# mvenouziou/Boosted_DETR

Measured on AMD Instinct MI355X. Metric: images/sec training step (fwd+matcher+loss+bwd), 640x640 N=100, higher is better.
Workload: dtype f32 (conv/GEMM products as 3 split-f16 [fwd] / split-bf16 [grad] MFMA products, f32 accumulate)

## Files before the change

### boosted_detr_amd/_lib.py

```python
from __future__ import annotations

import ctypes as C
import os
from pathlib import Path

_LIB_PATH = Path(os.environ.get("BDETR_LIB") or Path(__file__).resolve().parent / "csrc" / "libbdetr.so")
_lib = None

c_f32p = C.c_void_p
c_i32p = C.c_void_p
c_i64p = C.c_void_p
c_stream = C.c_void_p


class ConvDesc(C.Structure):
    _fields_ = [(n, C.c_int) for n in ("N", "H", "W", "C", "K", "R", "S", "stride", "pad", "OH", "OW")]


class GemmDesc(C.Structure):
    _fields_ = [
        ("I", C.c_int), ("J", C.c_int), ("R", C.c_int), ("nb0", C.c_int), ("nb1", C.c_int),
        ("a", C.c_void_p), ("lda", C.c_int64), ("sa0", C.c_int64), ("sa1", C.c_int64), ("a_rcontig", C.c_int),
        ("b", C.c_void_p), ("ldb", C.c_int64), ("sb0", C.c_int64), ("sb1", C.c_int64), ("b_rcontig", C.c_int),
        ("c", C.c_void_p), ("ldc", C.c_int64), ("sc0", C.c_int64), ("sc1", C.c_int64),
        ("bias", C.c_void_p), ("alpha", C.c_float), ("act", C.c_int), ("accumulate", C.c_int), ("splitk", C.c_int),
        ("grad", C.c_int),
    ]


class BnAffine(C.Structure):
    _fields_ = [("mean", C.c_void_p), ("rstd", C.c_void_p), ("gamma", C.c_void_p), ("beta", C.c_void_p)]


class BnBwdFuse(C.Structure):
    _fields_ = [("y", C.c_void_p), ("mean", C.c_void_p), ("rstd", C.c_void_p), ("gamma", C.c_void_p), ("beta", C.c_void_p), ("relu", C.c_int),
                ("part_g", C.c_void_p), ("part_gx", C.c_void_p), ("relu_mask", C.c_void_p),
                ("y2", C.c_void_p), ("mean2", C.c_void_p), ("rstd2", C.c_void_p), ("part_gx2", C.c_void_p)]


class RowchainFwdDesc(C.Structure):
    _fields_ = ([("M", C.c_int64), ("nstages", C.c_int), ("eps", C.c_float), ("rate", C.c_float), ("ctx", C.c_void_p), ("resid", C.c_void_p),
                 ("w", C.c_void_p * 3), ("bias", C.c_void_p * 3)]
                + [(n, C.c_void_p) for n in ("g1", "b1", "g2", "b2", "pre1", "x1", "mean1", "rstd1", "h", "pre2", "x2", "mean2", "rstd2")]
                + [("seed1", C.c_uint64), ("seed2", C.c_uint64), ("seed_base", C.c_void_p)])


class RowchainBwdDesc(C.Structure):
    _fields_ = ([("M", C.c_int64), ("nstages", C.c_int), ("rate", C.c_float)]
                + [(n, C.c_void_p) for n in ("dout", "pre2", "mean2", "rstd2", "g2", "h", "pre1", "mean1", "rstd1", "g1")]
                + [("wt", C.c_void_p * 3)]
                + [(n, C.c_void_p) for n in ("G2", "G1", "G0", "dresid", "dctx", "partials")]
                + [("seed1", C.c_uint64), ("seed2", C.c_uint64), ("seed_base", C.c_void_p)])


class LossDesc(C.Structure):
    _fields_ = [("B", C.c_int), ("M", C.c_int), ("N", C.c_int), ("C", C.c_int), ("A", C.c_int),
                ("category_weight", C.c_float), ("attribute_weight", C.c_float),
                ("box_weight", C.c_float), ("exist_weight", C.c_float)]


P = C.c_void_p
I = C.c_int
L = C.c_int64
F = C.c_float
U64 = C.c_uint64

SIGNATURES = {
    "bdetr_abi_version": (I, []),
    "bdetr_last_error": (C.c_char_p, []),
    "bdetr_device_cus": (I, []),
    "bdetr_low_priority_stream_create": (I, [P]),
    "bdetr_side_stream_candidates": (I, [P, I, I, I, P, P, P]),
    "bdetr_stream_destroy": (I, [P]),
    "bdetr_stream_priority_range": (I, [P, P]),
    "bdetr_set_gemm_precision": (I, [I]),
    "bdetr_get_gemm_precision": (I, []),
    "bdetr_prof_enable": (I, [I]),
    "bdetr_prof_read": (I, [P, P, P]),
    "bdetr_prof_read_arith": (I, [I, P, P, P]),
    "bdetr_prof_dump": (I, [C.c_char_p]),
    "bdetr_image_prep": (I, [P, I, I, I, P, I, I, P]),
    "bdetr_tokens_prepare": (I, [P, P, L, I, I, I, P, P, P]),
    "bdetr_augment_ws_floats": (I, [I]),
    "bdetr_augment": (I, [P, P, P, P, I, I, I, P, P]),
    "bdetr_jpeg_quality_ws_bytes": (C.c_int64, [I, I, I]),
    "bdetr_jpeg_quality": (I, [P, P, P, I, I, I, P, P]),
    "bdetr_augment_jpeg": (I, [P, P, P, P, P, I, I, I, P, P, P]),
    "bdetr_conv2d_fwd": (I, [P, P, P, P, C.POINTER(ConvDesc), I, P, P, P]),
    "bdetr_conv2d_fwd_stat_chunks": (I, [C.POINTER(ConvDesc)]),
    "bdetr_conv2d_bwd_data": (I, [P, P, P, C.POINTER(ConvDesc), I, P]),
    "bdetr_conv2d_bwd_weight": (I, [P, P, P, C.POINTER(ConvDesc), I, P]),
    "bdetr_conv2d_bwd_weight_splitk": (I, [C.POINTER(ConvDesc)]),
    "bdetr_bn_apply_p16": (I, [P, P, P, P, P, P, I, C.POINTER(BnAffine), I, P, P, P, P, P, L, I, P]),
    "bdetr_bn_bwd_p16": (I, [P, P, I, P, P, P, P, P, I, I, P, P, P, P, P, P, P, P, I, L, I, P]),
    "bdetr_bn_bwd_p16_even_pixels": (I, [P, P, I, P, P, P, P, P, I, I, P, P, P, P, P, P, I, I, I, I, I, P]),
    "bdetr_p16_supported": (I, [C.POINTER(ConvDesc)]),
    "bdetr_p16_pack": (I, [P, L, P, P, P, P]),
    "bdetr_p16_unpack": (I, [P, I, L, P, P]),
    "bdetr_p16_pack_conv_weights": (I, [P, I, I, I, I, P, P, P, P]),
    "bdetr_p16_pack_conv_weights_multi": (I, [P, I, P, P]),
    "bdetr_p16_conv2d_fwd_stat_chunks": (I, [C.POINTER(ConvDesc)]),
    "bdetr_p16_conv2d_fwd": (I, [P, P, P, P, C.POINTER(ConvDesc), I, P, P, P]),
    "bdetr_p16_conv2d_bwd_data": (I, [P, P, P, C.POINTER(ConvDesc), I, P]),
    "bdetr_p16_conv2d_bwd_data_stat_chunks": (I, [C.POINTER(ConvDesc)]),
    "bdetr_p16_conv2d_bwd_data_masked_accum": (I, [P, P, P, P, C.POINTER(ConvDesc), C.POINTER(BnBwdFuse), P]),
    "bdetr_p16_conv2d_bwd_data_masked_accum_compact": (I, [P, P, P, P, P, C.POINTER(ConvDesc), C.POINTER(BnBwdFuse), P]),
    "bdetr_relu_mask_apply": (I, [P, P, C.c_int64, P]),
    "bdetr_p16_conv2d_bwd_data_bnstats": (I, [P, P, P, C.POINTER(ConvDesc), C.POINTER(BnBwdFuse), P]),
    "bdetr_p16_conv2d_bwd_weight_splitk": (I, [C.POINTER(ConvDesc)]),
    "bdetr_p16_conv2d_bwd_weight": (I, [P, P, P, C.POINTER(ConvDesc), I, P]),
    "bdetr_p16_conv2d_bwd_weight_xf16": (I, [P, P, P, C.POINTER(ConvDesc), I, P]),
    "bdetr_gemm": (I, [C.POINTER(GemmDesc), P]),
    "bdetr_gemm_ws": (I, [C.POINTER(GemmDesc), P, L, P]),
    "bdetr_splitk_workspace_elems": (L, [L, L, I]),
    "bdetr_conv2d_bwd_weight_ws": (I, [P, P, P, C.POINTER(ConvDesc), I, P, L, P]),
    "bdetr_p16_conv2d_bwd_weight_ws": (I, [P, I, P, P, C.POINTER(ConvDesc), I, P, L, P]),
    "bdetr_gemm_grouped": (I, [C.POINTER(GemmDesc), I, P]),
    "bdetr_colsum_chunks": (I, [L]),
    "bdetr_colsum": (I, [P, L, I, P, P, P]),
    "bdetr_colsum_accumulate": (I, [P, L, I, P, P]),
    "bdetr_colsum_accumulate_group": (I, [P, P, I, P, I, P]),
    "bdetr_colstats": (I, [P, L, I, P, P, P]),
    "bdetr_bn_stats": (I, [P, L, I, P, P, I, F, F, I, P, P, P, P, P, P, P]),
    "bdetr_flag_nonfinite": (I, [P, L, P, P]),
    "bdetr_flag_snapshot": (I, [P, P, P, I, P]),
    "bdetr_debug_checksum": (I, [P, L, P, P, P, I, U64, P]),
    "bdetr_graph_node_census": (I, [P, P, I]),
    "bdetr_bn_stats_fold_rows": (I, []),
    "bdetr_bn_stats_frozen": (I, [P, P, I, F, P, P, P]),
    "bdetr_bn_apply": (I, [P, P, P, P, P, P, I, P, L, I, P]),
    "bdetr_bn_bwd_chunks": (I, [L]),
    "bdetr_bn_bwd": (I, [P, P, P, P, P, P, P, I, I, P, P, P, P, P, L, I, P]),
    "bdetr_bn_rows_stats": (I, [P, I, L, I, F, P, P, P, P, P]),
    "bdetr_bn_rows_apply": (I, [P, P, P, P, P, P, I, L, I, I, P, F, P, P, P, P]),
    "bdetr_bn_rows_bwd": (I, [P, P, P, P, P, I, I, P, P, P, P, I, L, I, P]),
    "bdetr_maxpool3x3s2_fwd": (I, [P, P, I, I, I, I, I, I, P]),
    "bdetr_maxpool3x3s2_bwd": (I, [P, P, P, P, I, I, I, I, I, I, P]),
    "bdetr_stem_pool_bwd_chunks": (I, [L]),
    "bdetr_stem_pool_fwd": (I, [P, P, P, P, P, I, I, I, I, P, P, P, P, P]),
    "bdetr_stem_pool_bwd": (I, [P, P, P, P, P, P, P, I, I, I, I, P, I, P, P, P, P]),
    "bdetr_p16_s2d_pack_bf16": (I, [P, I, I, I, P, P]),
    "bdetr_p16_stem_bwd_weight": (I, [P, P, P, I, I, I, I, P]),
    "bdetr_p16_s2d_unpack_dw": (I, [P, P, I, P]),
    "bdetr_attention_head_dim": (I, []),
    "bdetr_attention_fwd": (I, [P, P, P, P, P, I, I, I, I, F, P]),
    "bdetr_attention_bwd": (I, [P, P, P, P, P, P, P, P, P, P, I, I, I, I, F, P]),
    "bdetr_softmax_rows_fwd": (I, [P, P, L, I, F, P]),
    "bdetr_softmax_rows_bwd": (I, [P, P, P, L, I, F, P]),
    "bdetr_add_dropout_layernorm_fwd": (I, [P, P, P, P, P, P, P, L, I, F, F, U64, P, P]),
    "bdetr_ln_bwd_chunks": (I, [L]),
    "bdetr_add_dropout_layernorm_bwd": (I, [P, P, P, P, P, P, P, P, P, P, P, L, I, F, U64, P, I, P]),
    "bdetr_rowchain_fwd": (I, [C.POINTER(RowchainFwdDesc), P]),
    "bdetr_rowchain_bwd": (I, [C.POINTER(RowchainBwdDesc), P]),
    "bdetr_rowchain_reduce": (I, [P, I, C.POINTER(C.c_void_p * 7), C.POINTER(C.c_int * 7), P]),
    "bdetr_rowchain_width": (I, []),
    "bdetr_rowchain_pack_elems": (L, []),
    "bdetr_rowchain_partial_rows": (I, [L]),
    "bdetr_rowchain_pack_weights": (I, [P, I, P, P]),
    "bdetr_resize_bilinear_nhwc": (I, [P, I, I, I, I, P, I, I, P]),
    "bdetr_layernorm_act_fwd": (I, [P, L, I, I, P, P, F, F, P, I, P]),
    "bdetr_copy_cols": (I, [P, L, I, I, P, I, I, P]),
    "bdetr_nhwc_to_nchw": (I, [P, I, I, I, I, P, P]),
    "bdetr_layernorm_act_bwd_chunks": (I, [L]),
    "bdetr_layernorm_act_bwd": (I, [P, L, I, I, P, P, F, F, P, I, P, P, P, P, P, P]),
    "bdetr_resize_bilinear_nhwc_bwd": (I, [P, I, I, I, I, P, I, I, P]),
    "bdetr_nchw_to_nhwc": (I, [P, I, I, I, P, I, P]),
    "bdetr_conv_weight_pack": (I, [P, P, I, I, I, I, I, I, I, P, P, P]),
    "bdetr_conv_weight_unpack": (I, [P, P, I, I, I, I, I, I, P, P, P]),
    "bdetr_mask_loss": (I, [P, P, P, P, I, I, I, I, F, F, F, F, P, P, P, P]),
    "bdetr_softmax_lastdim_fwd": (I, [P, P, L, I, P]),
    "bdetr_softmax_lastdim_bwd": (I, [P, P, P, L, I, P]),
    "bdetr_sigmoid_fwd": (I, [P, P, L, P]),
    "bdetr_sigmoid_bwd": (I, [P, P, P, L, P]),
    "bdetr_boxsigmoid_fwd": (I, [P, P, L, P]),
    "bdetr_boxsigmoid_bwd": (I, [P, P, P, L, P]),
    "bdetr_zero": (I, [P, L, P]),
    "bdetr_add": (I, [P, P, P, L, P]),
    "bdetr_add_bcast_rows": (I, [P, P, P, L, L, P]),
    "bdetr_sum_over_batch": (I, [P, P, L, L, I, P]),
    "bdetr_tanh_bwd": (I, [P, P, P, L, P]),
    "bdetr_relu_bwd": (I, [P, P, P, L, P]),
    "bdetr_axpy": (I, [F, P, P, L, P]),
    "bdetr_cost_matrix": (I, [C.POINTER(LossDesc), P, P, P, P, P, P, P, P, P, P, P, P]),
    "bdetr_lsa": (I, [P, P, I, I, I, P, P]),
    "bdetr_set_loss": (I, [C.POINTER(LossDesc), P, P, P, P, P, P, P, P, P, P, P, P, F, P]),
    "bdetr_cost_matrix_tiled": (I, [C.POINTER(LossDesc), I, P, P, P, P, P, P, P, P, P]),
    "bdetr_lsa_tiled": (I, [P, P, I, I, I, I, P, P]),
    "bdetr_set_loss_tiled": (I, [C.POINTER(LossDesc), I, P, P, P, P, P, P, P, P, P, P, P, P, F, P]),
    "bdetr_match_to_mask": (I, [P, P, I, I, I, P]),
    "bdetr_sgd_slab_elems": (I, []),
    "bdetr_sgd_nesterov_clipnorm": (I, [P, P, I, P, P, I, P, P, P, F, F, F, P, P]),
    "bdetr_adamw_clipnorm": (I, [P, P, I, P, P, I, P, P, P, P, F, F, F, F, F, F, F, P, P]),
    "bdetr_det_postprocess": (I, [P, I, I, I, P, P, P]),
    "bdetr_det_match": (I, [P, P, P, P, P, P, P, I, I, I, I, I, I, P, P, P, P, P]),
    "bdetr_mask_binarize": (I, [P, L, I, F, P, P, P]),
    "bdetr_mask_match": (I, [P, P, P, P, P, P, P, P, P, I, I, I, I, I, I, I, P, P, P, P, P]),
    "bdetr_det_match_coco": (I, [P] * 11 + [I] * 7 + [P] * 7),
    "bdetr_mask_match_coco": (I, [P] * 13 + [I] * 8 + [P] * 7),
    "bdetr_mask_targets": (I, [P, L, P, P, P, P, I, I, I, P, P, P]),
    "bdetr_mask_upsample_bits": (I, [P, P, I, I, I, I, I, P, P, P]),
    "bdetr_mask_source_bits": (I, [P, L, P, P, P, I, I, I, I, P, P, P]),
    "bdetr_mask_inter": (I, [P, P, P, I, I, I, I, I, P, P]),
    "bdetr_mask_match_coco_inter": (I, [P] * 13 + [I] * 7 + [P] * 7),
    "bdetr_panoptic_select": (I, [P, P, P, I, I, I, F, P, P]),
    "bdetr_panoptic_merge": (I, [P, P, P, I, I, I, I, I, P, P, P, P]),
    "bdetr_panoptic_gt_exclusive": (I, [P, P, P, I, I, I, I, I, P, P]),
    "bdetr_panoptic_match": (I, [P] * 8 + [I] * 5 + [P] * 5),
}


class BdetrError(RuntimeError):
    pass


def lib_path() -> Path:
    return _LIB_PATH


def lib():
    global _lib
    if _lib is not None:
        return _lib
    if not _LIB_PATH.exists():
        raise BdetrError(
            f"{_LIB_PATH} not found: the HIP extension is not built. Run `python -m boosted_detr_amd.build` "
            "(or __graft_entry__.build()). There is no CPU fallback in the product path.")
    import torch
    h = C.CDLL(str(_LIB_PATH))
    for name, (res, args) in SIGNATURES.items():
        fn = getattr(h, name)
        fn.restype = res
        fn.argtypes = args
    if h.bdetr_abi_version() != 8:
        raise BdetrError("libbdetr.so ABI version mismatch; rebuild")
    _lib = h
    return _lib


def check(status: int, what: str = "") -> None:
    if status != 0:
        msg = lib().bdetr_last_error().decode(errors="replace")
        raise BdetrError(f"{what or 'libbdetr'} failed (status {status}): {msg}")
```

### boosted_detr_amd/build.py

```python
from __future__ import annotations

import hashlib
import os
import subprocess
import sys
from concurrent.futures import ThreadPoolExecutor
from pathlib import Path

CSRC = Path(__file__).resolve().parent / "csrc"
LIB = CSRC / "libbdetr.so"
OBJ_DIR = CSRC / "_obj"
SOURCES = ["common.cpp", "igemm.hip", "sgemm.hip", "hconv.hip", "hwgrad.hip", "p16.hip", "attention.hip", "rowchain.hip", "augment.hip", "norm.hip", "groupnorm_rows.hip", "elementwise.hip", "panoptic.hip", "matcher.hip", "optim.hip", "detmetric.hip", "maskmetric.hip", "maskraster.hip", "maskimage.hip", "panopticmerge.hip"]
ARCH = "gfx950"
COMMON_FLAGS = ["-O3", "-fPIC", f"--offload-arch={ARCH}", "-std=c++20", "-Wall", "-Wno-unused-function"] + os.environ.get("BDETR_CXXFLAGS", "").split()
PER_FILE_FLAGS = {"matcher.hip": ["-ffp-contract=off"], "detmetric.hip": ["-ffp-contract=off"], "maskmetric.hip": ["-ffp-contract=off"],
                  "maskraster.hip": ["-ffp-contract=off"], "maskimage.hip": ["-ffp-contract=off"], "panopticmerge.hip": ["-ffp-contract=off"]}


def _hipcc() -> str:
    for cand in (os.environ.get("HIPCC"), "/opt/rocm/bin/hipcc", "hipcc"):
        if cand and (os.path.isabs(cand) and os.path.exists(cand) or not os.path.isabs(cand)):
            return cand
    raise RuntimeError("hipcc not found")


def _digest(paths) -> str:
    h = hashlib.sha256()
    for p in sorted(paths):
        h.update(p.name.encode())
        h.update(p.read_bytes())
    return h.hexdigest()


def build(force: bool = False, verbose: bool = True) -> Path:
    deps = [CSRC / s for s in SOURCES] + [CSRC / "common.h", CSRC / "gemm_common.h", CSRC / "p16.h", CSRC.parent.parent / "include" / "bdetr.h"]
    stamp = CSRC / "_obj" / "stamp"
    dig = _digest(deps) + "|" + " ".join(COMMON_FLAGS)
    if not force and LIB.exists() and stamp.exists() and stamp.read_text() == dig:
        return LIB
    OBJ_DIR.mkdir(exist_ok=True)
    hipcc = _hipcc()

    headers = [d for d in deps if d.suffix == ".h"]

    def compile_one(src: str) -> Path:
        obj = OBJ_DIR / (src.rsplit(".", 1)[0] + ".o")
        flags = COMMON_FLAGS + PER_FILE_FLAGS.get(src, [])
        ostamp = OBJ_DIR / (src + ".stamp")
        odig = _digest([CSRC / src] + headers) + "|" + " ".join(flags)
        if not force and obj.exists() and ostamp.exists() and ostamp.read_text() == odig:
            return obj
        cmd = [hipcc, *flags, "-x", "hip", "-c", str(CSRC / src), "-o", str(obj)]
        if verbose:
            print(" ".join(cmd), flush=True)
        subprocess.run(cmd, check=True)
        ostamp.write_text(odig)
        return obj

    with ThreadPoolExecutor(max_workers=min(8, len(SOURCES))) as ex:
        objs = list(ex.map(compile_one, SOURCES))
    cmd = [hipcc, "-shared", "-fPIC", f"--offload-arch={ARCH}", *map(str, objs), "-o", str(LIB)]
    if verbose:
        print(" ".join(cmd), flush=True)
    subprocess.run(cmd, check=True)
    stamp.write_text(dig)
    return LIB


if __name__ == "__main__":
    build(force="--force" in sys.argv)
    print(LIB)
```

### boosted_detr_amd/csrc/igemm.hip

```cpp
#include "gemm_common.h"
#include <stdlib.h>
#include <string.h>
#include <type_traits>
#include <utility>
#include <vector>

using namespace bdgemm;

namespace {

constexpr int BK = 32;
constexpr int RPAD = 4;
constexpr int NTHREADS = 256;

constexpr int SLD = 36;
constexpr int SLD3 = 52;
constexpr float LO_SCALE = 2048.f;
typedef __bf16 bf16x2 __attribute__((ext_vector_type(2)));
typedef __bf16 bf16x8 __attribute__((ext_vector_type(8)));
typedef _Float16 f16x2 __attribute__((ext_vector_type(2)));
typedef _Float16 f16x8 __attribute__((ext_vector_type(8)));
typedef float f32x2 __attribute__((ext_vector_type(2)));

template <int ARITH>
__device__ __forceinline__ void split2(float x0, float x1, unsigned& hi, unsigned& lo) {
    f32x2 v; v[0] = x0; v[1] = x1;
    if (ARITH == AR_BF16X3) {
        hi = __builtin_bit_cast(unsigned, __builtin_convertvector(v, bf16x2));
        f32x2 r;
        r[0] = x0 - __builtin_bit_cast(float, hi << 16);
        r[1] = x1 - __builtin_bit_cast(float, hi & 0xFFFF0000u);
        lo = __builtin_bit_cast(unsigned, __builtin_convertvector(r, bf16x2));
    } else {
        const f16x2 h = __builtin_convertvector(v, f16x2);
        hi = __builtin_bit_cast(unsigned, h);
        const f32x2 r = (v - __builtin_convertvector(h, f32x2)) * LO_SCALE;
        lo = __builtin_bit_cast(unsigned, __builtin_convertvector(r, f16x2));
    }
}

__device__ __forceinline__ void split3(float x0, float x1, unsigned& hi, unsigned& mid, unsigned& lo) {
    f32x2 v; v[0] = x0; v[1] = x1;
    hi = __builtin_bit_cast(unsigned, __builtin_convertvector(v, bf16x2));
    f32x2 r;
    r[0] = x0 - __builtin_bit_cast(float, hi << 16);
    r[1] = x1 - __builtin_bit_cast(float, hi & 0xFFFF0000u);
    mid = __builtin_bit_cast(unsigned, __builtin_convertvector(r, bf16x2));
    r[0] -= __builtin_bit_cast(float, mid << 16);
    r[1] -= __builtin_bit_cast(float, mid & 0xFFFF0000u);
    lo = __builtin_bit_cast(unsigned, __builtin_convertvector(r, bf16x2));
}

struct DenseOp { const float* p; int64_t ld, s0, s1; int rows, cols; };
struct PatchOp { const float* p; int N, H, W, C, OH, OW, R, S, stride, pad; int rows, cols; };
struct WFlipOp { const float* p; int K, C, R, S; int rows, cols; };

typedef unsigned int u32x4 __attribute__((ext_vector_type(4)));
typedef unsigned int u32x2 __attribute__((ext_vector_type(2)));
constexpr unsigned OOB = 0xFFFFFFF0u;
constexpr unsigned NUM_RECORDS = 0xFFFFFF00u;

__device__ __forceinline__ __amdgpu_buffer_rsrc_t make_rsrc(const float* p) {
    const unsigned long long a = reinterpret_cast<unsigned long long>(p);
    const unsigned lo = __builtin_amdgcn_readfirstlane((unsigned)a), hi = __builtin_amdgcn_readfirstlane((unsigned)(a >> 32));
    void* q = reinterpret_cast<void*>(((unsigned long long)hi << 32) | lo);
    return __builtin_amdgcn_make_buffer_rsrc(q, 0, (int)NUM_RECORDS, 0x00020000);
}
__device__ __forceinline__ f32x4 buf_load4(__amdgpu_buffer_rsrc_t r, unsigned byte_off) {
    return __builtin_bit_cast(f32x4, __builtin_amdgcn_raw_buffer_load_b128(r, (int)byte_off, 0, 0));
}
__device__ __forceinline__ float buf_load1(__amdgpu_buffer_rsrc_t r, unsigned byte_off) {
    return __builtin_bit_cast(float, __builtin_amdgcn_raw_buffer_load_b32(r, (int)byte_off, 0, 0));
}

template <int VEC>
struct DenseLoader {
    using Op = DenseOp;
    struct Ctx { unsigned off; bool ok; };
    static __device__ __forceinline__ const float* batch_base(const Op& op, int b0, int b1) {
        return op.p + (int64_t)b0 * op.s0 + (int64_t)b1 * op.s1;
    }
    static __device__ __forceinline__ void regroup(Op& op, const float* p, int x_extent, bool rc) {
        op.p = p;
        if (x_extent >= 0) { if (rc) op.rows = x_extent; else op.cols = x_extent; }
    }
    static __device__ __forceinline__ Ctx row_ctx(const Op& op, int row, int row_limit) {
        Ctx c; c.ok = row < row_limit; c.off = (unsigned)row * (unsigned)op.ld; return c;
    }
    static __device__ __forceinline__ f32x4 load(__amdgpu_buffer_rsrc_t rs, const Op& op, const Ctx& c, int col, int col_limit) {
        if (VEC == 4) {
            return buf_load4(rs, (c.ok && col < col_limit) ? (c.off + (unsigned)col) * 4u : OOB);
        } else {
            f32x4 v;
#pragma unroll
            for (int e = 0; e < 4; ++e) v[e] = buf_load1(rs, (c.ok && col + e < col_limit) ? (c.off + (unsigned)(col + e)) * 4u : OOB);
            return v;
        }
    }
};

struct PatchLoader {
    using Op = PatchOp;
    struct Ctx { int nbase; int ih0, iw0; bool ok; };
    static __device__ __forceinline__ const float* batch_base(const Op& op, int, int) { return op.p; }
    static __device__ __forceinline__ void regroup(Op&, const float*, int, bool) {}
    static __device__ __forceinline__ Ctx row_ctx(const Op& op, int row, int row_limit) {
        Ctx c; c.ok = row < row_limit;
        int ohw = op.OH * op.OW;
        int n = row / ohw; int rem = row - n * ohw;
        int oh = rem / op.OW; int ow = rem - oh * op.OW;
        c.nbase = n * op.H * op.W;
        c.ih0 = oh * op.stride - op.pad; c.iw0 = ow * op.stride - op.pad;
        return c;
    }
    static __device__ __forceinline__ f32x4 load(__amdgpu_buffer_rsrc_t rs, const Op& op, const Ctx& c, int col, int col_limit) {
        int tap = col / op.C; int ch = col - tap * op.C;
        int r = tap / op.S; int s = tap - r * op.S;
        int ih = c.ih0 + r, iw = c.iw0 + s;
        const bool ok = c.ok && col < col_limit && (unsigned)ih < (unsigned)op.H && (unsigned)iw < (unsigned)op.W;
        const unsigned off = ((unsigned)(c.nbase + ih * op.W + iw) * (unsigned)op.C + (unsigned)ch) * 4u;
        return buf_load4(rs, ok ? off : OOB);
    }
};

struct WFlipLoader {
    using Op = WFlipOp;
    struct Ctx { unsigned off; bool ok; };
    static __device__ __forceinline__ const float* batch_base(const Op& op, int, int) { return op.p; }
    static __device__ __forceinline__ void regroup(Op&, const float*, int, bool) {}
    static __device__ __forceinline__ Ctx row_ctx(const Op& op, int row, int row_limit) {
        Ctx c; c.ok = row < row_limit;
        int tap = row / op.K; int k = row - tap * op.K;
        int r = tap / op.S; int s = tap - r * op.S;
        c.off = (unsigned)(((k * op.R + (op.R - 1 - r)) * op.S + (op.S - 1 - s)) * op.C);
        return c;
    }
    static __device__ __forceinline__ f32x4 load(__amdgpu_buffer_rsrc_t rs, const Op& op, const Ctx& c, int col, int col_limit) {
        return buf_load4(rs, (c.ok && col < col_limit) ? (c.off + (unsigned)col) * 4u : OOB);
    }
};

template <int BX, bool RC>
struct TileGeom {
    static constexpr int LDS_FLOATS = RC ? BX * (BK + RPAD) : BK * BX;
    static constexpr int NV = BX * BK / 4 / NTHREADS;
    static constexpr int VPR = RC ? BK / 4 : BX / 4;
    static constexpr int LDS_LD = RC ? BK + RPAD : BX;
};

template <int BM, int BN, int WM, int WN, class LA, bool A_RC, class LB, bool B_RC, int ARITH>
__global__ __launch_bounds__(NTHREADS, 2)
void igemm_kernel(typename LA::Op opa, typename LB::Op opb, GemmParams g)
{
    static_assert(WM * WN == 4, "4 waves per workgroup");
    constexpr int WTM = BM / WM, WTN = BN / WN;
    constexpr int TM = WTM / 32, TN = WTN / 32;
    static_assert(TM >= 1 && TN >= 1, "wave tile must hold at least one 32x32 MFMA tile");
    using GA = TileGeom<BM, A_RC>;
    using GB = TileGeom<BN, B_RC>;
    static_assert(GA::NV >= 1 && GB::NV >= 1, "tile too small for 256 threads");

    constexpr bool SPLIT = ARITH != AR_FP32;
    constexpr bool X6 = ARITH == AR_BF16X6;
    constexpr int SLDK = X6 ? SLD3 : SLD;
    constexpr int A_FLOATS = SPLIT ? BM * SLDK : GA::LDS_FLOATS;
    constexpr int B_FLOATS = SPLIT ? BN * SLDK : GB::LDS_FLOATS;
    constexpr int STAGE_FLOATS = A_FLOATS + B_FLOATS;
    static_assert(!SPLIT || ((A_RC || GA::NV % 2 == 0) && (B_RC || GB::NV % 2 == 0)), "split mode transposes k-pairs");
    __shared__ __attribute__((aligned(16))) float lds[2 * STAGE_FLOATS];

    const int tid = threadIdx.x;
    const int lane = tid & 63;
    const int wave = tid >> 6;
    const int wm = wave / WN, wn = wave % WN;
    const int li = lane & 31, lh = lane >> 5;

    const int nwg_ = g.tiles_i * g.tiles_j;
    const bool sk_ = g.ngroups == 0 && g.splitk > 1;
    const int lin_ = sk_ ? xcd_tile(blockIdx.z * nwg_ + blockIdx.x, nwg_ * gridDim.z) : xcd_tile(blockIdx.x, nwg_);
    const int zz_ = sk_ ? lin_ / nwg_ : blockIdx.z;
    const int wg = sk_ ? lin_ - zz_ * nwg_ : lin_;
    const int tile_i = wg / g.tiles_j, tile_j = wg - tile_i * g.tiles_j;
    const int i0 = tile_i * BM, j0 = tile_j * BN;

    int b0 = 0, b1 = 0, r_begin = 0, r_end = g.R;
    if (g.ngroups > 0) {
        const int z = g.splitk > 1 ? (int)blockIdx.z / g.splitk : (int)blockIdx.z;
        if (g.splitk > 1) {
            r_begin = ((int)blockIdx.z - z * g.splitk) * g.r_chunk;
            r_end = min(g.R, r_begin + g.r_chunk);
        }
#define BDETR_PICK(arr) (z == 0 ? g.arr[0] : z == 1 ? g.arr[1] : z == 2 ? g.arr[2] : g.arr[3])
        g.I = BDETR_PICK(gI); g.c = BDETR_PICK(gc); g.bias = BDETR_PICK(gbias);
        const float* pa = BDETR_PICK(ga);
        const float* pb = BDETR_PICK(gb);
#undef BDETR_PICK
        if (i0 >= g.I) return;
        LA::regroup(opa, pa, g.I, A_RC);
        LB::regroup(opb, pb, -1, B_RC);
    } else if (g.splitk > 1) {
        r_begin = zz_ * g.r_chunk;
        r_end = min(g.R, r_begin + g.r_chunk);
    } else {
        b0 = blockIdx.z / g.nb1; b1 = blockIdx.z - b0 * g.nb1;
    }
    const __amdgpu_buffer_rsrc_t rsA = make_rsrc(LA::batch_base(opa, b0, b1));
    const __amdgpu_buffer_rsrc_t rsB = make_rsrc(LB::batch_base(opb, b0, b1));
    const int a_rows = A_RC ? opa.rows : min(opa.rows, r_end), a_cols = A_RC ? min(opa.cols, r_end) : opa.cols;
    const int b_rows = B_RC ? opb.rows : min(opb.rows, r_end), b_cols = B_RC ? min(opb.cols, r_end) : opb.cols;

    typename LA::Ctx ctxA[GA::NV];
    typename LB::Ctx ctxB[GB::NV];
    int colA[GA::NV], colB[GB::NV], ldsoffA[GA::NV], ldsoffB[GB::NV], rowA[GA::NV], rowB[GB::NV];
    auto stage_geom = [&](int p, int vpr, int bx, bool rc, int lds_ld, int& row, int& col, int& ldsoff) {
        if (!SPLIT) {
            const int v = tid + NTHREADS * p;
            const int rt = v / vpr, c4 = v - rt * vpr;
            row = rt; col = 4 * c4; ldsoff = rt * lds_ld + 4 * c4;
        } else if (rc) {
            const int v = tid + NTHREADS * p;
            const int q = v / vpr, c4 = v - q * vpr;
            const int rt = (q & ~15) | ((q & 3) << 2) | ((q >> 2) & 3);
            row = rt; col = 4 * c4;
            ldsoff = rt * SLDK * 32 + ((((c4 >> 1) ^ ((rt >> 4) & 7)) << 2) | ((c4 & 1) << 1));
        } else {
            const int u = tid + NTHREADS * (p >> 1);
            const int kp = u / (bx / 4), c4 = u - kp * (bx / 4);
            row = 2 * kp + (p & 1); col = 4 * c4;
            ldsoff = (4 * c4) * SLDK * 32 + ((((kp >> 2) ^ ((c4 >> 2) & 7)) << 2) | (kp & 3));
        }
    };
#pragma unroll
    for (int p = 0; p < GA::NV; ++p) {
        stage_geom(p, GA::VPR, BM, A_RC, GA::LDS_LD, rowA[p], colA[p], ldsoffA[p]);
        if (A_RC) ctxA[p] = LA::row_ctx(opa, i0 + rowA[p], a_rows);
    }
#pragma unroll
    for (int p = 0; p < GB::NV; ++p) {
        stage_geom(p, GB::VPR, BN, B_RC, GB::LDS_LD, rowB[p], colB[p], ldsoffB[p]);
        if (B_RC) ctxB[p] = LB::row_ctx(opb, j0 + rowB[p], b_rows);
    }

    f32x4 stA0[GA::NV], stB0[GB::NV], stA1[GA::NV], stB1[GB::NV];
    auto load_stage = [&](int r0, f32x4 (&ra)[GA::NV], f32x4 (&rb)[GB::NV]) {
#pragma unroll
        for (int p = 0; p < GA::NV; ++p) {
            if (A_RC) ra[p] = LA::load(rsA, opa, ctxA[p], r0 + colA[p], a_cols);
            else      ra[p] = LA::load(rsA, opa, LA::row_ctx(opa, r0 + rowA[p], a_rows), i0 + colA[p], a_cols);
        }
#pragma unroll
        for (int p = 0; p < GB::NV; ++p) {
            if (B_RC) rb[p] = LB::load(rsB, opb, ctxB[p], r0 + colB[p], b_cols);
            else      rb[p] = LB::load(rsB, opb, LB::row_ctx(opb, r0 + rowB[p], b_rows), j0 + colB[p], b_cols);
        }
    };
    auto write_split = [&](unsigned* base, bool rc, auto nv_c, const f32x4* r, const int* ldsoff) {
        constexpr int nv = decltype(nv_c)::value;
        if (rc) {
#pragma unroll
            for (int p = 0; p < nv; ++p) {
                unsigned* row = base + (ldsoff[p] >> 5);
                const int w = ldsoff[p] & 31;
                if constexpr (X6) {
                    unsigned h0, m0, l0, h1, m1, l1;
                    split3(r[p][0], r[p][1], h0, m0, l0);
                    split3(r[p][2], r[p][3], h1, m1, l1);
                    u32x2 hi, mid, lo;
                    hi[0] = h0; hi[1] = h1; mid[0] = m0; mid[1] = m1; lo[0] = l0; lo[1] = l1;
                    *reinterpret_cast<u32x2*>(row + w) = hi;
                    *reinterpret_cast<u32x2*>(row + (w ^ 16)) = mid;
                    *reinterpret_cast<u32x2*>(row + 32 + (w & 15)) = lo;
                } else {
                    unsigned h0, l0, h1, l1;
                    split2<ARITH>(r[p][0], r[p][1], h0, l0);
                    split2<ARITH>(r[p][2], r[p][3], h1, l1);
                    u32x2 hi, lo;
                    hi[0] = h0; hi[1] = h1; lo[0] = l0; lo[1] = l1;
                    *reinterpret_cast<u32x2*>(row + w) = hi;
                    *reinterpret_cast<u32x2*>(row + (w ^ 16)) = lo;
                }
            }
        } else {
#pragma unroll
            for (int p = 0; p + 1 < nv; p += 2) {
                unsigned* row = base + (ldsoff[p] >> 5);
                const int w = ldsoff[p] & 31;
#pragma unroll
                for (int e = 0; e < 4; ++e) {
                    if constexpr (X6) {
                        unsigned hi, mid, lo;
                        split3(r[p][e], r[p + 1][e], hi, mid, lo);
                        row[e * SLDK + w] = hi;
                        row[e * SLDK + (w ^ 16)] = mid;
                        row[e * SLDK + 32 + (w & 15)] = lo;
                    } else {
                        unsigned hi, lo;
                        split2<ARITH>(r[p][e], r[p + 1][e], hi, lo);
                        row[e * SLDK + w] = hi;
                        row[e * SLDK + (w ^ 16)] = lo;
                    }
                }
            }
        }
    };
    auto write_stage = [&](int buf, const f32x4 (&ra)[GA::NV], const f32x4 (&rb)[GB::NV]) {
        if (SPLIT) {
            unsigned* st = reinterpret_cast<unsigned*>(lds + buf * STAGE_FLOATS);
            write_split(st, A_RC, std::integral_constant<int, GA::NV>{}, ra, ldsoffA);
            write_split(st + A_FLOATS, B_RC, std::integral_constant<int, GB::NV>{}, rb, ldsoffB);
            return;
        }
#pragma unroll
        for (int p = 0; p < GA::NV; ++p) *reinterpret_cast<f32x4*>(lds + buf * STAGE_FLOATS + ldsoffA[p]) = ra[p];
#pragma unroll
        for (int p = 0; p < GB::NV; ++p) *reinterpret_cast<f32x4*>(lds + buf * STAGE_FLOATS + GA::LDS_FLOATS + ldsoffB[p]) = rb[p];
    };

    constexpr int TM2 = ARITH == AR_FP16X3 ? TM : 1, TN2 = ARITH == AR_FP16X3 ? TN : 1;
    f32x16 acc[TM][TN], acc2[TM2][TN2];
#pragma unroll
    for (int a = 0; a < TM; ++a)
#pragma unroll
        for (int b = 0; b < TN; ++b)
#pragma unroll
            for (int e = 0; e < 16; ++e) acc[a][b][e] = 0.f;
#pragma unroll
    for (int a = 0; a < TM2; ++a)
#pragma unroll
        for (int b = 0; b < TN2; ++b)
#pragma unroll
            for (int e = 0; e < 16; ++e) acc2[a][b][e] = 0.f;

    auto compute = [&](int buf) {
        if (SPLIT) {
            const unsigned* qA = reinterpret_cast<const unsigned*>(lds + buf * STAGE_FLOATS);
            const unsigned* qB = qA + A_FLOATS;
#pragma unroll
            for (int ks = 0; ks < BK / 16; ++ks) {
                u32x4 ah[TM], al[TM], bh[TN], bl[TN];
                u32x4 a3[X6 ? TM : 1], b3[X6 ? TN : 1];
#pragma unroll
                for (int a = 0; a < TM; ++a) {
                    const int xb = wm * WTM + a * 32 + li;
                    const int w = ((ks * 2 + lh) ^ ((xb >> 4) & 7)) << 2;
                    ah[a] = *reinterpret_cast<const u32x4*>(qA + xb * SLDK + w);
                    al[a] = *reinterpret_cast<const u32x4*>(qA + xb * SLDK + (w ^ 16));
                    if constexpr (X6) a3[a] = *reinterpret_cast<const u32x4*>(qA + xb * SLDK + 32 + (w & 15));
                }
#pragma unroll
                for (int b = 0; b < TN; ++b) {
                    const int xb = wn * WTN + b * 32 + li;
                    const int w = ((ks * 2 + lh) ^ ((xb >> 4) & 7)) << 2;
                    bh[b] = *reinterpret_cast<const u32x4*>(qB + xb * SLDK + w);
                    bl[b] = *reinterpret_cast<const u32x4*>(qB + xb * SLDK + (w ^ 16));
                    if constexpr (X6) b3[b] = *reinterpret_cast<const u32x4*>(qB + xb * SLDK + 32 + (w & 15));
                }
#pragma unroll
                for (int a = 0; a < TM; ++a)
#pragma unroll
                    for (int b = 0; b < TN; ++b) {
                        if constexpr (X6) {
#define BF8(v) __builtin_bit_cast(bf16x8, v)
                            acc[a][b] = __builtin_amdgcn_mfma_f32_32x32x16_bf16(BF8(a3[a]), BF8(bh[b]), acc[a][b], 0, 0, 0);
                            acc[a][b] = __builtin_amdgcn_mfma_f32_32x32x16_bf16(BF8(ah[a]), BF8(b3[b]), acc[a][b], 0, 0, 0);
                            acc[a][b] = __builtin_amdgcn_mfma_f32_32x32x16_bf16(BF8(al[a]), BF8(bl[b]), acc[a][b], 0, 0, 0);
                            acc[a][b] = __builtin_amdgcn_mfma_f32_32x32x16_bf16(BF8(al[a]), BF8(bh[b]), acc[a][b], 0, 0, 0);
                            acc[a][b] = __builtin_amdgcn_mfma_f32_32x32x16_bf16(BF8(ah[a]), BF8(bl[b]), acc[a][b], 0, 0, 0);
                            acc[a][b] = __builtin_amdgcn_mfma_f32_32x32x16_bf16(BF8(ah[a]), BF8(bh[b]), acc[a][b], 0, 0, 0);
#undef BF8
                        } else if constexpr (ARITH == AR_BF16X3) {
#define BF8(v) __builtin_bit_cast(bf16x8, v)
                            acc[a][b] = __builtin_amdgcn_mfma_f32_32x32x16_bf16(BF8(al[a]), BF8(bh[b]), acc[a][b], 0, 0, 0);
                            acc[a][b] = __builtin_amdgcn_mfma_f32_32x32x16_bf16(BF8(ah[a]), BF8(bl[b]), acc[a][b], 0, 0, 0);
                            acc[a][b] = __builtin_amdgcn_mfma_f32_32x32x16_bf16(BF8(ah[a]), BF8(bh[b]), acc[a][b], 0, 0, 0);
#undef BF8
                        } else if constexpr (ARITH == AR_FP16X3) {
#define H8(v) __builtin_bit_cast(f16x8, v)
                            acc2[a][b] = __builtin_amdgcn_mfma_f32_32x32x16_f16(H8(al[a]), H8(bh[b]), acc2[a][b], 0, 0, 0);
                            acc2[a][b] = __builtin_amdgcn_mfma_f32_32x32x16_f16(H8(ah[a]), H8(bl[b]), acc2[a][b], 0, 0, 0);
                            acc[a][b] = __builtin_amdgcn_mfma_f32_32x32x16_f16(H8(ah[a]), H8(bh[b]), acc[a][b], 0, 0, 0);
#undef H8
                        }
                    }
            }
            return;
        }
        const float* sA = lds + buf * STAGE_FLOATS;
        const float* sB = sA + GA::LDS_FLOATS;
#pragma unroll
        for (int kb = 0; kb < BK / 8; ++kb) {
            f32x4 fa[TM], fb[TN];
#pragma unroll
            for (int a = 0; a < TM; ++a) {
                const int xb = wm * WTM + a * 32 + li;
                if (A_RC) {
                    fa[a] = *reinterpret_cast<const f32x4*>(sA + xb * GA::LDS_LD + kb * 8 + 4 * lh);
                } else {
#pragma unroll
                    for (int e = 0; e < 4; ++e) fa[a][e] = sA[(kb * 8 + 4 * lh + e) * GA::LDS_LD + xb];
                }
            }
#pragma unroll
            for (int b = 0; b < TN; ++b) {
                const int xb = wn * WTN + b * 32 + li;
                if (B_RC) {
                    fb[b] = *reinterpret_cast<const f32x4*>(sB + xb * GB::LDS_LD + kb * 8 + 4 * lh);
                } else {
#pragma unroll
                    for (int e = 0; e < 4; ++e) fb[b][e] = sB[(kb * 8 + 4 * lh + e) * GB::LDS_LD + xb];
                }
            }
#pragma unroll
            for (int e = 0; e < 4; ++e)
#pragma unroll
                for (int a = 0; a < TM; ++a)
#pragma unroll
                    for (int b = 0; b < TN; ++b)
                        acc[a][b] = __builtin_amdgcn_mfma_f32_32x32x2f32(fa[a][e], fb[b][e], acc[a][b], 0, 0, 0);
        }
    };

    const int nk = (r_end - r_begin + BK - 1) / BK;
    constexpr bool PF1 = SPLIT && BM * BN >= 128 * 128;
    if constexpr (PF1) {
        if (nk > 0) { load_stage(r_begin, stA0, stB0); write_stage(0, stA0, stB0); }
        __syncthreads();
        for (int kt = 0; kt < nk; ++kt) {
            if (kt + 1 < nk) load_stage(r_begin + (kt + 1) * BK, stA0, stB0);
            compute(kt & 1);
            if (kt + 1 < nk) write_stage((kt + 1) & 1, stA0, stB0);
            __syncthreads();
        }
    } else {
    if (nk > 0) {
        load_stage(r_begin, stA0, stB0);
        if (nk > 1) load_stage(r_begin + BK, stA1, stB1);
        write_stage(0, stA0, stB0);
    }
    __syncthreads();

    for (int kt = 0; kt < nk; kt += 2) {
        if (kt + 2 < nk) load_stage(r_begin + (kt + 2) * BK, stA0, stB0);
        compute(0);
        if (kt + 1 < nk) write_stage(1, stA1, stB1);
        __syncthreads();
        if (kt + 1 >= nk) break;
        if (kt + 3 < nk) load_stage(r_begin + (kt + 3) * BK, stA1, stB1);
        compute(1);
        if (kt + 2 < nk) write_stage(0, stA0, stB0);
        __syncthreads();
    }
    }

    if constexpr (ARITH == AR_FP16X3) {
#pragma unroll
        for (int a = 0; a < TM; ++a)
#pragma unroll
            for (int b = 0; b < TN; ++b)
#pragma unroll
                for (int e = 0; e < 16; ++e) acc[a][b][e] += acc2[a][b][e] * (1.f / LO_SCALE);
    }
    gemm_epilogue<BM, BN, WM, WN, NTHREADS, 2 * STAGE_FLOATS>(acc, g, lds, tile_i, i0, j0, g.c + (int64_t)(sk_ ? zz_ : b0) * g.sc0 + (int64_t)b1 * g.sc1);
}

struct TileChoice { int bm, bn; };

}

namespace bdgemm {
int g_num_cus = 0;
int num_cus() {
    if (g_num_cus == 0) {
        int dev = 0; hipDeviceProp_t p;
        if (hipGetDevice(&dev) == hipSuccess && hipGetDeviceProperties(&p, dev) == hipSuccess) g_num_cus = p.multiProcessorCount;
        if (g_num_cus <= 0) g_num_cus = 256;
    }
    return g_num_cus;
}
}

namespace {

}
namespace bdgemm {
thread_local int g_gemm_mode = -1;
int gemm_mode() {
    if (g_gemm_mode < 0) {
        const char* e = getenv("BDETR_GEMM_PRECISION");
        g_gemm_mode = !e ? BDETR_GEMM_MIXED : (!strcmp(e, "fp32") || !strcmp(e, "f32")) ? BDETR_GEMM_FP32
                    : !strcmp(e, "bf16x3") ? BDETR_GEMM_BF16X3 : !strcmp(e, "split") ? BDETR_GEMM_SPLIT : !strcmp(e, "bf16x6") ? BDETR_GEMM_BF16X6 : BDETR_GEMM_MIXED;
    }
    return g_gemm_mode;
}
}
namespace {
int use_split(bool grad) {
    switch (gemm_mode()) {
        case BDETR_GEMM_FP32:   return AR_FP32;
        case BDETR_GEMM_BF16X3: return AR_BF16X3;
        case BDETR_GEMM_SPLIT:  return grad ? AR_BF16X3 : AR_FP16X3;
        case BDETR_GEMM_BF16X6: return AR_BF16X6;
        default:                return grad ? AR_BF16X3 : AR_FP32;
    }
}

TileChoice choose_tile(int I, int J, int zdim, bool both_rc, bool split, bool patch = false) {
    static int forced_bm = -1, forced_bn = -1;
    if (forced_bm < 0) {
        forced_bm = forced_bn = 0;
        if (const char* e = getenv("BDETR_TILE")) sscanf(e, "%dx%d", &forced_bm, &forced_bn);
    }
    if (forced_bm > 0) {
        if (J <= 32) return {128, 32};
        return {forced_bm, forced_bn};
    }
    auto tiles = [&](int bm, int bn) { return cdiv64(I, bm) * cdiv64(J, bn) * zdim; };
    if (J <= 32) return {128, 32};
    if (split) {
        if (both_rc && J % 128 == 0 && tiles(128, 128) * 4 >= 3LL * num_cus()) return {128, 128};
        if (patch && !both_rc && I % 128 == 0 && J % 128 == 0 && (zdim > 1 || tiles(128, 128) * 4 >= 3LL * num_cus())) return {128, 128};
        return {64, 64};
    }
    if (tiles(128, 128) >= 16LL * num_cus() && J >= 1024) return {128, 128};
    return {64, 64};
}

struct ProfRec { hipEvent_t e0, e1; double flops; int I, J, R, z, bm, bn, kind; };
std::vector<ProfRec> g_prof_recs;
std::vector<std::pair<hipEvent_t, hipEvent_t>> g_prof_pool;
size_t g_prof_used = 0;

template <class L> struct LoaderId { static constexpr int v = 0; };
template <> struct LoaderId<PatchLoader> { static constexpr int v = 1; };
template <> struct LoaderId<WFlipLoader> { static constexpr int v = 2; };
template <> struct LoaderId<DenseLoader<1>> { static constexpr int v = 3; };

}
namespace bdgemm {
bool g_prof_on = false;
void prof_begin(hipStream_t st, double flops, int I, int J, int R, int z, int bm, int bn, int kind) {
    if (g_prof_used == g_prof_pool.size()) {
        hipEvent_t a, b;
        if (hipEventCreate(&a) != hipSuccess || hipEventCreate(&b) != hipSuccess) return;
        g_prof_pool.emplace_back(a, b);
    }
    auto& ev = g_prof_pool[g_prof_used++];
    g_prof_recs.push_back({ev.first, ev.second, flops, I, J, R, z, bm, bn, kind});
    (void)hipEventRecord(ev.first, st);
}
void prof_end(hipStream_t st) { (void)hipEventRecord(g_prof_recs.back().e1, st); }
}
namespace {

template <int BM, int BN, int WM, int WN, class LA, bool A_RC, class LB, bool B_RC, int ARITH = AR_FP32>
int launch_cfg(const typename LA::Op& a, const typename LB::Op& b, GemmParams g, int zdim, hipStream_t st) {
    g.tiles_i = (int)cdiv64(g.I, BM);
    g.tiles_j = (int)cdiv64(g.J, BN);
    dim3 grid(g.tiles_i * g.tiles_j, 1, zdim);
    g.vec_store = (g.J % 4 == 0) && (g.ldc % 4 == 0) && (g.sc0 % 4 == 0) && (g.sc1 % 4 == 0) && ((reinterpret_cast<uintptr_t>(g.c) & 15) == 0);
    const bool prof = g_prof_on;
    if (prof) prof_begin(st, 2.0 * (double)g.I * (double)g.J * (double)g.R * (g.splitk > 1 ? (g.ngroups > 0 ? (double)g.ngroups : 1.0) : (double)zdim), g.I, g.J, g.R, zdim, BM, BN,
                         ARITH * 10000 + LoaderId<LA>::v * 1000 + (A_RC ? 100 : 0) + LoaderId<LB>::v * 10 + (B_RC ? 1 : 0));
    hipLaunchKernelGGL((igemm_kernel<BM, BN, WM, WN, LA, A_RC, LB, B_RC, ARITH>), grid, dim3(NTHREADS), 0, st, a, b, g);
    if (prof) prof_end(st);
    return bdetr_launch_status("igemm");
}

template <class LA, bool A_RC, class LB, bool B_RC>
int launch_any(const typename LA::Op& a, const typename LB::Op& b, GemmParams g, int zdim, hipStream_t st, int arith, bool small_only = false) {
    if (arith == AR_FP16X3 && !(A_RC && B_RC)) arith = AR_FP32;
    constexpr bool PATCH = LoaderId<LA>::v == 1 || LoaderId<LB>::v == 1;
    TileChoice t = small_only ? TileChoice{64, 64} : choose_tile(g.I, g.J, g.splitk > 1 ? 2 : zdim, A_RC && B_RC, arith != AR_FP32, PATCH);
    if constexpr (LoaderId<LA>::v != 3 && LoaderId<LB>::v != 3) {
        if (arith == AR_BF16X3 && t.bn >= 64) {
            if (t.bm == 128 && t.bn == 128) return launch_cfg<128, 128, 2, 2, LA, A_RC, LB, B_RC, AR_BF16X3>(a, b, g, zdim, st);
            if (t.bm == 128 && t.bn == 64)  return launch_cfg<128, 64, 2, 2, LA, A_RC, LB, B_RC, AR_BF16X3>(a, b, g, zdim, st);
            return launch_cfg<64, 64, 2, 2, LA, A_RC, LB, B_RC, AR_BF16X3>(a, b, g, zdim, st);
        }
        if (arith == AR_BF16X6 && t.bn >= 64) {
            if (t.bm == 128) return launch_cfg<128, 64, 2, 2, LA, A_RC, LB, B_RC, AR_BF16X6>(a, b, g, zdim, st);
            return launch_cfg<64, 64, 2, 2, LA, A_RC, LB, B_RC, AR_BF16X6>(a, b, g, zdim, st);
        }
        if constexpr (A_RC && B_RC) {
            if (arith == AR_FP16X3 && t.bn >= 64) {
                if (t.bm == 128 && t.bn == 128) return launch_cfg<128, 128, 2, 2, LA, A_RC, LB, B_RC, AR_FP16X3>(a, b, g, zdim, st);
                if (t.bm == 128 && t.bn == 64)  return launch_cfg<128, 64, 2, 2, LA, A_RC, LB, B_RC, AR_FP16X3>(a, b, g, zdim, st);
                return launch_cfg<64, 64, 2, 2, LA, A_RC, LB, B_RC, AR_FP16X3>(a, b, g, zdim, st);
            }
        }
    }
    if (t.bm == 128 && t.bn == 128) return launch_cfg<128, 128, 2, 2, LA, A_RC, LB, B_RC>(a, b, g, zdim, st);
    if (t.bm == 128 && t.bn == 64)  return launch_cfg<128, 64, 2, 2, LA, A_RC, LB, B_RC>(a, b, g, zdim, st);
    if (t.bm == 128 && t.bn == 32)  return launch_cfg<128, 32, 4, 1, LA, A_RC, LB, B_RC>(a, b, g, zdim, st);
    return launch_cfg<64, 64, 2, 2, LA, A_RC, LB, B_RC>(a, b, g, zdim, st);
}

constexpr int64_t MAX_OPERAND_ELEMS = (int64_t)(NUM_RECORDS / 4) - 64;
bool span_ok(int64_t elems) { return elems >= 0 && elems <= MAX_OPERAND_ELEMS; }
int64_t dense_span(const DenseOp& o) { return (int64_t)(o.rows - 1) * o.ld + o.cols; }

int stat_chunks(int I, int J) {
    TileChoice t = choose_tile(I, J, 1, true, use_split(false) != AR_FP32);
    const int wm = (t.bm == 128 && t.bn == 32) ? 4 : 2;
    return (int)cdiv64(I, t.bm) * wm;
}

__global__ __launch_bounds__(256) void splitk_fold_kernel(const float* __restrict__ ws, int zdim, int64_t slab, float* __restrict__ dst, int64_t n) {
    const int64_t i = ((int64_t)blockIdx.x * 256 + threadIdx.x) * 4;
    if (i >= n) return;
    if (i + 4 <= n && (reinterpret_cast<uintptr_t>(dst) & 15) == 0) {
        f32x4 a = *reinterpret_cast<const f32x4*>(ws + i);
        for (int z = 1; z < zdim; ++z) a += *reinterpret_cast<const f32x4*>(ws + (int64_t)z * slab + i);
        f32x4 d = *reinterpret_cast<f32x4*>(dst + i);
        d += a;
        *reinterpret_cast<f32x4*>(dst + i) = d;
    } else {
        for (int64_t k = i; k < n && k < i + 4; ++k) {
            float a = ws[k];
            for (int z = 1; z < zdim; ++z) a += ws[(int64_t)z * slab + k];
            dst[k] += a;
        }
    }
}

}

namespace bdgemm {
int splitk_fold(const float* ws, int zdim, int64_t slab, float* dst, int64_t n, hipStream_t st) {
    hipLaunchKernelGGL(splitk_fold_kernel, dim3((unsigned)cdiv64(cdiv64(n, 4), 256)), dim3(256), 0, st, ws, zdim, slab, dst, n);
    return bdetr_launch_status("splitk_fold");
}
}

extern "C" int64_t bdetr_splitk_workspace_elems(int64_t I, int64_t J, int splitk) {
    return splitk > 1 ? (int64_t)splitk * bdgemm::splitk_slab(I * J) : 0;
}

extern "C" int bdetr_device_cus(void) { return num_cus(); }

extern "C" int bdetr_set_gemm_precision(int mode) {
    BDETR_CHECK_ARG(mode >= BDETR_GEMM_FP32 && mode <= BDETR_GEMM_BF16X6, "bdetr_set_gemm_precision: unknown mode %d", mode);
    bdgemm::g_gemm_mode = mode;
    return 0;
}
extern "C" int bdetr_get_gemm_precision(void) { return gemm_mode(); }

extern "C" int bdetr_prof_enable(int on) {
    g_prof_on = on != 0;
    if (on) { g_prof_recs.clear(); g_prof_used = 0; }
    return 0;
}
extern "C" int bdetr_prof_dump(const char* path) {
    FILE* f = fopen(path, "w");
    if (!f) { bdetr_set_error("bdetr_prof_dump: cannot open %s", path); return -1; }
    fprintf(f, "I,J,R,z,bm,bn,kind,ms,gflop\n");
    for (auto& r : g_prof_recs) {
        float t = 0.f;
        if (hipEventElapsedTime(&t, r.e0, r.e1) != hipSuccess) t = -1.f;
        fprintf(f, "%d,%d,%d,%d,%d,%d,%d,%.5f,%.4f\n", r.I, r.J, r.R, r.z, r.bm, r.bn, r.kind, t, r.flops * 1e-9);
    }
    fclose(f);
    return 0;
}

static int prof_sum(int arith, double* total_ms, int64_t* launches, double* flops) {
    double ms = 0, fl = 0; int64_t n = 0;
    for (auto& r : g_prof_recs) {
        if (arith >= 0 && r.kind / 10000 != arith) continue;
        float t = 0.f;
        hipError_t e = hipEventElapsedTime(&t, r.e0, r.e1);
        if (e != hipSuccess) { bdetr_set_error("bdetr_prof_read: %s", hipGetErrorString(e)); return (int)e; }
        ms += t; fl += r.flops; ++n;
    }
    if (total_ms) *total_ms = ms;
    if (launches) *launches = n;
    if (flops) *flops = fl;
    return 0;
}
extern "C" int bdetr_prof_read(double* total_ms, int64_t* launches, double* flops) { return prof_sum(-1, total_ms, launches, flops); }
extern "C" int bdetr_prof_read_arith(int arith, double* total_ms, int64_t* launches, double* flops) {
    BDETR_CHECK_ARG(arith >= AR_FP32 && arith <= AR_BF16X6, "bdetr_prof_read_arith: arith must be 0 (fp32), 1 (bf16x3), 2 (fp16x3), 3 (pre-split f16), 4 (pre-split bf16) or 5 (bf16x6)");
    return prof_sum(arith, total_ms, launches, flops);
}

extern "C" int bdetr_gemm_grouped(const bdetr_gemm_desc* d, int n, void* stream) {
    BDETR_CHECK_ARG(d && n >= 1 && n <= 4, "bdetr_gemm_grouped: 1..4 problems");
    GemmParams g; init_params(g);
    int maxI = 0;
    bool v4 = true;
    for (int k = 0; k < n; ++k) {
        const bdetr_gemm_desc& e = d[k];
        BDETR_CHECK_ARG(e.a && e.b && e.c && e.I > 0, "bdetr_gemm_grouped: null pointer / empty problem %d", k);
        BDETR_CHECK_ARG(e.J == d[0].J && e.R == d[0].R && e.a_rcontig == d[0].a_rcontig && e.b_rcontig == d[0].b_rcontig &&
                        e.act == d[0].act && e.alpha == d[0].alpha && e.accumulate == d[0].accumulate &&
                        e.lda == d[0].lda && e.ldb == d[0].ldb && e.ldc == d[0].ldc,
                        "bdetr_gemm_grouped: problems must share J, R, leading dimensions, flavours and epilogue");
        BDETR_CHECK_ARG(e.grad == d[0].grad, "bdetr_gemm_grouped: problems must share the grad flag");
        BDETR_CHECK_ARG((e.nb0 <= 1) && (e.nb1 <= 1) && e.splitk == d[0].splitk, "bdetr_gemm_grouped: no batching inside a group; one split-K factor for all problems");
        BDETR_CHECK_ARG(e.splitk <= 1 || (!e.bias && e.act == 0 && e.I == d[0].I), "bdetr_gemm_grouped: split-K problems are plain GEMMs of one shape (C += partial products, atomics)");
        BDETR_CHECK_ARG(span_ok((int64_t)(e.a_rcontig ? e.I : e.R) * e.lda) && span_ok((int64_t)(e.b_rcontig ? e.J : e.R) * e.ldb),
                        "bdetr_gemm_grouped: operand %d spans 4 GB or more (32-bit buffer offsets)", k);
        g.ga[k] = e.a; g.gb[k] = e.b; g.gc[k] = e.c; g.gbias[k] = e.bias; g.gI[k] = e.I;
        if (e.I > maxI) maxI = e.I;
        v4 = v4 && aligned16(e.a) && aligned16(e.b) && aligned16(e.c);
    }
    const bdetr_gemm_desc& f = d[0];
    bool dims4 = f.J % 4 == 0 && (f.a_rcontig || f.b_rcontig ? f.R % 4 == 0 : true);
    for (int k = 0; k < n; ++k) dims4 = dims4 && (f.a_rcontig || d[k].I % 4 == 0);
    BDETR_CHECK_ARG(v4 && f.lda % 4 == 0 && f.ldb % 4 == 0 && f.ldc % 4 == 0 && dims4,
                    "bdetr_gemm_grouped: operands must be 16-byte aligned with contiguous dimensions that are multiples of 4");
    g.ngroups = n;
    g.I = maxI; g.J = f.J; g.R = f.R;
    g.c = f.c; g.ldc = f.ldc; g.bias = f.bias; g.alpha = f.alpha; g.act = f.act;
    g.mode = f.accumulate ? ST_ACCUM : ST_STORE;
    int zdim = n;
    if (f.splitk > 1) {
        g.r_chunk = (int)(cdiv64(cdiv64(f.R, f.splitk), BK) * BK);
        g.splitk = (int)cdiv64(f.R, g.r_chunk);
        g.mode = ST_ATOMIC;
        zdim = n * g.splitk;
    }
    DenseOp a{f.a, f.lda, 0, 0, f.a_rcontig ? maxI : f.R, f.a_rcontig ? f.R : maxI};
    DenseOp b{f.b, f.ldb, 0, 0, f.b_rcontig ? f.J : f.R, f.b_rcontig ? f.R : f.J};
    hipStream_t st = (hipStream_t)stream;
    const bool arc = f.a_rcontig != 0, brc = f.b_rcontig != 0;
    const int sp = use_split(f.grad != 0);
    if (arc && brc)   return launch_any<DenseLoader<4>, true, DenseLoader<4>, true>(a, b, g, zdim, st, sp);
    if (arc && !brc)  return launch_any<DenseLoader<4>, true, DenseLoader<4>, false>(a, b, g, zdim, st, sp);
    if (!arc && !brc) return launch_any<DenseLoader<4>, false, DenseLoader<4>, false>(a, b, g, zdim, st, sp);
    return launch_any<DenseLoader<4>, false, DenseLoader<4>, true>(a, b, g, zdim, st, sp, true);
}

extern "C" int bdetr_gemm(const bdetr_gemm_desc* d, void* stream) { return bdetr_gemm_ws(d, nullptr, 0, stream); }

template <class F>
static int with_splitk_slabs(GemmParams& g, int zdim, float* ws, int64_t ws_elems, hipStream_t st, const char* who, F&& launch) {
    float* c = g.c;
    const int64_t n = (int64_t)g.I * g.J, slab = splitk_slab(n);
    BDETR_CHECK_ARG(g.ldc == g.J, "%s: the split-K workspace form needs a dense C (ldc == J)", who);
    BDETR_CHECK_ARG(aligned16(ws) && ws_elems >= (int64_t)zdim * slab, "%s: workspace too small or misaligned (%lld floats, need %lld)", who,
                    (long long)ws_elems, (long long)((int64_t)zdim * slab));
    g.c = ws; g.sc0 = slab; g.mode = ST_STORE;
    if (int e = launch()) return e;
    return splitk_fold(ws, zdim, slab, c, n, st);
}

extern "C" int bdetr_gemm_ws(const bdetr_gemm_desc* d, float* ws, int64_t ws_elems, void* stream) {
    BDETR_CHECK_ARG(d && d->a && d->b && d->c, "bdetr_gemm: null pointer");
    BDETR_CHECK_ARG(d->I > 0 && d->J > 0 && d->R >= 0, "bdetr_gemm: bad shape I=%d J=%d R=%d", d->I, d->J, d->R);
    const int nb0 = d->nb0 > 0 ? d->nb0 : 1, nb1 = d->nb1 > 0 ? d->nb1 : 1;
    const int splitk = d->splitk > 1 ? d->splitk : 1;
    BDETR_CHECK_ARG(splitk == 1 || (nb0 * nb1 == 1 && !d->bias && d->act == 0), "bdetr_gemm: splitk needs a single plain GEMM");
    hipStream_t st = (hipStream_t)stream;

    DenseOp a{d->a, d->lda, d->sa0, d->sa1, d->a_rcontig ? d->I : d->R, d->a_rcontig ? d->R : d->I};
    DenseOp b{d->b, d->ldb, d->sb0, d->sb1, d->b_rcontig ? d->J : d->R, d->b_rcontig ? d->R : d->J};
    BDETR_CHECK_ARG(span_ok(dense_span(a)) && span_ok(dense_span(b)),
                    "bdetr_gemm: an operand matrix spans 4 GB or more (32-bit buffer offsets); split the problem");
    GemmParams g; init_params(g);
    g.I = d->I; g.J = d->J; g.R = d->R; g.nb1 = nb1;
    g.c = d->c; g.ldc = d->ldc; g.sc0 = d->sc0; g.sc1 = d->sc1;
    g.bias = d->bias; g.alpha = d->alpha; g.act = d->act;
    g.mode = splitk > 1 ? ST_ATOMIC : (d->accumulate ? ST_ACCUM : ST_STORE);
    int zdim = nb0 * nb1;
    if (splitk > 1) {
        g.splitk = splitk;
        g.r_chunk = (int)(cdiv64(cdiv64(d->R, splitk), BK) * BK);
        zdim = (int)cdiv64(d->R, g.r_chunk);
        g.splitk = zdim > 1 ? zdim : 2;
    }
    auto vec_ok = [&](const DenseOp& o) {
        return aligned16(o.p) && o.ld % 4 == 0 && o.s0 % 4 == 0 && o.s1 % 4 == 0 && o.cols % 4 == 0;
    };
    const bool v4 = vec_ok(a) && vec_ok(b);
    const bool arc = d->a_rcontig != 0, brc = d->b_rcontig != 0;
    const int sp = use_split(d->grad != 0);
    auto launch = [&]() -> int {
        if (v4) {
            if (arc && brc)   return launch_any<DenseLoader<4>, true, DenseLoader<4>, true>(a, b, g, zdim, st, sp);
            if (arc && !brc)  return launch_any<DenseLoader<4>, true, DenseLoader<4>, false>(a, b, g, zdim, st, sp);
            if (!arc && !brc) return launch_any<DenseLoader<4>, false, DenseLoader<4>, false>(a, b, g, zdim, st, sp);
            return launch_any<DenseLoader<4>, false, DenseLoader<4>, true>(a, b, g, zdim, st, sp, true);
        }
        if (arc && brc)   return launch_any<DenseLoader<1>, true, DenseLoader<1>, true>(a, b, g, zdim, st, AR_FP32, true);
        if (arc && !brc)  return launch_any<DenseLoader<1>, true, DenseLoader<1>, false>(a, b, g, zdim, st, AR_FP32, true);
        if (!arc && !brc) return launch_any<DenseLoader<1>, false, DenseLoader<1>, false>(a, b, g, zdim, st, AR_FP32, true);
        return launch_any<DenseLoader<1>, false, DenseLoader<1>, true>(a, b, g, zdim, st, AR_FP32, true);
    };
    if (ws != nullptr && splitk > 1) return with_splitk_slabs(g, zdim, ws, ws_elems, st, "bdetr_gemm_ws", launch);
    return launch();
}

static int check_conv(const bdetr_conv_desc* d, const char* who) {
    BDETR_CHECK_ARG(d != nullptr, "%s: null desc", who);
    BDETR_CHECK_ARG(d->N > 0 && d->H > 0 && d->W > 0 && d->C > 0 && d->K > 0 && d->R > 0 && d->S > 0 && d->stride > 0 && d->pad >= 0,
                    "%s: bad conv geometry", who);
    BDETR_CHECK_ARG(d->C % 4 == 0, "%s: input channels must be a multiple of 4 (got %d)", who, d->C);
    BDETR_CHECK_ARG(d->OH == (d->H + 2 * d->pad - d->R) / d->stride + 1 && d->OW == (d->W + 2 * d->pad - d->S) / d->stride + 1,
                    "%s: OH/OW inconsistent with geometry", who);
    BDETR_CHECK_ARG((int64_t)d->N * d->OH * d->OW < (1LL << 31) && (int64_t)d->R * d->S * d->C < (1LL << 31), "%s: problem too large", who);
    BDETR_CHECK_ARG(span_ok((int64_t)d->N * d->H * d->W * d->C) && span_ok((int64_t)d->N * d->OH * d->OW * d->K) && span_ok((int64_t)d->K * d->R * d->S * d->C),
                    "%s: a tensor spans 4 GB or more (the loaders use 32-bit buffer offsets); use a smaller per-GPU batch", who);
    return 0;
}

extern "C" int bdetr_conv2d_fwd_stat_chunks(const bdetr_conv_desc* d) {
    if (check_conv(d, "bdetr_conv2d_fwd_stat_chunks")) return -1;
    return stat_chunks(d->N * d->OH * d->OW, d->K);
}

extern "C" int bdetr_conv2d_fwd(const float* x, const float* w, const float* bias, float* y,
                                const bdetr_conv_desc* d, int act, float* stat_sum, float* stat_sq, void* stream) {
    if (int e = check_conv(d, "bdetr_conv2d_fwd")) return e;
    BDETR_CHECK_ARG(x && w && y, "bdetr_conv2d_fwd: null pointer");
    BDETR_CHECK_ARG(aligned16(x) && aligned16(w), "bdetr_conv2d_fwd: x and w must be 16-byte aligned");
    BDETR_CHECK_ARG((stat_sum == nullptr) == (stat_sq == nullptr), "bdetr_conv2d_fwd: stat_sum/stat_sq must both be set or both null");
    const int M = d->N * d->OH * d->OW, Kd = d->R * d->S * d->C;
    GemmParams g; init_params(g);
    g.I = M; g.J = d->K; g.R = Kd;
    g.c = y; g.ldc = d->K; g.bias = bias; g.act = act;
    g.stat_sum = stat_sum; g.stat_sq = stat_sq;
    DenseOp wop{w, Kd, 0, 0, d->K, Kd};
    hipStream_t st = (hipStream_t)stream;
    if (d->R == 1 && d->S == 1 && d->stride == 1 && d->pad == 0) {
        DenseOp xop{x, d->C, 0, 0, M, d->C};
        return launch_any<DenseLoader<4>, true, DenseLoader<4>, true>(xop, wop, g, 1, st, use_split(false));
    }
    PatchOp xop{x, d->N, d->H, d->W, d->C, d->OH, d->OW, d->R, d->S, d->stride, d->pad, M, Kd};
    return launch_any<PatchLoader, true, DenseLoader<4>, true>(xop, wop, g, 1, st, use_split(false));
}

extern "C" int bdetr_conv2d_bwd_data(const float* dy, const float* w, float* dx,
                                     const bdetr_conv_desc* d, int accumulate, void* stream) {
    if (int e = check_conv(d, "bdetr_conv2d_bwd_data")) return e;
    BDETR_CHECK_ARG(dy && w && dx, "bdetr_conv2d_bwd_data: null pointer");
    BDETR_CHECK_ARG(d->K % 4 == 0, "bdetr_conv2d_bwd_data: output channels must be a multiple of 4");
    hipStream_t st = (hipStream_t)stream;
    const int M = d->N * d->OH * d->OW;
    GemmParams g; init_params(g);
    g.c = dx; g.ldc = d->C; g.mode = accumulate ? ST_ACCUM : ST_STORE;
    if (d->R == 1 && d->S == 1 && d->pad == 0) {
        g.I = M; g.J = d->C; g.R = d->K;
        if (d->stride > 1) {
            if (!accumulate) {
                if (int e = bdetr_zero_bytes(dx, sizeof(float) * (size_t)d->N * d->H * d->W * d->C, st)) return e;
            }
            g.rowmap = 1; g.rm_OW = d->OW; g.rm_OHOW = d->OH * d->OW; g.rm_H = d->H; g.rm_W = d->W; g.rm_stride = d->stride;
        }
        DenseOp a{dy, d->K, 0, 0, M, d->K};
        DenseOp b{w, d->C, 0, 0, d->K, d->C};
        return launch_any<DenseLoader<4>, true, DenseLoader<4>, false>(a, b, g, 1, st, use_split(true));
    }
    if (d->stride > 1 && d->pad == 0 && d->R <= d->stride && d->S <= d->stride) {
        if (!accumulate) {
            if (int e = bdetr_zero_bytes(dx, sizeof(float) * (size_t)d->N * d->H * d->W * d->C, st)) return e;
        }
        g.I = M; g.J = d->C; g.R = d->K;
        g.rowmap = 1; g.rm_OW = d->OW; g.rm_OHOW = d->OH * d->OW; g.rm_H = d->H; g.rm_W = d->W; g.rm_stride = d->stride;
        DenseOp a{dy, d->K, 0, 0, M, d->K};
        for (int r = 0; r < d->R; ++r)
            for (int s = 0; s < d->S; ++s) {
                g.rm_off = r * d->W + s;
                DenseOp b{w + (int64_t)(r * d->S + s) * d->C, (int64_t)d->R * d->S * d->C, 0, 0, d->K, d->C};
                if (int e = launch_any<DenseLoader<4>, true, DenseLoader<4>, false>(a, b, g, 1, st, use_split(true))) return e;
            }
        return 0;
    }
    BDETR_CHECK_ARG(d->stride == 1, "bdetr_conv2d_bwd_data: stride>1 only for 1x1 convs or taps that do not overlap (R, S <= stride, pad 0)");
    const int Mx = d->N * d->H * d->W;
    g.I = Mx; g.J = d->C; g.R = d->R * d->S * d->K;
    PatchOp a{dy, d->N, d->OH, d->OW, d->K, d->H, d->W, d->R, d->S, 1, d->R - 1 - d->pad, Mx, d->R * d->S * d->K};
    BDETR_CHECK_ARG(d->R == d->S, "bdetr_conv2d_bwd_data: square kernels only");
    WFlipOp b{w, d->K, d->C, d->R, d->S, d->R * d->S * d->K, d->C};
    return launch_any<PatchLoader, true, WFlipLoader, false>(a, b, g, 1, st, use_split(true));
}

extern "C" int bdetr_conv2d_bwd_weight_splitk(const bdetr_conv_desc* d) {
    if (check_conv(d, "bdetr_conv2d_bwd_weight_splitk")) return -1;
    const int M = d->N * d->OH * d->OW, Kd = d->R * d->S * d->C;
    TileChoice t = choose_tile(d->K, Kd, 2, false, use_split(true) != AR_FP32, !(d->R == 1 && d->S == 1 && d->stride == 1 && d->pad == 0));
    int64_t tiles = cdiv64(d->K, t.bm) * cdiv64(Kd, t.bn);
    int64_t want = 3LL * num_cus();
    const bool few_tiles = tiles <= 8 && M >= (1 << 20);
    if (few_tiles) want = 16LL * num_cus();
    int64_t sk = cdiv64(want, tiles);
// ... 42 lines not shown
```

### boosted_detr_amd/engine.py

```python
from __future__ import annotations

import math
import zlib
from typing import Callable, Dict, List, Optional, Sequence

import numpy as np
import torch

from . import kernels as K

_DEVICE = None


def device() -> torch.device:
    global _DEVICE
    if _DEVICE is None:
        if not torch.cuda.is_available():
            raise RuntimeError("boosted_detr_amd needs an AMD GPU (HIP device); there is no CPU execution path")
        _DEVICE = torch.device("cuda", torch.cuda.current_device())
    return _DEVICE


def to_device(a, dtype=torch.float32) -> torch.Tensor:
    if isinstance(a, torch.Tensor):
# ... 50 lines not shown
            a = a.T
        return np.ascontiguousarray(a)

    def _to_keras(self, a: np.ndarray) -> np.ndarray:
        if self.kind == "conv_kernel":
            if self.pad_in_channels:
                a = a[..., : a.shape[3] - self.pad_in_channels]
            a = np.transpose(a, (1, 2, 3, 0))
        elif self.kind == "dense_kernel":
            a = a.T
        return np.ascontiguousarray(a)

    def assign(self, keras_array) -> None:
        t = to_device(self._to_internal(np.asarray(keras_array)))
        bump_weights_version()
        if self.value is None:
            self.value = t
        else:
            self.value.copy_(t)

    def numpy(self) -> np.ndarray:
        return self._to_keras(self.value.detach().cpu().numpy())

    def grad_numpy(self) -> np.ndarray:
        return self._to_keras(self.grad.detach().cpu().numpy())

    @property
    def num_params(self) -> int:
        return int(np.prod(self.keras_shape))

    @property
    def needs_grad(self) -> bool:
        return self.trainable and getattr(self, "owner", None) is not None and self.owner.trainable

    def reset_grad(self) -> None:
        self.grad, self._grad_fresh = None, False


def _seed_for(name: str, seed: int) -> int:
    return (zlib.crc32(name.encode()) ^ (seed * 0x9E3779B1)) & 0xFFFFFFFF


def _fans(shape):
    if len(shape) == 2:
        return shape[0], shape[1]
    rf = int(np.prod(shape[:-2]))
    return shape[-2] * rf, shape[-1] * rf


def initializer(kind: str) -> Callable:
    def trunc_normal(rng, shape, std):
        out = rng.standard_normal(shape)
        bad = np.abs(out) > 2.0
        while bad.any():
            out[bad] = rng.standard_normal(int(bad.sum()))
            bad = np.abs(out) > 2.0
        return (out * std / 0.87962566103423978).astype(np.float32)

    def init(name, shape, seed=0):
        rng = np.random.Generator(np.random.PCG64(_seed_for(name, seed)))
        fan_in, fan_out = _fans(shape) if len(shape) >= 2 else (shape[0], shape[0])
        if kind == "zeros":
            return np.zeros(shape, np.float32)
        if kind == "ones":
            return np.ones(shape, np.float32)
        if kind == "glorot_normal":
            return trunc_normal(rng, shape, math.sqrt(2.0 / (fan_in + fan_out)))
        if kind == "he_normal":
            return trunc_normal(rng, shape, math.sqrt(2.0 / fan_in))
        if kind == "lecun_normal":
            return trunc_normal(rng, shape, math.sqrt(1.0 / fan_in))
        if kind == "glorot_uniform":
            lim = math.sqrt(6.0 / (fan_in + fan_out))
            return rng.uniform(-lim, lim, size=shape).astype(np.float32)
        raise ValueError(kind)

    return init


class GradInfo:
    __slots__ = ("owned", "lazy_mask", "compact_even", "even_pixels", "bnb_parts", "bnb_parts_shortcut")

    def __init__(self):
        self.owned = False
        self.lazy_mask = self.compact_even = self.even_pixels = self.bnb_parts = self.bnb_parts_shortcut = None


_NO_INFO = GradInfo()


def info(g) -> GradInfo:
    return getattr(g, "_grad_info", _NO_INFO)


def tag(g: torch.Tensor) -> GradInfo:
    r = getattr(g, "_grad_info", None)
    if r is None:
        r = g._grad_info = GradInfo()
    return r


def own(t: torch.Tensor) -> torch.Tensor:
    tag(t).owned = True
    return t


def dense_contribution(g: torch.Tensor, keep_even=None) -> None:
    r = info(g)
    if r is _NO_INFO:
        return
    r.bnb_parts = r.bnb_parts_shortcut = None
    if r.even_pixels != keep_even:
        r.even_pixels = None


def materialise(g):
    r = info(g)
    if r.compact_even is not None:
        N, H, W = r.compact_even
        d = torch.empty(N, H, W, g.shape[-1], dtype=g.dtype, device=g.device)
        K.zero_(d)
        d[:, ::2, ::2] = g.view(N, H // 2, W // 2, g.shape[-1])
        mask, r = r.lazy_mask, tag(d)
        r.owned, r.even_pixels, r.lazy_mask = True, (N, H, W), mask
        g = d
    if r.lazy_mask is not None:
        K.relu_mask_apply_(g, r.lazy_mask)
        r.lazy_mask = None
    return g


class Tape:

    def __init__(self):
        self.nodes: List[tuple] = []

    def record(self, outputs: Sequence[torch.Tensor], inputs: Sequence[Optional[torch.Tensor]], fn: Callable) -> None:
        self.nodes.append((tuple(outputs), tuple(inputs), fn))

    def backward(self, seeds: Dict[int, torch.Tensor]) -> Dict[int, torch.Tensor]:
        grads: Dict[int, torch.Tensor] = dict(seeds)
        for outputs, inputs, fn in reversed(self.nodes):
            gouts = [grads.pop(id(o), None) for o in outputs]
            if all(g is None for g in gouts):
                continue
            if not getattr(fn, "accepts_lazy", False):
                gouts = [materialise(g) for g in gouts]
            acc = None
            if getattr(fn, "wants_acc", False):
                acc = []
                for t in inputs:
                    have = grads.get(id(t)) if t is not None else None
                    acc.append(have if info(have).owned else None)
                gins = fn(*gouts, acc=acc)
            else:
                gins = fn(*gouts)
            if not isinstance(gins, (tuple, list)):
                gins = (gins,)
            assert len(gins) == len(inputs), (len(gins), len(inputs))
            for i, (t, g) in enumerate(zip(inputs, gins)):
                if t is None or g is None:
                    continue
                key = id(t)
                if key in grads:
                    if acc is not None and acc[i] is not None and g is acc[i]:
                        grads[key] = g
                        continue
                    g, have = materialise(g), materialise(grads[key])
                    dense_contribution(have)
                    if info(have).owned:
                        K.axpy_(1.0, g.view(have.shape), have)
                        grads[key] = have
                    else:
                        grads[key] = own(K.add(have, g.view(have.shape)))
                else:
                    grads[key] = g
            if _CAPTURE[0] is not None:
                _CAPTURE[0].maybe_cut(next((g for g in gins if isinstance(g, torch.Tensor)), None) if _DEBUG_LOG[0] is not None else None)
            elif _DEBUG_LOG[0] is not None and _DEBUG_LOG[0].eager_pending >= SegmentedCapture.SIDE_TASKS_PER_SEGMENT:
                _debug_cut(next((g for g in gins if isinstance(g, torch.Tensor)), None))
        return grads


_TAPE: Optional[Tape] = None
_CAPTURE = [None]


def capture() -> Optional["SegmentedCapture"]:
    return _CAPTURE[0]


def set_capture(cap: Optional["SegmentedCapture"]) -> None:
    _CAPTURE[0] = cap

import os as _os

_SIDE = {"stream": None, "enabled": _os.environ.get("BDETR_SIDE_STREAM", "1") != "0", "used": False, "keep": []}


def side_stream() -> Optional["torch.cuda.Stream"]:
    if not _SIDE["enabled"]:
        return None
    if _SIDE["stream"] is None:
        if _os.environ.get("BDETR_SIDE_PRIORITY", "low") == "low":
            import ctypes as _C
            from . import _lib
            for _ in range(int(_os.environ.get("BDETR_SIDE_QUEUE_SKIP", "0"))):
                d = _C.c_void_p()
                _lib.check(_lib.lib().bdetr_low_priority_stream_create(_C.byref(d)), "low_priority_stream_create")
                _SIDE.setdefault("dummies", []).append(d)
            ncand = int(_os.environ.get("BDETR_SIDE_CANDIDATES", "4"))
            if ncand > 1 and not torch.cuda.is_current_stream_capturing():
                _SIDE["placement"] = {"picked": None, "tick_ms": [], "unloaded_ms": None, "good": [], "limit": ncand}
                _SIDE["candidates"] = []
                _more_candidates(1)
                while not _SIDE["placement"]["good"] and len(_SIDE["placement"]["tick_ms"]) < ncand:
                    _more_candidates(1)
                pl = _SIDE["placement"]
                pick = pl["good"][0] if pl["good"] else min(range(len(pl["tick_ms"])), key=lambda c: pl["tick_ms"][c])
                pl["picked"] = pick
                _SIDE["stream"] = _SIDE["candidates"][pick]
                side_stream_release()
            else:
                h = _C.c_void_p()
                _lib.check(_lib.lib().bdetr_low_priority_stream_create(_C.byref(h)), "low_priority_stream_create")
                _SIDE["stream"] = torch.cuda.ExternalStream(h.value, device=device())
        else:
            _SIDE["stream"] = torch.cuda.Stream(device=device())
    return _SIDE["stream"]


SIDE_BAD_RATIO = 3.0


def _more_candidates(n: int) -> None:
    import ctypes as _C
    from . import _lib
    pl = _SIDE["placement"]
    hs, scores, base = (_C.c_void_p * n)(), (_C.c_float * n)(), _C.c_float(0.0)
    _lib.check(_lib.lib().bdetr_side_stream_candidates(_C.c_void_p(torch.cuda.current_stream().cuda_stream), n, 120, 200, hs, scores, _C.byref(base)),
               "side_stream_candidates")
    if pl["unloaded_ms"] is None:
        pl["unloaded_ms"] = round(float(base.value), 3)
    for c in range(n):
        _SIDE["candidates"].append(torch.cuda.ExternalStream(hs[c], device=device()))
        pl["tick_ms"].append(round(float(scores[c]), 3))
        if float(scores[c]) < SIDE_BAD_RATIO * max(pl["unloaded_ms"], 1e-3):
            pl["good"].append(len(pl["tick_ms"]) - 1)


def side_stream_expand() -> list:
    pl = _SIDE.get("placement")
    if pl is None or _SIDE["used"] or torch.cuda.is_current_stream_capturing():
        return [] if pl is None else [c for c in pl["good"] if _SIDE["candidates"][c] is not None]
    while len(pl["tick_ms"]) < pl["limit"]:
        _more_candidates(1)
    return [c for c in pl["good"] if _SIDE["candidates"][c] is not None]


def side_stream_release() -> None:
    from . import _lib
    if _SIDE["used"]:
        raise RuntimeError("side_stream_release: side-stream work is pending (join_side_stream first)")
    for c, st in enumerate(_SIDE.get("candidates", [])):
        if st is not None and st is not _SIDE["stream"]:
            st.synchronize()
            _lib.check(_lib.lib().bdetr_stream_destroy(st.cuda_stream), "stream_destroy")
            _SIDE["candidates"][c] = None


def side_stream_placement() -> Optional[dict]:
    return _SIDE.get("placement")


def side_stream_select(index: int) -> None:
    if _SIDE["used"]:
        raise RuntimeError("side_stream_select: side-stream work is pending (join_side_stream first)")
    if _SIDE["candidates"][index] is None:
        raise RuntimeError(f"side_stream_select: candidate {index} was released")
    _SIDE["stream"] = _SIDE["candidates"][index]
    _SIDE["placement"]["picked"] = index


def set_side_stream_enabled(on: bool) -> None:
    _SIDE["enabled"] = bool(on)


class on_side_stream:

    def __init__(self, *tensors):
        self.tensors = [t for t in tensors if t is not None]
        self.side = side_stream()

    def __enter__(self):
        if self.side is None:
            return self
        ev = torch.cuda.Event()
        ev.record()
        self.side.wait_event(ev)
        _SIDE["keep"].extend(self.tensors)
        self.ctx = torch.cuda.stream(self.side)
        self.ctx.__enter__()
        self.prev_handle = K.set_launch_stream(self.side.cuda_stream if K._LAUNCH_STREAM[0] is not None else None)
        _SIDE["used"] = True
        return self

    def __exit__(self, *exc):
# ... 340 lines not shown
```

### boosted_detr_amd/kernels.py

```python
from __future__ import annotations

import ctypes as C
from dataclasses import dataclass
from typing import Optional, Tuple

import numpy as np
import torch

from . import _lib
from ._lib import BnAffine, BnBwdFuse, ConvDesc, GemmDesc, LossDesc, RowchainBwdDesc, RowchainFwdDesc, check

ACT_NONE, ACT_RELU, ACT_TANH = 0, 1, 2


_LAUNCH_STREAM = [None]


def set_launch_stream(handle: Optional[int]) -> Optional[int]:
    prev = _LAUNCH_STREAM[0]
    _LAUNCH_STREAM[0] = handle
    return prev


GEMM_FP32, GEMM_BF16X3, GEMM_MIXED, GEMM_SPLIT, GEMM_BF16X6 = 0, 1, 2, 3, 4
_GEMM_MODES = {"fp32": GEMM_FP32, "bf16x3": GEMM_BF16X3, "mixed": GEMM_MIXED, "split": GEMM_SPLIT, "bf16x6": GEMM_BF16X6}


def set_gemm_precision(mode) -> int:
    code = _GEMM_MODES.get(mode, mode)
    prev = _lib.lib().bdetr_get_gemm_precision()
    check(_lib.lib().bdetr_set_gemm_precision(int(code)), "set_gemm_precision")
    return prev


def get_gemm_precision() -> str:
    code = _lib.lib().bdetr_get_gemm_precision()
    return next(k for k, v in _GEMM_MODES.items() if v == code)


def demote_split_forward() -> None:
    L = _lib.lib()
    if L.bdetr_get_gemm_precision() == GEMM_SPLIT:
        check(L.bdetr_set_gemm_precision(GEMM_MIXED), "set_gemm_precision")


import os as _os

_DETERMINISTIC = [_os.environ.get("BDETR_DETERMINISTIC", "0") == "1"]


def set_deterministic(on: bool) -> bool:
    prev = _DETERMINISTIC[0]
    _DETERMINISTIC[0] = bool(on)
    return prev


def deterministic() -> bool:
    return _DETERMINISTIC[0]


def _splitk_ws(rows: int, cols: int, sk: int, like: torch.Tensor):
    if not _DETERMINISTIC[0] or sk <= 1:
        return None, 0
    n = int(_lib.lib().bdetr_splitk_workspace_elems(rows, cols, sk))
    return torch.empty(n, dtype=torch.float32, device=like.device), n


class gemm_precision:

    def __init__(self, mode):
        self.mode = mode

    def __enter__(self):
        self.prev = set_gemm_precision(self.mode) if self.mode is not None else None
        return self

    def __exit__(self, *exc):
        if self.prev is not None:
            set_gemm_precision(self.prev)
        return False


def _stream() -> int:
    h = _LAUNCH_STREAM[0]
    return h if h is not None else torch.cuda.current_stream().cuda_stream


def _p(t: Optional[torch.Tensor]) -> Optional[int]:
    if t is None:
        return None
    return t.data_ptr()


def _chk(*tensors, dtype=torch.float32):
    for t in tensors:
        if t is None:
            continue
        if not t.is_cuda:
            raise _lib.BdetrError("kernel operands must live in HBM (cuda tensors); no CPU path exists")
        if t.dtype != dtype:
            raise _lib.BdetrError(f"expected {dtype}, got {t.dtype}")
        if not t.is_contiguous():
            raise _lib.BdetrError("kernel operands must be contiguous")


def empty(*shape, like: torch.Tensor, dtype=torch.float32) -> torch.Tensor:
    return torch.empty(shape, dtype=dtype, device=like.device)


def image_prep(image: torch.Tensor, H: int, W: int) -> torch.Tensor:
    _chk(image)
    B, h, w, c = image.shape
    assert c == 3
    out = empty(B, H, W, 4, like=image)
    check(_lib.lib().bdetr_image_prep(_p(image), B, h, w, _p(out), H, W, _stream()), "image_prep")
    return out


def tokens_prepare(cat_ids: torch.Tensor, att_ids: torch.Tensor, C_: int, A: int):
    _chk(cat_ids, att_ids, dtype=torch.int32)
    if cat_ids.dim() == 3:
        cat_ids = cat_ids[..., 0].contiguous()
    B, M = cat_ids.shape
    slots = att_ids.shape[2] if att_ids.dim() == 3 else 1
    cat = torch.empty_like(cat_ids)
    hot = torch.empty((B, M, A), dtype=torch.float32, device=cat_ids.device)
    check(_lib.lib().bdetr_tokens_prepare(_p(cat_ids), _p(att_ids), B * M, slots, C_, A, _p(cat), _p(hot), _stream()), "tokens_prepare")
    return cat, hot


def augment(image: torch.Tensor, iparams: torch.Tensor, fparams: torch.Tensor, quality: Optional[torch.Tensor] = None) -> torch.Tensor:
    _chk(image, fparams)
    _chk(iparams, dtype=torch.int32)
    B, H, W, c = image.shape
    assert c == 3
    L = _lib.lib()
    out = torch.empty_like(image)
    ws = empty(L.bdetr_augment_ws_floats(B), like=image)
    if quality is None:
        check(L.bdetr_augment(_p(image), _p(out), _p(iparams), _p(fparams), B, H, W, _p(ws), _stream()), "augment")
        return out
    _chk(quality, dtype=torch.int32)
    jws = torch.empty(int(L.bdetr_jpeg_quality_ws_bytes(B, H, W)), dtype=torch.uint8, device=image.device)
    check(L.bdetr_augment_jpeg(_p(image), _p(out), _p(iparams), _p(fparams), _p(quality), B, H, W, _p(ws), _p(jws), _stream()), "augment_jpeg")
    return out


def jpeg_quality(image: torch.Tensor, quality: torch.Tensor) -> torch.Tensor:
    _chk(image)
    _chk(quality, dtype=torch.int32)
    B, H, W, c = image.shape
    assert c == 3 and quality.numel() == B
    L = _lib.lib()
    out = torch.empty_like(image)
    jws = torch.empty(int(L.bdetr_jpeg_quality_ws_bytes(B, H, W)), dtype=torch.uint8, device=image.device)
    check(L.bdetr_jpeg_quality(_p(image), _p(out), _p(quality), B, H, W, _p(jws), _stream()), "jpeg_quality")
    return out


@dataclass(frozen=True)
class ConvGeom:
    N: int
    H: int
# ... 162 lines not shown
    ws = empty(2 * Cc * L.bdetr_bn_bwd_chunks(rows), like=x2d) if pre is None else None
    if even_pixels is not None and pre is None:
        N, H, W = even_pixels
        assert N * H * W == rows
        assert not dout_compact or (dres is None and dout.numel() == N * (H // 2) * (W // 2) * Cc and H % 2 == 0 and W % 2 == 0)
        check(L.bdetr_bn_bwd_p16_even_pixels(_p(dout), _p(out), int(out_p16), _p(x2d), _p(mean), _p(rstd), _p(gamma), _p(beta), int(relu), int(frozen),
                                             _p(dx32), _p(dxb), _p(dgamma), _p(dbeta), _p(dres), _p(ws), N, H, W, Cc, int(dout_compact), _stream()), "bn_bwd_p16_even_pixels")
        return dxb, dx32, dgamma, dbeta, dres
    assert not dout_compact, "a compact dout goes through the even-pixel reduction (even_pixels=(N, H, W), no pre)"
    pg, pgx, pn = pre if pre is not None else (None, None, 0)
    check(L.bdetr_bn_bwd_p16(_p(dout), _p(out), int(out_p16), _p(x2d), _p(mean), _p(rstd), _p(gamma), _p(beta), int(relu), int(frozen), _p(dx32),
                             _p(dxb), _p(dgamma), _p(dbeta), _p(dres), _p(ws), _p(pg), _p(pgx), int(pn), rows, Cc, _stream()), "bn_bwd_p16")
    return dxb, dx32, dgamma, dbeta, dres


def p16_pack_conv_weights_multi(table: torch.Tensor) -> None:
    _chk(table, dtype=torch.int64)
    check(_lib.lib().bdetr_p16_pack_conv_weights_multi(_p(table), table.shape[0], _p(overflow_flag()), _stream()), "p16_pack_conv_weights_multi")


def p16_conv2d_fwd(x_f16, w_f16, bias, g: ConvGeom, act: int = ACT_NONE, want_stats: bool = False):
    _chk(x_f16, w_f16, bias)
    L = _lib.lib()
    d = g.desc()
    y = empty(g.N, g.OH, g.OW, g.K, like=x_f16)
    psum = psq = None
    nparts = 0
    if want_stats:
        nparts = L.bdetr_p16_conv2d_fwd_stat_chunks(C.byref(d))
        if nparts <= 0:
            check(-1, "p16_conv2d_fwd_stat_chunks")
        psum = empty(nparts, g.K, like=x_f16)
        psq = empty(nparts, g.K, like=x_f16)
    check(L.bdetr_p16_conv2d_fwd(_p(x_f16), _p(w_f16), _p(bias), _p(y), C.byref(d), act, _p(psum), _p(psq), _stream()), "p16_conv2d_fwd")
    return y, (psum, psq, nparts)


def p16_conv2d_bwd_data(dy_bf16, wt_bf16, g: ConvGeom, dx: Optional[torch.Tensor] = None, accumulate: bool = False):
    _chk(dy_bf16, wt_bf16, dx)
    d = g.desc()
    if dx is None:
        assert not accumulate
        dx = empty(g.N, g.H, g.W, g.C, like=dy_bf16)
    check(_lib.lib().bdetr_p16_conv2d_bwd_data(_p(dy_bf16), _p(wt_bf16), _p(dx), C.byref(d), int(accumulate), _stream()), "p16_conv2d_bwd_data")
    return dx


def relu_mask_apply_(x: torch.Tensor, relu_mask: torch.Tensor) -> torch.Tensor:
    _chk(x)
    _chk(relu_mask, dtype=torch.int64)
    check(_lib.lib().bdetr_relu_mask_apply(_p(x), _p(relu_mask), x.numel(), _stream()), "relu_mask_apply")
    return x


def p16_conv2d_bwd_data_masked_accum(dy_bf16, wt_bf16, g: ConvGeom, dx: torch.Tensor, relu_mask: torch.Tensor, bn_ctx=None, bn_ctx2=None, old_even=None):
    _chk(dy_bf16, wt_bf16, dx)
    _chk(relu_mask, dtype=torch.int64)
    L = _lib.lib()
    d = g.desc()
    if old_even is not None:
        _chk(old_even)
        assert bn_ctx2 is None and old_even.numel() * 4 == dx.numel() and g.H % 2 == 0 and g.W % 2 == 0

        def launch(fuse):
            check(L.bdetr_p16_conv2d_bwd_data_masked_accum_compact(_p(dy_bf16), _p(wt_bf16), _p(dx), _p(old_even), _p(relu_mask), C.byref(d), fuse, _stream()),
                  "p16_conv2d_bwd_data_masked_accum_compact")
    else:
        def launch(fuse):
            check(L.bdetr_p16_conv2d_bwd_data_masked_accum(_p(dy_bf16), _p(wt_bf16), _p(dx), _p(relu_mask), C.byref(d), fuse, _stream()),
                  "p16_conv2d_bwd_data_masked_accum")
    if bn_ctx is None:
        launch(None)
        return dx
    y_prev, mean, rstd, gamma, beta, bits_prev = bn_ctx
    _chk(y_prev, mean, rstd, gamma, beta)
    _chk(bits_prev, dtype=torch.int64)
    n = L.bdetr_p16_conv2d_bwd_data_stat_chunks(C.byref(d))
    if n <= 0:
        check(-1, "p16_conv2d_bwd_data_stat_chunks")
    pg, pgx = empty(n, g.C, like=dy_bf16), empty(n, g.C, like=dy_bf16)
    f = BnBwdFuse(_p(y_prev), _p(mean), _p(rstd), _p(gamma), _p(beta), 1, _p(pg), _p(pgx), _p(bits_prev))
    pgx2 = None
    if bn_ctx2 is not None:
        y0, mean0, rstd0 = bn_ctx2
        _chk(y0, mean0, rstd0)
        pgx2 = empty(n, g.C, like=dy_bf16)
        f.y2, f.mean2, f.rstd2, f.part_gx2 = _p(y0), _p(mean0), _p(rstd0), _p(pgx2)
    launch(C.byref(f))
    if pgx2 is not None:
        return dx, (pg, pgx, n), (pg, pgx2, n)
    return dx, (pg, pgx, n)


def p16_conv2d_bwd_data_bnstats(dy_bf16, wt_bf16, g: ConvGeom, y_prev, mean, rstd, gamma, beta, relu: bool):
    _chk(dy_bf16, wt_bf16, y_prev, mean, rstd, gamma, beta)
    L = _lib.lib()
    d = g.desc()
    dx = empty(g.N, g.H, g.W, g.C, like=dy_bf16)
    n = L.bdetr_p16_conv2d_bwd_data_stat_chunks(C.byref(d))
    if n <= 0:
        check(-1, "p16_conv2d_bwd_data_stat_chunks")
    pg, pgx = empty(n, g.C, like=dy_bf16), empty(n, g.C, like=dy_bf16)
    f = BnBwdFuse(_p(y_prev), _p(mean), _p(rstd), _p(gamma), _p(beta), int(relu), _p(pg), _p(pgx), None)
    check(L.bdetr_p16_conv2d_bwd_data_bnstats(_p(dy_bf16), _p(wt_bf16), _p(dx), C.byref(d), C.byref(f), _stream()), "p16_conv2d_bwd_data_bnstats")
    return dx, (pg, pgx, n)


def p16_conv2d_bwd_weight(x_bf16, dy_bf16, g: ConvGeom, dw: Optional[torch.Tensor] = None, prezeroed: bool = False, x_f16: bool = False):
    _chk(x_bf16, dy_bf16, dw)
    L = _lib.lib()
    d = g.desc()
    if dw is None:
        dw = empty(g.K, g.R, g.S, g.C, like=x_bf16)
        prezeroed = False
    sk = L.bdetr_p16_conv2d_bwd_weight_splitk(C.byref(d))
    if sk > 1 and not prezeroed:
        check(L.bdetr_zero(_p(dw), dw.numel(), _stream()), "zero")
    ws, n = _splitk_ws(g.K, g.R * g.S * g.C, sk, x_bf16)
    check(L.bdetr_p16_conv2d_bwd_weight_ws(_p(x_bf16), int(x_f16), _p(dy_bf16), _p(dw), C.byref(d), sk, _p(ws), n, _stream()), "p16_conv2d_bwd_weight")
    return dw


def gemm_raw(I, J, R, a, lda, a_rc, b, ldb, b_rc, c, ldc, *, nb0=1, nb1=1, sa=(0, 0), sb=(0, 0), sc=(0, 0),
             bias=None, alpha=1.0, act=ACT_NONE, accumulate=False, splitk=1, grad=False):
    _chk(a, b, c, bias)
    g = GemmDesc(I, J, R, nb0, nb1, _p(a), lda, sa[0], sa[1], int(a_rc), _p(b), ldb, sb[0], sb[1], int(b_rc),
                 _p(c), ldc, sc[0], sc[1], _p(bias), float(alpha), act, int(accumulate), splitk, int(grad))
    ws, n = _splitk_ws(I, J, splitk, c) if ldc == J else (None, 0)
    check(_lib.lib().bdetr_gemm_ws(C.byref(g), _p(ws), n, _stream()), "gemm")
    return c


def gemm_grouped(descs):
    arr = (GemmDesc * len(descs))()
    for k, (I, J, R, a, lda, a_rc, b, ldb, b_rc, c, ldc, bias, act, acc) in enumerate(descs):
        _chk(a, b, c, bias)
        arr[k] = GemmDesc(I, J, R, 1, 1, _p(a), lda, 0, 0, int(a_rc), _p(b), ldb, 0, 0, int(b_rc), _p(c), ldc, 0, 0, _p(bias), 1.0, act,
                          int(acc), 1, int(not (a_rc and b_rc)))
    check(_lib.lib().bdetr_gemm_grouped(arr, len(descs), _stream()), "gemm_grouped")


def linear_fwd_group(xs, ws, biases, act=ACT_NONE):
    K_, O = xs[0].shape[1], ws[0].shape[0]
    ys = [empty(x.shape[0], O, like=x) for x in xs]
    gemm_grouped([(x.shape[0], O, K_, x, K_, True, w, K_, True, y, O, b, act, False) for x, w, b, y in zip(xs, ws, biases, ys)])
    return ys


def linear_bwd_data_group(dys, ws):
    O, K_ = ws[0].shape
    dxs = [empty(dy.shape[0], K_, like=dy) for dy in dys]
    gemm_grouped([(dy.shape[0], K_, O, dy, O, True, w, K_, False, dx, K_, None, ACT_NONE, False) for dy, w, dx in zip(dys, ws, dxs)])
    return dxs


def linear_fwd(x2d, w, bias, act=ACT_NONE):
    M, K = x2d.shape
    O = w.shape[0]
    y = empty(M, O, like=x2d)
    return gemm_raw(M, O, K, x2d, K, True, w, K, True, y, O, bias=bias, act=act)


def linear_bwd_data(dy2d, w, dx=None, accumulate=False):
    M, O = dy2d.shape
    K = w.shape[1]
    if dx is None:
        dx = empty(M, K, like=dy2d)
    return gemm_raw(M, K, O, dy2d, O, True, w, K, False, dx, K, accumulate=accumulate, grad=True)


def _auto_splitk(I, J, R) -> int:
    cus = _lib.lib().bdetr_device_cus()
    tiles = max(1, ((I + 63) // 64) * ((J + 63) // 64))
    sk = max(1, min((2 * cus) // tiles, R // 128))
    return sk


def linear_bwd_weight(dy2d, x2d, dw=None, prezeroed: bool = False):
    M, O = dy2d.shape
    K = x2d.shape[1]
    if dw is None:
        dw = empty(O, K, like=dy2d)
        prezeroed = False
    sk = _auto_splitk(O, K, M)
    if sk > 1 and not prezeroed:
        check(_lib.lib().bdetr_zero(_p(dw), dw.numel(), _stream()), "zero")
    return gemm_raw(O, K, M, dy2d, O, False, x2d, K, False, dw, K, splitk=sk, grad=True)


def linear_bwd_weight_group(dys, xs, dws, prezeroed):
    same = all(dy.shape == dys[0].shape and x.shape == xs[0].shape for dy, x in zip(dys, xs))
    if _DETERMINISTIC[0] or not same or len(dys) == 1 or len(dys) > 4:
        for dy, x, dw, pz in zip(dys, xs, dws, prezeroed):
            linear_bwd_weight(dy, x, dw=dw, prezeroed=pz)
        return dws
    M, O = dys[0].shape
    K_ = xs[0].shape[1]
    L = _lib.lib()
    for dw, pz in zip(dws, prezeroed):
        if not pz:
            check(L.bdetr_zero(_p(dw), dw.numel(), _stream()), "zero")
    tiles = len(dys) * max(1, ((O + 63) // 64) * ((K_ + 63) // 64))
    sk = max(1, min((2 * L.bdetr_device_cus()) // tiles, M // 128))
    arr = (GemmDesc * len(dys))()
    for k, (dy, x, dw) in enumerate(zip(dys, xs, dws)):
        _chk(dy, x, dw)
        arr[k] = GemmDesc(O, K_, M, 1, 1, _p(dy), O, 0, 0, 0, _p(x), K_, 0, 0, 0, _p(dw), K_, 0, 0, None, 1.0, ACT_NONE, 0, sk, 1)
    check(L.bdetr_gemm_grouped(arr, len(dys), _stream()), "gemm_grouped(weight gradients)")
    return dws


def colsum(x2d, out=None, prezeroed=False):
    _chk(x2d, out)
    L = _lib.lib()
    rows, cols = x2d.shape
    if prezeroed and out is not None and not _DETERMINISTIC[0]:
        check(L.bdetr_colsum_accumulate(_p(x2d), rows, cols, _p(out), _stream()), "colsum_accumulate")
        return out
    if out is None:
        out = empty(cols, like=x2d)
    ws = empty(L.bdetr_colsum_chunks(rows) * cols, like=x2d)
    check(L.bdetr_colsum(_p(x2d), rows, cols, _p(out), _p(ws), _stream()), "colsum")
    return out


def colsum_group(xs, outs):
    _chk(*xs, *outs)
    n, cols = len(xs), xs[0].shape[1]
    assert 1 <= n <= 4 and all(x.dim() == 2 and x.shape[1] == cols for x in xs) and all(o.numel() == cols for o in outs)
    PA, LA = C.c_void_p * n, C.c_int64 * n
    check(_lib.lib().bdetr_colsum_accumulate_group(PA(*[x.data_ptr() for x in xs]), LA(*[x.shape[0] for x in xs]), cols, PA(*[o.data_ptr() for o in outs]), n,
                                                   _stream()), "colsum_accumulate_group")


def colstats(x2d):
    _chk(x2d)
    L = _lib.lib()
    rows, Cc = x2d.shape
    n = L.bdetr_bn_bwd_chunks(rows)
    psum, psq = empty(n, Cc, like=x2d), empty(n, Cc, like=x2d)
    check(L.bdetr_colstats(_p(x2d), rows, Cc, _p(psum), _p(psq), _stream()), "colstats")
    return psum, psq, n


def bn_stats(rows, Cc, parts, eps, momentum, bessel, moving_mean, moving_var, like):
    psum, psq, n = parts
    L = _lib.lib()
    mean, rstd = empty(Cc, like=like), empty(Cc, like=like)
    fold = L.bdetr_bn_stats_fold_rows()
    ws = empty(2 * fold * Cc, like=like) if n > 4 * fold else None
    check(L.bdetr_bn_stats(None, rows, Cc, _p(psum), _p(psq), n, eps, momentum, int(bessel), _p(mean), _p(rstd),
                           _p(moving_mean), _p(moving_var), _p(ws), _p(overflow_flag()) if _GUARD_ACTIVE[0] else None, _stream()), "bn_stats")
    return mean, rstd


def bn_stats_frozen(moving_mean, moving_var, eps):
    _chk(moving_mean, moving_var)
    Cc = moving_mean.numel()
    mean, rstd = empty(Cc, like=moving_mean), empty(Cc, like=moving_mean)
    check(_lib.lib().bdetr_bn_stats_frozen(_p(moving_mean), _p(moving_var), Cc, eps, _p(mean), _p(rstd), _stream()), "bn_stats_frozen")
    return mean, rstd


def bn_apply(x2d, mean, rstd, gamma, beta, residual=None, relu=False, out=None):
    _chk(x2d, mean, rstd, gamma, beta, residual, out)
    rows, Cc = x2d.shape
    if out is None:
        out = torch.empty_like(x2d)
    check(_lib.lib().bdetr_bn_apply(_p(x2d), _p(mean), _p(rstd), _p(gamma), _p(beta), _p(residual), int(relu), _p(out), rows, Cc, _stream()),
          "bn_apply")
    return out


def bn_bwd(dout, out, x2d, mean, rstd, gamma, relu, frozen, want_residual_grad=False, dgamma=None, dbeta=None, beta=None):
    _chk(dout, out, x2d, mean, rstd, gamma, dgamma, dbeta)
    L = _lib.lib()
    rows, Cc = x2d.shape
    dx = torch.empty_like(x2d)
    dgamma = empty(Cc, like=x2d) if dgamma is None else dgamma
    dbeta = empty(Cc, like=x2d) if dbeta is None else dbeta
    dres = torch.empty_like(x2d) if want_residual_grad else None
    ws = empty(2 * Cc * L.bdetr_bn_bwd_chunks(rows), like=x2d)
    check(L.bdetr_bn_bwd(_p(dout), _p(out), _p(x2d), _p(mean), _p(rstd), _p(gamma), _p(beta), int(relu), int(frozen), _p(dx), _p(dgamma), _p(dbeta),
                         _p(dres), _p(ws), rows, Cc, _stream()), "bn_bwd")
    return dx, dgamma, dbeta, dres


def bn_rows_stats(x2d, groups: int, eps):
    _chk(x2d)
    rows, Cc = x2d.shape
    assert rows % groups == 0, (rows, groups)
    mean, rstd, var = empty(groups, Cc, like=x2d), empty(groups, Cc, like=x2d), empty(groups, Cc, like=x2d)
    check(_lib.lib().bdetr_bn_rows_stats(_p(x2d), groups, rows // groups, Cc, eps, _p(mean), _p(rstd), _p(var),
                                         _p(overflow_flag()) if _GUARD_ACTIVE[0] else None, _stream()), "bn_rows_stats")
    return mean, rstd, var


def bn_rows_apply(x2d, groups: int, mean, rstd, gamma, beta, var=None, momentum=0.0, moving_mean=None, moving_var=None):
    _chk(x2d, mean, rstd, gamma, beta, var, moving_mean, moving_var)
    rows, Cc = x2d.shape
    assert rows % groups == 0, (rows, groups)
    grouped = mean.dim() == 2
    out = torch.empty_like(x2d)
    check(_lib.lib().bdetr_bn_rows_apply(_p(x2d), _p(mean), _p(rstd), _p(gamma), _p(beta), _p(out), groups, rows // groups, Cc, int(grouped), _p(var),
                                         momentum, _p(moving_mean), _p(moving_var),
                                         _p(overflow_flag()) if (_GUARD_ACTIVE[0] and moving_mean is not None) else None, _stream()), "bn_rows_apply")
# ... 865 lines not shown
```

### boosted_detr_amd/ops.py

```python
from __future__ import annotations

import math
import os
import weakref
from typing import Optional

import numpy as np
import torch

from . import kernels as K
from . import _lib
from .engine import WEIGHTS_VERSION, Variable, capture, current_tape, dense_contribution, info, materialise, own, side_task, tag

_dropout_site = [0]
_dropout_seed_dev = [None]


def dropout_seed_tensor() -> torch.Tensor:
    if _dropout_seed_dev[0] is None:
        _dropout_seed_dev[0] = torch.full((1,), 0x5EED, dtype=torch.int64, device="cuda")
    return _dropout_seed_dev[0]


def set_dropout_seed(seed: int, write: bool = True) -> None:
# ... 401 lines not shown
        if s2:
            tag(dx).even_pixels = imap
    return own(dx)


def conv_act(x: torch.Tensor, w: Variable, b: Variable, stride: int, pad: int, act: int) -> torch.Tensor:
    N, H, W, Cin = x.shape
    Kout, R, S, _ = w.value.shape
    g = K.ConvGeom(N, H, W, Cin, Kout, R, S, stride, pad)
    y, _ = K.conv2d_fwd(x, w.value, b.value, g, act)

    def backward(g_out):
        g_out = g_out.contiguous()
        if act == K.ACT_TANH:
            dpre = K.tanh_bwd(y, g_out)
        elif act == K.ACT_RELU:
            dpre = K.relu_bwd(y, g_out)
        else:
            dpre = g_out
        _param_grads_task(w, b, lambda dw, pz: K.conv2d_bwd_weight(x, dpre, g, dw=dw, prezeroed=pz), _2d(dpre), x, dpre)
        return (own(K.conv2d_bwd_data(dpre, w.value, g)),)

    _rec([y], [x], backward)
    return y


def batchnorm(x: torch.Tensor, bn: BNState, training: bool, bessel: bool) -> torch.Tensor:
    x2d = _2d(x)
    rows, Cc = x2d.shape
    out2d, mean, rstd = _bn_forward(x2d, rows, Cc, None, bn, training, bessel, None, False)
    out = out2d.view(x.shape)

    def backward(g_out):
        dx, _ = _bn_backward(_2d(g_out.contiguous()), None, x2d, mean, rstd, bn, False, not training, False)
        return (own(dx.view(x.shape)),)

    _rec([out], [x], backward)
    return out


def batchnorm_rows(x: torch.Tensor, bn: BNState, training: bool, groups: int) -> torch.Tensor:
    x2d = _2d(x)
    g, b = bn.gamma.value, bn.beta.value
    if training:
        mean, rstd, var = K.bn_rows_stats(x2d, groups, bn.eps)
        out2d = K.bn_rows_apply(x2d, groups, mean, rstd, g, b, var, bn.momentum, bn.moving_mean.value, bn.moving_var.value)
    else:
        K.demote_split_forward()
        mean, rstd = K.bn_stats_frozen(bn.moving_mean.value, bn.moving_var.value, bn.eps)
        out2d = K.bn_rows_apply(x2d, groups, mean, rstd, g, b)
    out = out2d.view(x.shape)

    def backward(g_out):
        sg, sb = GradSink(bn.gamma), GradSink(bn.beta)
        dx, _, _ = K.bn_rows_bwd(_2d(g_out.contiguous()), x2d, groups, mean, rstd, bn.gamma.value, not training, dgamma=sg.buf, dbeta=sb.buf)
        sg.commit()
        sb.commit()
        return (own(dx.view(x.shape)),)

    _rec([out], [x], backward)
    return out


def stack_rows(xs) -> torch.Tensor:
    L, B = len(xs), xs[0].shape[0]
    out = torch.empty((L * B,) + tuple(xs[0].shape[1:]), dtype=xs[0].dtype, device=xs[0].device)
    for l, x in enumerate(xs):
        K.copy_cols(x.contiguous(), x.shape[-1], out[l * B:(l + 1) * B], 0)

    def backward(g):
        g, mine = g.contiguous(), info(g).owned
        return tuple(own(g[l * B:(l + 1) * B]) if mine else g[l * B:(l + 1) * B] for l in range(L))

    _rec([out], list(xs), backward)
    return out


def maxpool(x: torch.Tensor) -> torch.Tensor:
    y = K.maxpool_fwd(x)
    _rec([y], [x], lambda g: (own(K.maxpool_bwd(x, y, g.contiguous())),))
    return y


STEM_FUSE = os.environ.get("BDETR_STEM_FUSE", "1") != "0"
STEM_S2D = os.environ.get("BDETR_STEM_S2D", "1") != "0"


def conv_bn_relu_maxpool(x: torch.Tensor, w: Variable, b: Variable, bn: BNState, stride: int, pad: int, training: bool,
                         bn_batch_stats: bool) -> torch.Tensor:
    N, H, W, Cin = x.shape
    Kout, R, S, _ = w.value.shape
    if not (STEM_FUSE and training and bn_batch_stats and _p16_active() and Kout % 8 == 0):
        return maxpool(conv_bn(x, w, b, bn, stride, pad, True, training=training, bn_batch_stats=bn_batch_stats, x_needs_grad=False))
    g = K.ConvGeom(N, H, W, Cin, Kout, R, S, stride, pad)
    x32 = as_fp32(x)
    y, parts = K.conv2d_fwd(x32, w.value, b.value, g, K.ACT_NONE, want_stats=True)
    if parts is None or parts[0] is None:
        parts = K.colstats(_2d(y))
    mean, rstd = K.bn_stats(g.M, Kout, parts, bn.eps, bn.momentum, True, bn.moving_mean.value, bn.moving_var.value, like=y)
    _, out, tap = K.stem_pool_fwd(y, mean, rstd, bn.gamma.value, bn.beta.value)
    attach_packed(out, out.detach(), p16_only=True)

    def backward(g_out):
        sg, sb = GradSink(bn.gamma), GradSink(bn.beta)
        s2d = (STEM_S2D and w.needs_grad and (R, S, stride, pad, Cin) == (7, 7, 2, 3, 4) and H % 2 == 0 and W % 2 == 0 and Kout % 64 == 0
               and K.get_gemm_precision() in ("split", "mixed") and not K.deterministic())
        dy, _, _ = K.stem_pool_bwd(materialise(g_out).contiguous(), tap, y, mean, rstd, bn.gamma.value, bn.beta.value, dgamma=sg.buf, dbeta=sb.buf,
                                   dy_p16=s2d)
        sg.commit()
        sb.commit()
        if s2d:
            _param_grads_task(w, b, lambda dw, pz: K.stem_bwd_weight_s2d(x32, dy, dw), None, x32, dy)
        else:
            _param_grads_task(w, b, lambda dw, pz: K.conv2d_bwd_weight(x32, dy, g, dw=dw, prezeroed=pz), None, x32, dy)
        return (None,)

    _rec([out], [x], backward)
    return out


def dense(x: torch.Tensor, w: Variable, b: Variable, act: int = K.ACT_NONE) -> torch.Tensor:
    x2d = _2d(x)
    y2d = K.linear_fwd(x2d, w.value, b.value, act)
    y = y2d.view(*x.shape[:-1], w.value.shape[0])

    def backward(g_out, acc=None):
        g2d = _2d(g_out.contiguous())
        if act == K.ACT_RELU:
            g2d = K.relu_bwd(y2d, g2d)
        elif act == K.ACT_TANH:
            g2d = K.tanh_bwd(y2d, g2d)
        _param_grads_task(w, b, lambda dw, pz: K.linear_bwd_weight(g2d, x2d, dw=dw, prezeroed=pz), g2d, x2d, g2d)
        have = acc[0] if acc is not None else None
        if have is not None and have.is_contiguous() and have.shape == x.shape:
            K.linear_bwd_data(g2d, w.value, dx=_2d(materialise(have)), accumulate=True)
            dense_contribution(have)
            return (have,)
        return (own(K.linear_bwd_data(g2d, w.value).view(x.shape)),)

    backward.wants_acc = True
    _rec([y], [x], backward)
    return y


def dense_group(xs, ws, bs):
    x2 = [_2d(x) for x in xs]
    aligned = all(t.data_ptr() % 16 == 0 for t in x2) and x2[0].shape[1] % 4 == 0 and ws[0].value.shape[0] % 4 == 0
    same = all(w.value.shape == ws[0].value.shape for w in ws)
    if not (aligned and same) or len(xs) > 4:
        return [dense(x, w, b) for x, w, b in zip(xs, ws, bs)]
    y2 = K.linear_fwd_group(x2, [w.value for w in ws], [b.value for b in bs])
    ys = [y.view(*x.shape[:-1], y.shape[1]) for y, x in zip(y2, xs)]

    def backward(*gs):
        g2 = [_2d(g.contiguous()) for g in gs]

        def param_grads():
            groups = {}
            for g, x, w in zip(g2, x2, ws):
                if w.needs_grad:
                    groups.setdefault((tuple(g.shape), tuple(x.shape)), []).append((g, x, GradSink(w)))
            for members in groups.values():
                K.linear_bwd_weight_group([m[0] for m in members], [m[1] for m in members], [m[2].buf for m in members], [m[2].mode == "direct" for m in members])
                for m in members:
                    m[2].commit()
            sinks = [(g, GradSink(b)) for g, b in zip(g2, bs) if b.needs_grad]
            direct = [(g, s) for g, s in sinks if s.mode == "direct"]
            if len(direct) > 1 and not K.deterministic() and all(g.shape[1] == direct[0][0].shape[1] for g, _ in direct):
                K.colsum_group([g for g, _ in direct], [s.buf for _, s in direct])
                for _, s in direct:
                    s.commit()
                sinks = [(g, s) for g, s in sinks if s.mode != "direct"]
            for g, s in sinks:
                K.colsum(g, out=s.buf, prezeroed=s.mode == "direct")
                s.commit()
        if any(w.needs_grad or b.needs_grad for w, b in zip(ws, bs)):
            side_task(param_grads, *x2, *g2)
        dxs = K.linear_bwd_data_group(g2, [w.value for w in ws])
        return tuple(own(dx.view(x.shape)) for dx, x in zip(dxs, xs))

    _rec(ys, list(xs), backward)
    return ys


def add(a: torch.Tensor, b: torch.Tensor) -> torch.Tensor:
    out = K.add(a, b)
    _rec([out], [a, b], lambda g: (g, g))
    return out


def _param_or_tensor_grad(p, fn):
    if isinstance(p, Variable):
        if p.needs_grad:
            s = GradSink(p)
            fn(s.buf)
            s.commit()
        return None
    return fn(None)


def add_bcast(x: torch.Tensor, row) -> torch.Tensor:
    rv = row.value if isinstance(row, Variable) else row
    out = K.add_bcast_rows(x, rv)
    n = rv.numel()

    def backward(g):
        g = g.contiguous()
        grow = _param_or_tensor_grad(row, lambda out_: K.sum_over_batch(g, n, out=out_))
        return g, (grow.view(rv.shape) if grow is not None else None)

    _rec([out], [x, None if isinstance(row, Variable) else row], backward)
    return out


def tile_batch(row: Variable, B: int) -> torch.Tensor:
    rv = row.value
    zeros = torch.empty((B,) + tuple(rv.shape), dtype=rv.dtype, device=rv.device)
    K.zero_(zeros)
    out = K.add_bcast_rows(zeros, rv)
    n = rv.numel()
    from . import engine as _engine
    if _engine._DEBUG_LOG[0] is not None:
        _engine._DEBUG_LOG[0].emit("L", out)

    def backward(g):
        g = g.contiguous()
        _param_or_tensor_grad(row, lambda out_: K.sum_over_batch(g, n, out=out_))
        return ()

    _rec([out], [], backward)
    return out


def reshape(x: torch.Tensor, shape) -> torch.Tensor:
    y = x.view(shape)

    def backward(g):
        r = g.contiguous().view(x.shape)
        return (own(r) if info(g).owned else r,)

    _rec([y], [x], backward)
    return y


def attention_core(Q: torch.Tensor, Kt: torch.Tensor, V: torch.Tensor, heads: int) -> torch.Tensor:
    B, q, D = Q.shape
    kk = Kt.shape[1]
    d = D // heads
    scale = 1.0 / math.sqrt(float(d))
    if d == 32 and FUSED_ATTENTION[0]:
        O, lse = K.attention_fwd(Q, Kt, V, heads, scale)

        def backward_fused(gO):
            dQ, dK, dV = K.attention_bwd(Q, Kt, V, O, gO.contiguous(), lse, heads, scale)
            return own(dQ), own(dK), own(dV)

        _rec([O], [Q, Kt, V], backward_fused)
        return O
    S = K.empty(B, heads, q, kk, like=Q)
    K.gemm_raw(q, kk, d, Q, D, True, Kt, D, True, S, kk, nb0=B, nb1=heads, sa=(q * D, d), sb=(kk * D, d), sc=(heads * q * kk, q * kk))
    P = K.softmax_rows_fwd(S.view(-1, kk), scale, out=S.view(-1, kk)).view(B, heads, q, kk)
    O = K.empty(B, heads, q, d, like=Q)
    K.gemm_raw(q, d, kk, P, kk, True, V, D, False, O, d, nb0=B, nb1=heads, sa=(heads * q * kk, q * kk), sb=(kk * D, d), sc=(heads * q * d, q * d))

    def backward(gO):
        gO = gO.contiguous()
        sP, sO = (heads * q * kk, q * kk), (heads * q * d, q * d)
        dP = K.empty(B, heads, q, kk, like=Q)
        K.gemm_raw(q, kk, d, gO, d, True, V, D, True, dP, kk, nb0=B, nb1=heads, sa=sO, sb=(kk * D, d), sc=sP, grad=True)
        dV = K.empty(B, kk, D, like=Q)
        K.gemm_raw(kk, d, q, P, kk, False, gO, d, False, dV, D, nb0=B, nb1=heads, sa=sP, sb=sO, sc=(kk * D, d), grad=True)
        dS = K.softmax_rows_bwd(P.view(-1, kk), dP.view(-1, kk), scale, out=dP.view(-1, kk)).view(B, heads, q, kk)
        dQ = K.empty(B, q, D, like=Q)
        K.gemm_raw(q, d, kk, dS, kk, True, Kt, D, False, dQ, D, nb0=B, nb1=heads, sa=sP, sb=(kk * D, d), sc=(q * D, d), grad=True)
        dK = K.empty(B, kk, D, like=Q)
        K.gemm_raw(kk, d, q, dS, kk, False, Q, D, False, dK, D, nb0=B, nb1=heads, sa=sP, sb=(q * D, d), sc=(kk * D, d), grad=True)
        return own(dQ), own(dK), own(dV)

    _rec([O], [Q, Kt, V], backward)
    return O


FUSED_ATTENTION = [True]


def add_dropout_layernorm(x: torch.Tensor, y: torch.Tensor, gamma: Variable, beta: Variable, eps: float, rate: float,
                          training: bool) -> torch.Tensor:
    r = rate if training else 0.0
    seed = _next_dropout_seed() if r > 0.0 else 0
    x2d, y2d = _2d(x), _2d(y)
    base = dropout_seed_tensor() if r > 0.0 else None
    out2d, mean, rstd = K.add_dropout_layernorm_fwd(x2d, y2d, gamma.value, beta.value, eps, r, seed, seed_base=base)
    out = out2d.view(x.shape)

    def backward(g_out):
        sg, sb = GradSink(gamma), GradSink(beta)
        dx, dy, _, _ = K.add_dropout_layernorm_bwd(_2d(g_out.contiguous()), x2d, y2d, gamma.value, mean, rstd, r, seed,
                                                   dgamma=sg.buf, dbeta=sb.buf, seed_base=base)
        sg.commit()
        sb.commit()
        return own(dx.view(x.shape)), own(dy.view(y.shape))

    _rec([out], [x, y], backward)
    return out


ROWCHAIN = [os.environ.get("BDETR_ROWCHAIN", "1") != "0"]


def rowchain_active(width: int) -> bool:
    return ROWCHAIN[0] and width == K.ROWCHAIN_WIDTH and K.get_gemm_precision() == "split"


def _rowchain_pack_buffers(v: torch.Tensor):
    n = int(_lib.lib().bdetr_rowchain_pack_elems())
    return torch.empty(n, dtype=torch.float32, device=v.device), torch.empty(n, dtype=torch.float32, device=v.device)


_RC_PACKED = _PackCache(_rowchain_pack_buffers, lambda v, f, t: [v.data_ptr(), f.data_ptr(), t.data_ptr()],
                        K.rowchain_pack_weights)


def attention_out_chain(ctx: torch.Tensor, resid: torch.Tensor, out_proj, ln1, ffn, eps: float, rate: float, training: bool) -> torch.Tensor:
    r = rate if training else 0.0
    seed1 = _next_dropout_seed() if r > 0.0 else 0
    seed2 = _next_dropout_seed() if (r > 0.0 and ffn is not None) else 0
    base = dropout_seed_tensor() if r > 0.0 else None
    ctx2d, res2d = _2d(ctx.contiguous()), _2d(resid.contiguous())
    Wo, bo = out_proj
    g1, b1 = ln1
    ws = [Wo] + ([ffn[0], ffn[2]] if ffn is not None else [])
    bs = [bo] + ([ffn[1], ffn[3]] if ffn is not None else [])
    packs = [_RC_PACKED.get(w) for w in ws]
# ... 73 lines not shown
```

### include/bdetr.h

```cpp
#ifndef BDETR_H
#define BDETR_H
#include <stdint.h>
#ifdef __cplusplus
extern "C" {
#endif

#define BDETR_ABI_VERSION 8

int         bdetr_abi_version(void);
const char* bdetr_last_error(void);
int         bdetr_device_cus(void);

int         bdetr_low_priority_stream_create(void** stream_out);
int         bdetr_stream_priority_range(int* least, int* greatest);
int         bdetr_side_stream_candidates(void* main_stream, int ncand, int loads, int ticks, void** streams_out, float* scores_ms, float* unloaded_ms);
int         bdetr_stream_destroy(void* stream);

enum { BDETR_GEMM_FP32 = 0, BDETR_GEMM_BF16X3 = 1, BDETR_GEMM_MIXED = 2, BDETR_GEMM_SPLIT = 3, BDETR_GEMM_BF16X6 = 4 };
int         bdetr_set_gemm_precision(int mode);
int         bdetr_get_gemm_precision(void);

int bdetr_prof_enable(int on);
int bdetr_prof_read(double* total_ms, int64_t* launches, double* flops);
int bdetr_prof_read_arith(int arith, double* total_ms, int64_t* launches, double* flops);
int bdetr_prof_dump(const char* path);

enum { BDETR_ACT_NONE = 0, BDETR_ACT_RELU = 1, BDETR_ACT_TANH = 2 };

int bdetr_image_prep(const float* in, int B, int h, int w, float* out, int H, int W, void* stream);

int bdetr_tokens_prepare(const int* cat_ids, const int* att_ids, int64_t rows, int slots, int C, int A,
                         int* cat_out, float* att_hot, void* stream);

int bdetr_augment_ws_floats(int B);
int bdetr_augment(const float* in, float* out, const int32_t* iparams, const float* fparams,
                  int B, int H, int W, float* ws, void* stream);
int64_t bdetr_jpeg_quality_ws_bytes(int B, int H, int W);
int bdetr_jpeg_quality(const float* in, float* out, const int32_t* quality, int B, int H, int W, void* ws, void* stream);
int bdetr_augment_jpeg(const float* in, float* out, const int32_t* iparams, const float* fparams, const int32_t* quality,
                       int B, int H, int W, float* ws, void* jpeg_ws, void* stream);

typedef struct {
    int N, H, W, C;
    int K, R, S;
    int stride, pad;
    int OH, OW;
} bdetr_conv_desc;

int bdetr_conv2d_fwd(const float* x, const float* w, const float* bias, float* y,
                     const bdetr_conv_desc* d, int act, float* stat_sum, float* stat_sq, void* stream);
int bdetr_conv2d_fwd_stat_chunks(const bdetr_conv_desc* d);
int bdetr_conv2d_bwd_data(const float* dy, const float* w, float* dx,
                          const bdetr_conv_desc* d, int accumulate, void* stream);
int bdetr_conv2d_bwd_weight(const float* x, const float* dy, float* dw,
                            const bdetr_conv_desc* d, int splitk, void* stream);
int bdetr_conv2d_bwd_weight_splitk(const bdetr_conv_desc* d);
int bdetr_conv2d_bwd_weight_ws(const float* x, const float* dy, float* dw,
                               const bdetr_conv_desc* d, int splitk, float* ws, int64_t ws_elems, void* stream);
int64_t bdetr_splitk_workspace_elems(int64_t I, int64_t J, int splitk);

typedef struct { const float* mean; const float* rstd; const float* gamma; const float* beta; } bdetr_bn_affine;
int bdetr_bn_apply_p16(const float* x, const float* mean, const float* rstd, const float* gamma,
                       const float* beta, const void* residual, int residual_p16, const bdetr_bn_affine* residual_bn, int relu, float* out32,
                       void* out_f16, void* out_bf16, uint64_t* relu_mask, int* overflow_flag, int64_t rows, int C,
                       void* stream);
int bdetr_bn_bwd_p16(const float* dout, const void* out, int out_p16, const float* x, const float* mean,
                     const float* rstd, const float* gamma, const float* beta, int relu, int frozen,
                     float* dx32, void* dx_bf16, float* dgamma, float* dbeta, float* dresidual,
                     float* ws, const float* pre_g, const float* pre_gx, int pre_n, int64_t rows, int C, void* stream);
int bdetr_bn_bwd_p16_even_pixels(const float* dout, const void* out, int out_p16, const float* x, const float* mean,
                                 const float* rstd, const float* gamma, const float* beta, int relu, int frozen,
                                 float* dx32, void* dx_bf16, float* dgamma, float* dbeta, float* dresidual,
                                 float* ws, int N, int H, int W, int C,
                                 int dout_compact , void* stream);
int bdetr_p16_supported(const bdetr_conv_desc* d);
int bdetr_p16_pack(const float* x, int64_t n, void* f16_out, void* bf16_out, int* overflow_flag, void* stream);
int bdetr_p16_unpack(const void* p, int is_f16, int64_t n, float* out, void* stream);
int bdetr_p16_pack_conv_weights(const float* w, int K, int R, int S, int C, void* w_f16, void* wt_bf16,
                                int* overflow_flag, void* stream);
int bdetr_p16_pack_conv_weights_multi(const int64_t* table, int ntensors, int* overflow_flag, void* stream);
int bdetr_p16_conv2d_fwd_stat_chunks(const bdetr_conv_desc* d);
int bdetr_p16_conv2d_fwd(const void* x_f16, const void* w_f16, const float* bias, float* y,
                         const bdetr_conv_desc* d, int act, float* stat_sum, float* stat_sq, void* stream);
int bdetr_p16_conv2d_bwd_data(const void* dy_bf16, const void* wt_bf16, float* dx,
                              const bdetr_conv_desc* d, int accumulate, void* stream);
typedef struct {
    const float* y; const float* mean; const float* rstd; const float* gamma; const float* beta; int relu;
    float* part_g; float* part_gx;
    const uint64_t* relu_mask;
    const float* y2; const float* mean2; const float* rstd2; float* part_gx2;
} bdetr_bn_bwd_fuse;
int bdetr_p16_conv2d_bwd_data_stat_chunks(const bdetr_conv_desc* d);
int bdetr_relu_mask_apply(float* x, const uint64_t* relu_mask, int64_t n, void* stream);
int bdetr_p16_conv2d_bwd_data_masked_accum(const void* dy_bf16, const void* wt_bf16, float* dx, const uint64_t* relu_mask,
                                           const bdetr_conv_desc* d, const bdetr_bn_bwd_fuse* bn , void* stream);
int bdetr_p16_conv2d_bwd_data_masked_accum_compact(const void* dy_bf16, const void* wt_bf16, float* dx, const float* old_even,
                                                   const uint64_t* relu_mask, const bdetr_conv_desc* d, const bdetr_bn_bwd_fuse* bn, void* stream);
int bdetr_p16_conv2d_bwd_data_bnstats(const void* dy_bf16, const void* wt_bf16, float* dx,
                                      const bdetr_conv_desc* d, const bdetr_bn_bwd_fuse* bn, void* stream);
int bdetr_p16_conv2d_bwd_weight_splitk(const bdetr_conv_desc* d);
int bdetr_p16_conv2d_bwd_weight(const void* x_bf16, const void* dy_bf16, float* dw,
                                const bdetr_conv_desc* d, int splitk, void* stream);
int bdetr_p16_conv2d_bwd_weight_xf16(const void* x_f16, const void* dy_bf16, float* dw,
                                     const bdetr_conv_desc* d, int splitk, void* stream);
int bdetr_p16_conv2d_bwd_weight_ws(const void* x, int x_is_f16, const void* dy_bf16, float* dw,
                                   const bdetr_conv_desc* d, int splitk, float* ws, int64_t ws_elems, void* stream);

typedef struct {
    int I, J, R;
    int nb0, nb1;
    const float* a; int64_t lda, sa0, sa1; int a_rcontig;
    const float* b; int64_t ldb, sb0, sb1; int b_rcontig;
    float*       c; int64_t ldc, sc0, sc1;
    const float* bias; float alpha; int act; int accumulate; int splitk;
    int grad;
} bdetr_gemm_desc;
int bdetr_gemm(const bdetr_gemm_desc* g, void* stream);
int bdetr_gemm_ws(const bdetr_gemm_desc* g, float* ws, int64_t ws_elems, void* stream);
int bdetr_gemm_grouped(const bdetr_gemm_desc* g, int n, void* stream);

int bdetr_colsum_chunks(int64_t rows);
int bdetr_colsum(const float* x, int64_t rows, int cols, float* out, float* ws, void* stream);
int bdetr_colsum_accumulate(const float* x, int64_t rows, int cols, float* out, void* stream);
int bdetr_colsum_accumulate_group(const float* const* xs, const int64_t* rows, int cols, float* const* outs, int n, void* stream);

int bdetr_colstats(const float* x, int64_t rows, int C, float* part_sum, float* part_sq, void* stream);
int bdetr_bn_stats(const float* x, int64_t rows, int C, const float* part_sum, const float* part_sq,
                   int nparts, float eps, float momentum, int bessel,
                   float* mean, float* rstd, float* moving_mean, float* moving_var, float* fold_ws,
                   int* guard_flag, void* stream);
int bdetr_flag_nonfinite(const float* x, int64_t n, int* flag, void* stream);
int bdetr_flag_snapshot(const int* flag, int* ordinal, int* host_ring, int ring_len, void* stream);
int bdetr_debug_checksum(const float* x, int64_t n, uint64_t* scratch, uint64_t* log, int* cursor, int cap, uint64_t tag, void* stream);
int bdetr_graph_node_census(void* graph, int64_t* counts, int ncounts);
int bdetr_bn_stats_fold_rows(void);
int bdetr_bn_stats_frozen(const float* moving_mean, const float* moving_var, int C, float eps,
                          float* mean, float* rstd, void* stream);
int bdetr_bn_apply(const float* x, const float* mean, const float* rstd, const float* gamma,
                   const float* beta, const float* residual, int relu, float* out,
                   int64_t rows, int C, void* stream);
int bdetr_bn_bwd_chunks(int64_t rows);
int bdetr_bn_bwd(const float* dout, const float* out, const float* x, const float* mean,
                 const float* rstd, const float* gamma, const float* beta, int relu, int frozen,
                 float* dx, float* dgamma, float* dbeta, float* dresidual,
                 float* ws, int64_t rows, int C, void* stream);

int bdetr_bn_rows_stats(const float* x, int G, int64_t R, int C, float eps, float* mean, float* rstd, float* var,
                        int* guard_flag, void* stream);
int bdetr_bn_rows_apply(const float* x, const float* mean, const float* rstd, const float* gamma, const float* beta, float* out,
                        int G, int64_t R, int C, int grouped_stats, const float* var, float momentum, float* moving_mean,
                        float* moving_var, const int* guard_flag, void* stream);
int bdetr_bn_rows_bwd(const float* dout, const float* x, const float* mean, const float* rstd, const float* gamma,
                      int grouped_stats, int frozen, float* dx, float* dgamma, float* dbeta, float* ws, int G, int64_t R, int C,
                      void* stream);

int bdetr_maxpool3x3s2_fwd(const float* x, float* y, int N, int H, int W, int C, int OH, int OW, void* stream);
int bdetr_maxpool3x3s2_bwd(const float* x, const float* y, const float* dy, float* dx,
                           int N, int H, int W, int C, int OH, int OW, void* stream);

int bdetr_stem_pool_bwd_chunks(int64_t rows);
int bdetr_stem_pool_fwd(const float* y, const float* mean, const float* rstd, const float* gamma, const float* beta,
                        int N, int H, int W, int C, float* out32, void* out_f16, uint8_t* tap, int* overflow_flag, void* stream);
int bdetr_stem_pool_bwd(const float* dpool, const uint8_t* tap, const float* y, const float* mean, const float* rstd, const float* gamma,
                        const float* beta, int N, int H, int W, int C, float* dy, int dy_p16 , float* dgamma, float* dbeta, float* ws, void* stream);
int bdetr_p16_s2d_pack_bf16(const float* x, int N, int H, int W, void* out_bf16, void* stream);
int bdetr_p16_stem_bwd_weight(const void* x2_bf16, const void* dy_bf16, float* dw2, int N, int H2, int W2, int K, void* stream);
int bdetr_p16_s2d_unpack_dw(const float* dw2, float* dw, int K, void* stream);

int bdetr_softmax_rows_fwd(const float* s, float* p, int64_t rows, int cols, float scale, void* stream);
int bdetr_softmax_rows_bwd(const float* p, const float* dp, float* ds, int64_t rows, int cols, float scale, void* stream);

int bdetr_attention_head_dim(void);
int bdetr_attention_fwd(const float* q, const float* k, const float* v, float* o, float* lse,
                        int B, int h, int nq, int nk, float scale, void* stream);
int bdetr_attention_bwd(const float* q, const float* k, const float* v, const float* o, const float* d_o,
                        const float* lse, float* dq, float* dk, float* dv, float* dvec_ws,
                        int B, int h, int nq, int nk, float scale, void* stream);

int bdetr_add_dropout_layernorm_fwd(const float* x, const float* y, const float* gamma, const float* beta,
                                    float* out, float* mean, float* rstd, int64_t rows, int D,
                                    float eps, float rate, uint64_t seed, const uint64_t* seed_base, void* stream);
int bdetr_ln_bwd_chunks(int64_t rows);
int bdetr_add_dropout_layernorm_bwd(const float* dout, const float* x, const float* y, const float* gamma,
                                    const float* mean, const float* rstd, float* dx, float* dy,
                                    float* dgamma, float* dbeta, float* ws, int64_t rows, int D,
                                    float rate, uint64_t seed, const uint64_t* seed_base, int accumulate_dx, void* stream);

typedef struct {
    int64_t M; int nstages; float eps, rate;
    const float* ctx; const float* resid;
    const void* w[3];
    const float* bias[3];
    const float* g1; const float* b1; const float* g2; const float* b2;
    float* pre1; float* x1; float* mean1; float* rstd1;
    float* h; float* pre2; float* x2; float* mean2; float* rstd2;
    uint64_t seed1, seed2; const uint64_t* seed_base;
} bdetr_rowchain_fwd_desc;
int bdetr_rowchain_fwd(const bdetr_rowchain_fwd_desc* d, void* stream);
typedef struct {
    int64_t M; int nstages; float rate;
    const float* dout;
    const float* pre2; const float* mean2; const float* rstd2; const float* g2;
    const float* h;
    const float* pre1; const float* mean1; const float* rstd1; const float* g1;
    const void* wt[3];
    float* G2; float* G1; float* G0;
    float* dresid; float* dctx;
    float* partials;
    uint64_t seed1, seed2; const uint64_t* seed_base;
} bdetr_rowchain_bwd_desc;
int bdetr_rowchain_bwd(const bdetr_rowchain_bwd_desc* d, void* stream);
int bdetr_rowchain_reduce(const float* partials, int nparts, float* const* dst7, const int* accumulate7, void* stream);
int bdetr_rowchain_width(void);
int64_t bdetr_rowchain_pack_elems(void);
int bdetr_rowchain_partial_rows(int64_t M);
int bdetr_rowchain_pack_weights(const int64_t* table, int n, int* overflow_flag, void* stream);

int bdetr_resize_bilinear_nhwc(const float* in, int B, int h, int w, int C, float* out, int H, int W, void* stream);
int bdetr_layernorm_act_fwd(const float* x, int64_t rows, int C, int ldx, const float* gamma, const float* beta,
                            float eps, float slope, float* out, int ldo, void* stream);
int bdetr_copy_cols(const float* src, int64_t rows, int C, int ld_src, float* dst, int ld_dst, int dst_col0, void* stream);
int bdetr_nhwc_to_nchw(const float* in, int B, int P, int C, int ld_in, float* out, void* stream);

int bdetr_layernorm_act_bwd_chunks(int64_t rows);
int bdetr_layernorm_act_bwd(const float* x, int64_t rows, int C, int ldx, const float* gamma, const float* beta, float eps, float slope,
                            const float* dout, int ldo, float* dx, float* part_g, float* part_b, float* dgamma, float* dbeta, void* stream);
int bdetr_resize_bilinear_nhwc_bwd(const float* dout, int B, int H, int W, int C, float* din, int h, int w, void* stream);
int bdetr_nchw_to_nhwc(const float* in, int B, int P, int C, float* out, int ld_out, void* stream);
int bdetr_conv_weight_pack(const float* kernel, const float* bias, int R, int S, int Cin, int K, int transpose, int Cp, int Kp,
                           float* w, float* b, void* stream);
int bdetr_conv_weight_unpack(const float* dw, const float* db, int R, int S, int Cin, int K, int transpose, int Cp,
                             float* dkernel, float* dbias, void* stream);
int bdetr_mask_loss(const float* logits, const float* masks, const int* match, const int* num_objects, int B, int M, int N, int P,
                    float alpha, float gamma, float mask_weight, float loss_scale, float* row_loss, float* loss, float* dlogits, void* stream);

int bdetr_softmax_lastdim_fwd(const float* logits, float* p, int64_t rows, int cols, void* stream);
int bdetr_softmax_lastdim_bwd(const float* p, const float* dp, float* dlogits, int64_t rows, int cols, void* stream);
int bdetr_sigmoid_fwd(const float* x, float* y, int64_t n, void* stream);
int bdetr_sigmoid_bwd(const float* y, const float* dy, float* dx, int64_t n, void* stream);
int bdetr_boxsigmoid_fwd(const float* x, float* y, int64_t n, void* stream);
int bdetr_boxsigmoid_bwd(const float* y, const float* dy, float* dx, int64_t n, void* stream);

int bdetr_zero(float* p, int64_t n, void* stream);
int bdetr_add(const float* a, const float* b, float* out, int64_t n, void* stream);
int bdetr_add_bcast_rows(const float* a, const float* row, float* out, int64_t rows, int64_t rowlen, void* stream);
int bdetr_sum_over_batch(const float* x, float* out, int64_t batch, int64_t n, int accumulate, void* stream);
int bdetr_tanh_bwd(const float* y, const float* dy, float* dx, int64_t n, void* stream);
int bdetr_relu_bwd(const float* y, const float* dy, float* dx, int64_t n, void* stream);
int bdetr_axpy(float alpha, const float* x, float* y, int64_t n, void* stream);

typedef struct {
    int B, M, N, C, A;
    float category_weight, attribute_weight, box_weight, exist_weight;
} bdetr_loss_desc;
int bdetr_cost_matrix(const bdetr_loss_desc* d, const float* cat_pred, const float* att_pred,
                      const float* box_pred, const int32_t* cat_ids, const float* att_hot,
                      const float* bbox, const int32_t* num_objects, float* cost, float* cost_cat,
                      float* cost_att, float* cost_box, void* stream);
int bdetr_lsa(const float* cost, const int32_t* num_objects, int B, int M, int N,
              int32_t* match, void* stream);
int bdetr_set_loss(const bdetr_loss_desc* d, const float* cat_pred, const float* att_pred,
                   const float* box_pred, const int32_t* cat_ids, const float* att_hot,
                   const float* bbox, const int32_t* num_objects, const int32_t* match,
                   float* losses, float* d_cat, float* d_att, float* d_box, float loss_scale,
                   void* stream);
int bdetr_cost_matrix_tiled(const bdetr_loss_desc* d, int period, const float* cat_pred, const float* att_pred,
                            const float* box_pred, const int32_t* cat_ids, const float* att_hot,
                            const float* bbox, const int32_t* num_objects, float* cost, void* stream);
int bdetr_lsa_tiled(const float* cost, const int32_t* num_objects, int B, int period, int M, int N,
                    int32_t* match, void* stream);
int bdetr_set_loss_tiled(const bdetr_loss_desc* d, int period, const float* cat_pred, const float* att_pred,
                         const float* box_pred, const int32_t* cat_ids, const float* att_hot,
// ... 72 lines not shown
```

Baseline: 657.3.

## Fuse fan-in linear backward-data products and gradient accumulation into one multi-GEMM kernel

Moves the igemm kernel body into an include file and builds a multi-member variant. That variant sums several dy·W products for the same input slot in registers and adds the existing gradient before writing. The grouped linear backward now groups inputs that share a tensor (such as the same x feeding q/k/v projections) and calls this fused kernel. This replaces separate GEMMs plus axpy/add passes, removing extra kernel launches and global read/write traffic. The cost is more autograd plumbing (a 'have' argument passed to backward functions) and an extra set of accumulator registers, which may reduce occupancy.

```diff
diff --git a/boosted_detr_amd/_lib.py b/boosted_detr_amd/_lib.py
--- a/boosted_detr_amd/_lib.py
+++ b/boosted_detr_amd/_lib.py
@@ -26,6 +26,10 @@
         ("bias", C.c_void_p), ("alpha", C.c_float), ("act", C.c_int), ("accumulate", C.c_int), ("splitk", C.c_int),
         ("grad", C.c_int),
     ]
+
+
+class BwdDataMember(C.Structure):
+    _fields_ = [("dy", C.c_void_p), ("w", C.c_void_p), ("dx", C.c_void_p), ("old", C.c_void_p), ("rows", C.c_int)]
 
 
 class BnAffine(C.Structure):
@@ -116,6 +120,8 @@
     "bdetr_conv2d_bwd_weight_ws": (I, [P, P, P, C.POINTER(ConvDesc), I, P, L, P]),
     "bdetr_p16_conv2d_bwd_weight_ws": (I, [P, I, P, P, C.POINTER(ConvDesc), I, P, L, P]),
     "bdetr_gemm_grouped": (I, [C.POINTER(GemmDesc), I, P]),
+    "bdetr_linear_bwd_data_multi_ok": (I, [I, I, I, I]),
+    "bdetr_linear_bwd_data_multi": (I, [C.POINTER(BwdDataMember), I, I, I, P]),
     "bdetr_colsum_chunks": (I, [L]),
     "bdetr_colsum": (I, [P, L, I, P, P, P]),
     "bdetr_colsum_accumulate": (I, [P, L, I, P, P]),
diff --git a/boosted_detr_amd/build.py b/boosted_detr_amd/build.py
--- a/boosted_detr_amd/build.py
+++ b/boosted_detr_amd/build.py
@@ -34,6 +34,8 @@
 
 def build(force: bool = False, verbose: bool = True) -> Path:
     deps = [CSRC / s for s in SOURCES] + [CSRC / "common.h", CSRC / "gemm_common.h", CSRC / "p16.h", CSRC.parent.parent / "include" / "bdetr.h"]
+    includes = {"igemm.hip": [CSRC / "igemm_kernel.inc"]}
+    deps += [p for ps in includes.values() for p in ps]
     stamp = CSRC / "_obj" / "stamp"
     dig = _digest(deps) + "|" + " ".join(COMMON_FLAGS)
     if not force and LIB.exists() and stamp.exists() and stamp.read_text() == dig:
@@ -47,7 +49,7 @@
         obj = OBJ_DIR / (src.rsplit(".", 1)[0] + ".o")
         flags = COMMON_FLAGS + PER_FILE_FLAGS.get(src, [])
         ostamp = OBJ_DIR / (src + ".stamp")
-        odig = _digest([CSRC / src] + headers) + "|" + " ".join(flags)
+        odig = _digest([CSRC / src] + includes.get(src, []) + headers) + "|" + " ".join(flags)
         if not force and obj.exists() and ostamp.exists() and ostamp.read_text() == odig:
             return obj
         cmd = [hipcc, *flags, "-x", "hip", "-c", str(CSRC / src), "-o", str(obj)]
diff --git a/boosted_detr_amd/csrc/igemm.hip b/boosted_detr_amd/csrc/igemm.hip
--- a/boosted_detr_amd/csrc/igemm.hip
+++ b/boosted_detr_amd/csrc/igemm.hip
@@ -148,320 +148,27 @@
     static constexpr int LDS_LD = RC ? BK + RPAD : BX;
 };
 
-template <int BM, int BN, int WM, int WN, class LA, bool A_RC, class LB, bool B_RC, int ARITH>
-__global__ __launch_bounds__(NTHREADS, 2)
-void igemm_kernel(typename LA::Op opa, typename LB::Op opb, GemmParams g)
-{
-    static_assert(WM * WN == 4, "4 waves per workgroup");
-    constexpr int WTM = BM / WM, WTN = BN / WN;
-    constexpr int TM = WTM / 32, TN = WTN / 32;
-    static_assert(TM >= 1 && TN >= 1, "wave tile must hold at least one 32x32 MFMA tile");
-    using GA = TileGeom<BM, A_RC>;
-    using GB = TileGeom<BN, B_RC>;
-    static_assert(GA::NV >= 1 && GB::NV >= 1, "tile too small for 256 threads");
-
-    constexpr bool SPLIT = ARITH != AR_FP32;
-    constexpr bool X6 = ARITH == AR_BF16X6;
-    constexpr int SLDK = X6 ? SLD3 : SLD;
-    constexpr int A_FLOATS = SPLIT ? BM * SLDK : GA::LDS_FLOATS;
-    constexpr int B_FLOATS = SPLIT ? BN * SLDK : GB::LDS_FLOATS;
-    constexpr int STAGE_FLOATS = A_FLOATS + B_FLOATS;
-    static_assert(!SPLIT || ((A_RC || GA::NV % 2 == 0) && (B_RC || GB::NV % 2 == 0)), "split mode transposes k-pairs");
-    __shared__ __attribute__((aligned(16))) float lds[2 * STAGE_FLOATS];
-
-    const int tid = threadIdx.x;
-    const int lane = tid & 63;
-    const int wave = tid >> 6;
-    const int wm = wave / WN, wn = wave % WN;
-    const int li = lane & 31, lh = lane >> 5;
-
-    const int nwg_ = g.tiles_i * g.tiles_j;
-    const bool sk_ = g.ngroups == 0 && g.splitk > 1;
-    const int lin_ = sk_ ? xcd_tile(blockIdx.z * nwg_ + blockIdx.x, nwg_ * gridDim.z) : xcd_tile(blockIdx.x, nwg_);
-    const int zz_ = sk_ ? lin_ / nwg_ : blockIdx.z;
-    const int wg = sk_ ? lin_ - zz_ * nwg_ : lin_;
-    const int tile_i = wg / g.tiles_j, tile_j = wg - tile_i * g.tiles_j;
-    const int i0 = tile_i * BM, j0 = tile_j * BN;
-
-    int b0 = 0, b1 = 0, r_begin = 0, r_end = g.R;
-    if (g.ngroups > 0) {
-        const int z = g.splitk > 1 ? (int)blockIdx.z / g.splitk : (int)blockIdx.z;
-        if (g.splitk > 1) {
-            r_begin = ((int)blockIdx.z - z * g.splitk) * g.r_chunk;
-            r_end = min(g.R, r_begin + g.r_chunk);
-        }
-#define BDETR_PICK(arr) (z == 0 ? g.arr[0] : z == 1 ? g.arr[1] : z == 2 ? g.arr[2] : g.arr[3])
-        g.I = BDETR_PICK(gI); g.c = BDETR_PICK(gc); g.bias = BDETR_PICK(gbias);
-        const float* pa = BDETR_PICK(ga);
-        const float* pb = BDETR_PICK(gb);
-#undef BDETR_PICK
-        if (i0 >= g.I) return;
-        LA::regroup(opa, pa, g.I, A_RC);
-        LB::regroup(opb, pb, -1, B_RC);
-    } else if (g.splitk > 1) {
-        r_begin = zz_ * g.r_chunk;
-        r_end = min(g.R, r_begin + g.r_chunk);
-    } else {
-        b0 = blockIdx.z / g.nb1; b1 = blockIdx.z - b0 * g.nb1;
-    }
-    const __amdgpu_buffer_rsrc_t rsA = make_rsrc(LA::batch_base(opa, b0, b1));
-    const __amdgpu_buffer_rsrc_t rsB = make_rsrc(LB::batch_base(opb, b0, b1));
-    const int a_rows = A_RC ? opa.rows : min(opa.rows, r_end), a_cols = A_RC ? min(opa.cols, r_end) : opa.cols;
-    const int b_rows = B_RC ? opb.rows : min(opb.rows, r_end), b_cols = B_RC ? min(opb.cols, r_end) : opb.cols;
-
-    typename LA::Ctx ctxA[GA::NV];
-    typename LB::Ctx ctxB[GB::NV];
-    int colA[GA::NV], colB[GB::NV], ldsoffA[GA::NV], ldsoffB[GB::NV], rowA[GA::NV], rowB[GB::NV];
-    auto stage_geom = [&](int p, int vpr, int bx, bool rc, int lds_ld, int& row, int& col, int& ldsoff) {
-        if (!SPLIT) {
-            const int v = tid + NTHREADS * p;
-            const int rt = v / vpr, c4 = v - rt * vpr;
-            row = rt; col = 4 * c4; ldsoff = rt * lds_ld + 4 * c4;
-        } else if (rc) {
-            const int v = tid + NTHREADS * p;
-            const int q = v / vpr, c4 = v - q * vpr;
-            const int rt = (q & ~15) | ((q & 3) << 2) | ((q >> 2) & 3);
-            row = rt; col = 4 * c4;
-            ldsoff = rt * SLDK * 32 + ((((c4 >> 1) ^ ((rt >> 4) & 7)) << 2) | ((c4 & 1) << 1));
-        } else {
-            const int u = tid + NTHREADS * (p >> 1);
-            const int kp = u / (bx / 4), c4 = u - kp * (bx / 4);
-            row = 2 * kp + (p & 1); col = 4 * c4;
-            ldsoff = (4 * c4) * SLDK * 32 + ((((kp >> 2) ^ ((c4 >> 2) & 7)) << 2) | (kp & 3));
-        }
-    };
-#pragma unroll
-    for (int p = 0; p < GA::NV; ++p) {
-        stage_geom(p, GA::VPR, BM, A_RC, GA::LDS_LD, rowA[p], colA[p], ldsoffA[p]);
-        if (A_RC) ctxA[p] = LA::row_ctx(opa, i0 + rowA[p], a_rows);
-    }
-#pragma unroll
-    for (int p = 0; p < GB::NV; ++p) {
-        stage_geom(p, GB::VPR, BN, B_RC, GB::LDS_LD, rowB[p], colB[p], ldsoffB[p]);
-        if (B_RC) ctxB[p] = LB::row_ctx(opb, j0 + rowB[p], b_rows);
-    }
-
-    f32x4 stA0[GA::NV], stB0[GB::NV], stA1[GA::NV], stB1[GB::NV];
-    auto load_stage = [&](int r0, f32x4 (&ra)[GA::NV], f32x4 (&rb)[GB::NV]) {
-#pragma unroll
-        for (int p = 0; p < GA::NV; ++p) {
-            if (A_RC) ra[p] = LA::load(rsA, opa, ctxA[p], r0 + colA[p], a_cols);
-            else      ra[p] = LA::load(rsA, opa, LA::row_ctx(opa, r0 + rowA[p], a_rows), i0 + colA[p], a_cols);
-        }
-#pragma unroll
-        for (int p = 0; p < GB::NV; ++p) {
-            if (B_RC) rb[p] = LB::load(rsB, opb, ctxB[p], r0 + colB[p], b_cols);
-            else      rb[p] = LB::load(rsB, opb, LB::row_ctx(opb, r0 + rowB[p], b_rows), j0 + colB[p], b_cols);
-        }
-    };
-    auto write_split = [&](unsigned* base, bool rc, auto nv_c, const f32x4* r, const int* ldsoff) {
-        constexpr int nv = decltype(nv_c)::value;
-        if (rc) {
-#pragma unroll
-            for (int p = 0; p < nv; ++p) {
-                unsigned* row = base + (ldsoff[p] >> 5);
-                const int w = ldsoff[p] & 31;
-                if constexpr (X6) {
-                    unsigned h0, m0, l0, h1, m1, l1;
-                    split3(r[p][0], r[p][1], h0, m0, l0);
-                    split3(r[p][2], r[p][3], h1, m1, l1);
-                    u32x2 hi, mid, lo;
-                    hi[0] = h0; hi[1] = h1; mid[0] = m0; mid[1] = m1; lo[0] = l0; lo[1] = l1;
-                    *reinterpret_cast<u32x2*>(row + w) = hi;
-                    *reinterpret_cast<u32x2*>(row + (w ^ 16)) = mid;
-                    *reinterpret_cast<u32x2*>(row + 32 + (w & 15)) = lo;
-                } else {
-                    unsigned h0, l0, h1, l1;
-                    split2<ARITH>(r[p][0], r[p][1], h0, l0);
-                    split2<ARITH>(r[p][2], r[p][3], h1, l1);
-                    u32x2 hi, lo;
-                    hi[0] = h0; hi[1] = h1; lo[0] = l0; lo[1] = l1;
-                    *reinterpret_cast<u32x2*>(row + w) = hi;
-                    *reinterpret_cast<u32x2*>(row + (w ^ 16)) = lo;
-                }
-            }
-        } else {
-#pragma unroll
-            for (int p = 0; p + 1 < nv; p += 2) {
-                unsigned* row = base + (ldsoff[p] >> 5);
-                const int w = ldsoff[p] & 31;
-#pragma unroll
-                for (int e = 0; e < 4; ++e) {
-                    if constexpr (X6) {
-                        unsigned hi, mid, lo;
-                        split3(r[p][e], r[p + 1][e], hi, mid, lo);
-                        row[e * SLDK + w] = hi;
-                        row[e * SLDK + (w ^ 16)] = mid;
-                        row[e * SLDK + 32 + (w & 15)] = lo;
-                    } else {
-                        unsigned hi, lo;
-                        split2<ARITH>(r[p][e], r[p + 1][e], hi, lo);
-                        row[e * SLDK + w] = hi;
-                        row[e * SLDK + (w ^ 16)] = lo;
-                    }
-                }
-            }
-        }
-    };
-    auto write_stage = [&](int buf, const f32x4 (&ra)[GA::NV], const f32x4 (&rb)[GB::NV]) {
-        if (SPLIT) {
-            unsigned* st = reinterpret_cast<unsigned*>(lds + buf * STAGE_FLOATS);
-            write_split(st, A_RC, std::integral_constant<int, GA::NV>{}, ra, ldsoffA);
-            write_split(st + A_FLOATS, B_RC, std::integral_constant<int, GB::NV>{}, rb, ldsoffB);
-            return;
-        }
-#pragma unroll
-        for (int p = 0; p < GA::NV; ++p) *reinterpret_cast<f32x4*>(lds + buf * STAGE_FLOATS + ldsoffA[p]) = ra[p];
-#pragma unroll
-        for (int p = 0; p < GB::NV; ++p) *reinterpret_cast<f32x4*>(lds + buf * STAGE_FLOATS + GA::LDS_FLOATS + ldsoffB[p]) = rb[p];
-    };
-
-    constexpr int TM2 = ARITH == AR_FP16X3 ? TM : 1, TN2 = ARITH == AR_FP16X3 ? TN : 1;
-    f32x16 acc[TM][TN], acc2[TM2][TN2];
-#pragma unroll
-    for (int a = 0; a < TM; ++a)
-#pragma unroll
-        for (int b = 0; b < TN; ++b)
-#pragma unroll
-            for (int e = 0; e < 16; ++e) acc[a][b][e] = 0.f;
-#pragma unroll
-    for (int a = 0; a < TM2; ++a)
-#pragma unroll
-        for (int b = 0; b < TN2; ++b)
-#pragma unroll
-            for (int e = 0; e < 16; ++e) acc2[a][b][e] = 0.f;
-
-    auto compute = [&](int buf) {
-        if (SPLIT) {
-            const unsigned* qA = reinterpret_cast<const unsigned*>(lds + buf * STAGE_FLOATS);
-            const unsigned* qB = qA + A_FLOATS;
-#pragma unroll
-            for (int ks = 0; ks < BK / 16; ++ks) {
-                u32x4 ah[TM], al[TM], bh[TN], bl[TN];
-                u32x4 a3[X6 ? TM : 1], b3[X6 ? TN : 1];
-#pragma unroll
-                for (int a = 0; a < TM; ++a) {
-                    const int xb = wm * WTM + a * 32 + li;
-                    const int w = ((ks * 2 + lh) ^ ((xb >> 4) & 7)) << 2;
-                    ah[a] = *reinterpret_cast<const u32x4*>(qA + xb * SLDK + w);
-                    al[a] = *reinterpret_cast<const u32x4*>(qA + xb * SLDK + (w ^ 16));
-                    if constexpr (X6) a3[a] = *reinterpret_cast<const u32x4*>(qA + xb * SLDK + 32 + (w & 15));
-                }
-#pragma unroll
-                for (int b = 0; b < TN; ++b) {
-                    const int xb = wn * WTN + b * 32 + li;
-                    const int w = ((ks * 2 + lh) ^ ((xb >> 4) & 7)) << 2;
-                    bh[b] = *reinterpret_cast<const u32x4*>(qB + xb * SLDK + w);
-                    bl[b] = *reinterpret_cast<const u32x4*>(qB + xb * SLDK + (w ^ 16));
-                    if constexpr (X6) b3[b] = *reinterpret_cast<const u32x4*>(qB + xb * SLDK + 32 + (w & 15));
-                }
-#pragma unroll
-                for (int a = 0; a < TM; ++a)
-#pragma unroll
-                    for (int b = 0; b < TN; ++b) {
-                        if constexpr (X6) {
-#define BF8(v) __builtin_bit_cast(bf16x8, v)
-                            acc[a][b] = __builtin_amdgcn_mfma_f32_32x32x16_bf16(BF8(a3[a]), BF8(bh[b]), acc[a][b], 0, 0, 0);
-                            acc[a][b] = __builtin_amdgcn_mfma_f32_32x32x16_bf16(BF8(ah[a]), BF8(b3[b]), acc[a][b], 0, 0, 0);
-                            acc[a][b] = __builtin_amdgcn_mfma_f32_32x32x16_bf16(BF8(al[a]), BF8(bl[b]), acc[a][b], 0, 0, 0);
-                            acc[a][b] = __builtin_amdgcn_mfma_f32_32x32x16_bf16(BF8(al[a]), BF8(bh[b]), acc[a][b], 0, 0, 0);
-                            acc[a][b] = __builtin_amdgcn_mfma_f32_32x32x16_bf16(BF8(ah[a]), BF8(bl[b]), acc[a][b], 0, 0, 0);
-                            acc[a][b] = __builtin_amdgcn_mfma_f32_32x32x16_bf16(BF8(ah[a]), BF8(bh[b]), acc[a][b], 0, 0, 0);
-#undef BF8
-                        } else if constexpr (ARITH == AR_BF16X3) {
-#define BF8(v) __builtin_bit_cast(bf16x8, v)
-                            acc[a][b] = __builtin_amdgcn_mfma_f32_32x32x16_bf16(BF8(al[a]), BF8(bh[b]), acc[a][b], 0, 0, 0);
-                            acc[a][b] = __builtin_amdgcn_mfma_f32_32x32x16_bf16(BF8(ah[a]), BF8(bl[b]), acc[a][b], 0, 0, 0);
-                            acc[a][b] = __builtin_amdgcn_mfma_f32_32x32x16_bf16(BF8(ah[a]), BF8(bh[b]), acc[a][b], 0, 0, 0);
-#undef BF8
-                        } else if constexpr (ARITH == AR_FP16X3) {
-#define H8(v) __builtin_bit_cast(f16x8, v)
-                            acc2[a][b] = __builtin_amdgcn_mfma_f32_32x32x16_f16(H8(al[a]), H8(bh[b]), acc2[a][b], 0, 0, 0);
-                            acc2[a][b] = __builtin_amdgcn_mfma_f32_32x32x16_f16(H8(ah[a]), H8(bl[b]), acc2[a][b], 0, 0, 0);
-                            acc[a][b] = __builtin_amdgcn_mfma_f32_32x32x16_f16(H8(ah[a]), H8(bh[b]), acc[a][b], 0, 0, 0);
-#undef H8
-                        }
-                    }
-            }
-            return;
-        }
-        const float* sA = lds + buf * STAGE_FLOATS;
-        const float* sB = sA + GA::LDS_FLOATS;
-#pragma unroll
-        for (int kb = 0; kb < BK / 8; ++kb) {
-            f32x4 fa[TM], fb[TN];
-#pragma unroll
-            for (int a = 0; a < TM; ++a) {
-                const int xb = wm * WTM + a * 32 + li;
-                if (A_RC) {
-                    fa[a] = *reinterpret_cast<const f32x4*>(sA + xb * GA::LDS_LD + kb * 8 + 4 * lh);
-                } else {
-#pragma unroll
-                    for (int e = 0; e < 4; ++e) fa[a][e] = sA[(kb * 8 + 4 * lh + e) * GA::LDS_LD + xb];
-                }
-            }
-#pragma unroll
-            for (int b = 0; b < TN; ++b) {
-                const int xb = wn * WTN + b * 32 + li;
-                if (B_RC) {
-                    fb[b] = *reinterpret_cast<const f32x4*>(sB + xb * GB::LDS_LD + kb * 8 + 4 * lh);
-                } else {
-#pragma unroll
-                    for (int e = 0; e < 4; ++e) fb[b][e] = sB[(kb * 8 + 4 * lh + e) * GB::LDS_LD + xb];
-                }
-            }
-#pragma unroll
-            for (int e = 0; e < 4; ++e)
-#pragma unroll
-                for (int a = 0; a < TM; ++a)
-#pragma unroll
-                    for (int b = 0; b < TN; ++b)
-                        acc[a][b] = __builtin_amdgcn_mfma_f32_32x32x2f32(fa[a][e], fb[b][e], acc[a][b], 0, 0, 0);
-        }
-    };
-
-    const int nk = (r_end - r_begin + BK - 1) / BK;
-    constexpr bool PF1 = SPLIT && BM * BN >= 128 * 128;
-    if constexpr (PF1) {
-        if (nk > 0) { load_stage(r_begin, stA0, stB0); write_stage(0, stA0, stB0); }
-        __syncthreads();
-        for (int kt = 0; kt < nk; ++kt) {
-            if (kt + 1 < nk) load_stage(r_begin + (kt + 1) * BK, stA0, stB0);
-            compute(kt & 1);
-            if (kt + 1 < nk) write_stage((kt + 1) & 1, stA0, stB0);
-            __syncthreads();
-        }
-    } else {
-    if (nk > 0) {
-        load_stage(r_begin, stA0, stB0);
-        if (nk > 1) load_stage(r_begin + BK, stA1, stB1);
-        write_stage(0, stA0, stB0);
-    }
-    __syncthreads();
-
-    for (int kt = 0; kt < nk; kt += 2) {
-        if (kt + 2 < nk) load_stage(r_begin + (kt + 2) * BK, stA0, stB0);
-        compute(0);
-        if (kt + 1 < nk) write_stage(1, stA1, stB1);
-        __syncthreads();
-        if (kt + 1 >= nk) break;
-        if (kt + 3 < nk) load_stage(r_begin + (kt + 3) * BK, stA1, stB1);
-        compute(1);
-        if (kt + 2 < nk) write_stage(0, stA0, stB0);
-        __syncthreads();
-    }
-    }
-
-    if constexpr (ARITH == AR_FP16X3) {
-#pragma unroll
-        for (int a = 0; a < TM; ++a)
-#pragma unroll
-            for (int b = 0; b < TN; ++b)
-#pragma unroll
-                for (int e = 0; e < 16; ++e) acc[a][b][e] += acc2[a][b][e] * (1.f / LO_SCALE);
-    }
-    gemm_epilogue<BM, BN, WM, WN, NTHREADS, 2 * STAGE_FLOATS>(acc, g, lds, tile_i, i0, j0, g.c + (int64_t)(sk_ ? zz_ : b0) * g.sc0 + (int64_t)b1 * g.sc1);
-}
+constexpr int MULTI_MAX_OUT = 4, MULTI_MAX_SRC = 16;
+struct MultiSrc {
+    int nout;
+    int I[MULTI_MAX_OUT], first[MULTI_MAX_OUT], count[MULTI_MAX_OUT];
+    float* c[MULTI_MAX_OUT]; const float* old[MULTI_MAX_OUT];
+    const float* a[MULTI_MAX_SRC]; const float* b[MULTI_MAX_SRC];
+};
+#define IGEMM_KERNEL igemm_kernel
+#define IGEMM_MULTI 0
+#define IGEMM_MULTI_PARAM
+#include "igemm_kernel.inc"
+#undef IGEMM_KERNEL
+#undef IGEMM_MULTI
+#undef IGEMM_MULTI_PARAM
+#define IGEMM_KERNEL igemm_multi_kernel
+#define IGEMM_MULTI 1
+#define IGEMM_MULTI_PARAM , MultiSrc ms
+#include "igemm_kernel.inc"
+#undef IGEMM_KERNEL
+#undef IGEMM_MULTI
+#undef IGEMM_MULTI_PARAM
 
 struct TileChoice { int bm, bn; };
 
@@ -731,6 +438,79 @@
     return launch_any<DenseLoader<4>, false, DenseLoader<4>, true>(a, b, g, zdim, st, sp, true);
 }
 
+namespace {
+bool multi_tile_ok(int maxI, int J, int zdim, int arith) {
+    if (J <= 32) return false;
+    const TileChoice t = choose_tile(maxI, J, zdim, false, arith != AR_FP32);
+    return t.bm == 64 && t.bn == 64;
+}
+
+template <int ARITH>
+int launch_multi(const DenseOp& a, const DenseOp& b, GemmParams g, const MultiSrc& ms, int nsrc, hipStream_t st) {
+    using L = DenseLoader<4>;
+    g.tiles_i = (int)cdiv64(g.I, 64);
+    g.tiles_j = (int)cdiv64(g.J, 64);
+    g.vec_store = 1;
+    dim3 grid(g.tiles_i * g.tiles_j, 1, ms.nout);
+    const bool prof = g_prof_on;
+    if (prof) prof_begin(st, 2.0 * (double)g.I * (double)g.J * (double)g.R * (double)nsrc, g.I, g.J, g.R, ms.nout, 64, 64, ARITH * 10000 + 100);
+    hipLaunchKernelGGL((igemm_multi_kernel<64, 64, 2, 2, L, true, L, false, ARITH>), grid, dim3(NTHREADS), 0, st, a, b, g, ms);
+    if (prof) prof_end(st);
+    return bdetr_launch_status("igemm_multi");
+}
+}
+
+extern "C" int bdetr_linear_bwd_data_multi_ok(int max_rows, int out_features, int in_features, int outputs) {
+    const int arith = use_split(true);
+    return out_features > 0 && in_features % 4 == 0 && out_features % 4 == 0 && outputs >= 1 && outputs <= MULTI_MAX_OUT &&
+           arith != AR_FP16X3 && multi_tile_ok(max_rows, in_features, outputs, arith) ? 1 : 0;
+}
+
+extern "C" int bdetr_linear_bwd_data_multi(const bdetr_bwd_data_member* m, int n, int out_features, int in_features, void* stream) {
+    BDETR_CHECK_ARG(m && n >= 1 && n <= MULTI_MAX_SRC, "bdetr_linear_bwd_data_multi: 1..%d members", MULTI_MAX_SRC);
+    const int O = out_features, J = in_features;
+    BDETR_CHECK_ARG(O > 0 && J > 0 && O % 4 == 0 && J % 4 == 0, "bdetr_linear_bwd_data_multi: widths must be positive multiples of 4 (got %d -> %d)", J, O);
+    MultiSrc ms{};
+    int maxI = 0;
+    for (int k = 0; k < n; ++k) {
+        const bdetr_bwd_data_member& e = m[k];
+        BDETR_CHECK_ARG(e.dy && e.w && e.dx && e.rows > 0, "bdetr_linear_bwd_data_multi: null pointer / empty member %d", k);
+        BDETR_CHECK_ARG(aligned16(e.dy) && aligned16(e.w) && aligned16(e.dx) && (e.old == nullptr || aligned16(e.old)),
+                        "bdetr_linear_bwd_data_multi: member %d is not 16-byte aligned", k);
+        BDETR_CHECK_ARG(span_ok((int64_t)e.rows * O) && span_ok((int64_t)O * J), "bdetr_linear_bwd_data_multi: operand %d spans 4 GB or more (32-bit buffer offsets)", k);
+        for (int q = 0; q < n; ++q)
+            BDETR_CHECK_ARG(m[q].dx != e.dy && m[q].dx != e.w, "bdetr_linear_bwd_data_multi: output %d aliases an operand of member %d", q, k);
+        const bool cont = k > 0 && e.dx == m[k - 1].dx;
+        if (cont) {
+            BDETR_CHECK_ARG(e.rows == m[k - 1].rows && e.old == nullptr, "bdetr_linear_bwd_data_multi: members of one output share its row count; only the first names `old`");
+            ++ms.count[ms.nout - 1];
+        } else {
+            for (int q = 0; q < ms.nout; ++q)
+                BDETR_CHECK_ARG(ms.c[q] != e.dx, "bdetr_linear_bwd_data_multi: the members of one output must be consecutive (member %d)", k);
+            BDETR_CHECK_ARG(ms.nout < MULTI_MAX_OUT, "bdetr_linear_bwd_data_multi: at most %d distinct outputs", MULTI_MAX_OUT);
+            const int o = ms.nout++;
+            ms.I[o] = e.rows; ms.first[o] = k; ms.count[o] = 1; ms.c[o] = e.dx; ms.old[o] = e.old;
+        }
+        ms.a[k] = e.dy; ms.b[k] = e.w;
+        if (e.rows > maxI) maxI = e.rows;
+    }
+    for (int o = 0; o < ms.nout; ++o)
+        for (int q = 0; q < ms.nout; ++q)
+            BDETR_CHECK_ARG(q == o || ms.old[o] != ms.c[q], "bdetr_linear_bwd_data_multi: `old` of output %d is output %d", o, q);
+    const int arith = use_split(true);
+    BDETR_CHECK_ARG(arith != AR_FP16X3 && multi_tile_ok(maxI, J, ms.nout, arith),
+                    "bdetr_linear_bwd_data_multi: no multi-source kernel for this shape / policy (ask bdetr_linear_bwd_data_multi_ok first)");
+    GemmParams g; init_params(g);
+    g.I = maxI; g.J = J; g.R = O;
+    g.c = ms.c[0]; g.ldc = J;
+    DenseOp a{ms.a[0], O, 0, 0, maxI, O};
+    DenseOp b{ms.b[0], J, 0, 0, O, J};
+    hipStream_t st = (hipStream_t)stream;
+    if (arith == AR_BF16X3) return launch_multi<AR_BF16X3>(a, b, g, ms, n, st);
+    if (arith == AR_BF16X6) return launch_multi<AR_BF16X6>(a, b, g, ms, n, st);
+    return launch_multi<AR_FP32>(a, b, g, ms, n, st);
+}
+
 extern "C" int bdetr_gemm(const bdetr_gemm_desc* d, void* stream) { return bdetr_gemm_ws(d, nullptr, 0, stream); }
 
 template <class F>
diff --git a/boosted_detr_amd/csrc/igemm_kernel.inc b/boosted_detr_amd/csrc/igemm_kernel.inc
--- /dev/null
+++ b/boosted_detr_amd/csrc/igemm_kernel.inc
@@ -0,0 +1,371 @@
+template <int BM, int BN, int WM, int WN, class LA, bool A_RC, class LB, bool B_RC, int ARITH>
+__global__ __launch_bounds__(NTHREADS, 2)
+void IGEMM_KERNEL(typename LA::Op opa, typename LB::Op opb, GemmParams g IGEMM_MULTI_PARAM)
+{
+    static_assert(WM * WN == 4, "4 waves per workgroup");
+    constexpr int WTM = BM / WM, WTN = BN / WN;
+    constexpr int TM = WTM / 32, TN = WTN / 32;
+    static_assert(TM >= 1 && TN >= 1, "wave tile must hold at least one 32x32 MFMA tile");
+    using GA = TileGeom<BM, A_RC>;
+    using GB = TileGeom<BN, B_RC>;
+    static_assert(GA::NV >= 1 && GB::NV >= 1, "tile too small for 256 threads");
+
+    constexpr bool SPLIT = ARITH != AR_FP32;
+    constexpr bool X6 = ARITH == AR_BF16X6;
+    constexpr int SLDK = X6 ? SLD3 : SLD;
+    constexpr int A_FLOATS = SPLIT ? BM * SLDK : GA::LDS_FLOATS;
+    constexpr int B_FLOATS = SPLIT ? BN * SLDK : GB::LDS_FLOATS;
+    constexpr int STAGE_FLOATS = A_FLOATS + B_FLOATS;
+    static_assert(!SPLIT || ((A_RC || GA::NV % 2 == 0) && (B_RC || GB::NV % 2 == 0)), "split mode transposes k-pairs");
+    __shared__ __attribute__((aligned(16))) float lds[2 * STAGE_FLOATS];
+
+    const int tid = threadIdx.x;
+    const int lane = tid & 63;
+    const int wave = tid >> 6;
+    const int wm = wave / WN, wn = wave % WN;
+    const int li = lane & 31, lh = lane >> 5;
+
+    const int nwg_ = g.tiles_i * g.tiles_j;
+    const bool sk_ = g.ngroups == 0 && g.splitk > 1;
+    const int lin_ = sk_ ? xcd_tile(blockIdx.z * nwg_ + blockIdx.x, nwg_ * gridDim.z) : xcd_tile(blockIdx.x, nwg_);
+    const int zz_ = sk_ ? lin_ / nwg_ : blockIdx.z;
+    const int wg = sk_ ? lin_ - zz_ * nwg_ : lin_;
+    const int tile_i = wg / g.tiles_j, tile_j = wg - tile_i * g.tiles_j;
+    const int i0 = tile_i * BM, j0 = tile_j * BN;
+
+    int b0 = 0, b1 = 0, r_begin = 0, r_end = g.R;
+#if IGEMM_MULTI
+    const int msz = (int)blockIdx.z;
+#define BDETR_PICK(arr) (msz == 0 ? ms.arr[0] : msz == 1 ? ms.arr[1] : msz == 2 ? ms.arr[2] : ms.arr[3])
+    const float* const ms_old = BDETR_PICK(old);
+    const int ms_first = BDETR_PICK(first), ms_count = BDETR_PICK(count);
+    g.I = BDETR_PICK(I); g.c = BDETR_PICK(c);
+#undef BDETR_PICK
+    if (i0 >= g.I) return;
+    LA::regroup(opa, ms.a[ms_first], g.I, A_RC);
+    LB::regroup(opb, ms.b[ms_first], -1, B_RC);
+    if (false) {
+    } else
+#endif
+    if (g.ngroups > 0) {
+        const int z = g.splitk > 1 ? (int)blockIdx.z / g.splitk : (int)blockIdx.z;
+        if (g.splitk > 1) {
+            r_begin = ((int)blockIdx.z - z * g.splitk) * g.r_chunk;
+            r_end = min(g.R, r_begin + g.r_chunk);
+        }
+#define BDETR_PICK(arr) (z == 0 ? g.arr[0] : z == 1 ? g.arr[1] : z == 2 ? g.arr[2] : g.arr[3])
+        g.I = BDETR_PICK(gI); g.c = BDETR_PICK(gc); g.bias = BDETR_PICK(gbias);
+        const float* pa = BDETR_PICK(ga);
+        const float* pb = BDETR_PICK(gb);
+#undef BDETR_PICK
+        if (i0 >= g.I) return;
+        LA::regroup(opa, pa, g.I, A_RC);
+        LB::regroup(opb, pb, -1, B_RC);
+    } else if (g.splitk > 1) {
+        r_begin = zz_ * g.r_chunk;
+        r_end = min(g.R, r_begin + g.r_chunk);
+    } else {
+        b0 = blockIdx.z / g.nb1; b1 = blockIdx.z - b0 * g.nb1;
+    }
+#if IGEMM_MULTI
+    __amdgpu_buffer_rsrc_t rsA = make_rsrc(opa.p), rsB = make_rsrc(opb.p);
+#else
+    const __amdgpu_buffer_rsrc_t rsA = make_rsrc(LA::batch_base(opa, b0, b1));
+    const __amdgpu_buffer_rsrc_t rsB = make_rsrc(LB::batch_base(opb, b0, b1));
+#endif
+    const int a_rows = A_RC ? opa.rows : min(opa.rows, r_end), a_cols = A_RC ? min(opa.cols, r_end) : opa.cols;
+    const int b_rows = B_RC ? opb.rows : min(opb.rows, r_end), b_cols = B_RC ? min(opb.cols, r_end) : opb.cols;
+
+    typename LA::Ctx ctxA[GA::NV];
+    typename LB::Ctx ctxB[GB::NV];
+    int colA[GA::NV], colB[GB::NV], ldsoffA[GA::NV], ldsoffB[GB::NV], rowA[GA::NV], rowB[GB::NV];
+    auto stage_geom = [&](int p, int vpr, int bx, bool rc, int lds_ld, int& row, int& col, int& ldsoff) {
+        if (!SPLIT) {
+            const int v = tid + NTHREADS * p;
+            const int rt = v / vpr, c4 = v - rt * vpr;
+            row = rt; col = 4 * c4; ldsoff = rt * lds_ld + 4 * c4;
+        } else if (rc) {
+            const int v = tid + NTHREADS * p;
+            const int q = v / vpr, c4 = v - q * vpr;
+            const int rt = (q & ~15) | ((q & 3) << 2) | ((q >> 2) & 3);
+            row = rt; col = 4 * c4;
+            ldsoff = rt * SLDK * 32 + ((((c4 >> 1) ^ ((rt >> 4) & 7)) << 2) | ((c4 & 1) << 1));
+        } else {
+            const int u = tid + NTHREADS * (p >> 1);
+            const int kp = u / (bx / 4), c4 = u - kp * (bx / 4);
+            row = 2 * kp + (p & 1); col = 4 * c4;
+            ldsoff = (4 * c4) * SLDK * 32 + ((((kp >> 2) ^ ((c4 >> 2) & 7)) << 2) | (kp & 3));
+        }
+    };
+#pragma unroll
+    for (int p = 0; p < GA::NV; ++p) {
+        stage_geom(p, GA::VPR, BM, A_RC, GA::LDS_LD, rowA[p], colA[p], ldsoffA[p]);
+        if (A_RC) ctxA[p] = LA::row_ctx(opa, i0 + rowA[p], a_rows);
+    }
+#pragma unroll
+    for (int p = 0; p < GB::NV; ++p) {
+        stage_geom(p, GB::VPR, BN, B_RC, GB::LDS_LD, rowB[p], colB[p], ldsoffB[p]);
+        if (B_RC) ctxB[p] = LB::row_ctx(opb, j0 + rowB[p], b_rows);
+    }
+
+    f32x4 stA0[GA::NV], stB0[GB::NV], stA1[GA::NV], stB1[GB::NV];
+    auto load_stage = [&](int r0, f32x4 (&ra)[GA::NV], f32x4 (&rb)[GB::NV]) {
+#pragma unroll
+        for (int p = 0; p < GA::NV; ++p) {
+            if (A_RC) ra[p] = LA::load(rsA, opa, ctxA[p], r0 + colA[p], a_cols);
+            else      ra[p] = LA::load(rsA, opa, LA::row_ctx(opa, r0 + rowA[p], a_rows), i0 + colA[p], a_cols);
+        }
+#pragma unroll
+        for (int p = 0; p < GB::NV; ++p) {
+            if (B_RC) rb[p] = LB::load(rsB, opb, ctxB[p], r0 + colB[p], b_cols);
+            else      rb[p] = LB::load(rsB, opb, LB::row_ctx(opb, r0 + rowB[p], b_rows), j0 + colB[p], b_cols);
+        }
+    };
+    auto write_split = [&](unsigned* base, bool rc, auto nv_c, const f32x4* r, const int* ldsoff) {
+        constexpr int nv = decltype(nv_c)::value;
+        if (rc) {
+#pragma unroll
+            for (int p = 0; p < nv; ++p) {
+                unsigned* row = base + (ldsoff[p] >> 5);
+                const int w = ldsoff[p] & 31;
+                if constexpr (X6) {
+                    unsigned h0, m0, l0, h1, m1, l1;
+                    split3(r[p][0], r[p][1], h0, m0, l0);
+                    split3(r[p][2], r[p][3], h1, m1, l1);
+                    u32x2 hi, mid, lo;
+                    hi[0] = h0; hi[1] = h1; mid[0] = m0; mid[1] = m1; lo[0] = l0; lo[1] = l1;
+                    *reinterpret_cast<u32x2*>(row + w) = hi;
+                    *reinterpret_cast<u32x2*>(row + (w ^ 16)) = mid;
+                    *reinterpret_cast<u32x2*>(row + 32 + (w & 15)) = lo;
+                } else {
+                    unsigned h0, l0, h1, l1;
+                    split2<ARITH>(r[p][0], r[p][1], h0, l0);
+                    split2<ARITH>(r[p][2], r[p][3], h1, l1);
+                    u32x2 hi, lo;
+                    hi[0] = h0; hi[1] = h1; lo[0] = l0; lo[1] = l1;
+                    *reinterpret_cast<u32x2*>(row + w) = hi;
+                    *reinterpret_cast<u32x2*>(row + (w ^ 16)) = lo;
+                }
+            }
+        } else {
+#pragma unroll
+            for (int p = 0; p + 1 < nv; p += 2) {
+                unsigned* row = base + (ldsoff[p] >> 5);
+                const int w = ldsoff[p] & 31;
+#pragma unroll
+                for (int e = 0; e < 4; ++e) {
+                    if constexpr (X6) {
+                        unsigned hi, mid, lo;
+                        split3(r[p][e], r[p + 1][e], hi, mid, lo);
+                        row[e * SLDK + w] = hi;
+                        row[e * SLDK + (w ^ 16)] = mid;
+                        row[e * SLDK + 32 + (w & 15)] = lo;
+                    } else {
+                        unsigned hi, lo;
+                        split2<ARITH>(r[p][e], r[p + 1][e], hi, lo);
+                        row[e * SLDK + w] = hi;
+                        row[e * SLDK + (w ^ 16)] = lo;
+                    }
+                }
+            }
+        }
+    };
+    auto write_stage = [&](int buf, const f32x4 (&ra)[GA::NV], const f32x4 (&rb)[GB::NV]) {
+        if (SPLIT) {
+            unsigned* st = reinterpret_cast<unsigned*>(lds + buf * STAGE_FLOATS);
+            write_split(st, A_RC, std::integral_constant<int, GA::NV>{}, ra, ldsoffA);
+            write_split(st + A_FLOATS, B_RC, std::integral_constant<int, GB::NV>{}, rb, ldsoffB);
+            return;
+        }
+#pragma unroll
+        for (int p = 0; p < GA::NV; ++p) *reinterpret_cast<f32x4*>(lds + buf * STAGE_FLOATS + ldsoffA[p]) = ra[p];
+#pragma unroll
+        for (int p = 0; p < GB::NV; ++p) *reinterpret_cast<f32x4*>(lds + buf * STAGE_FLOATS + GA::LDS_FLOATS + ldsoffB[p]) = rb[p];
+    };
+
+    constexpr int TM2 = ARITH == AR_FP16X3 ? TM : 1, TN2 = ARITH == AR_FP16X3 ? TN : 1;
+    f32x16 acc[TM][TN], acc2[TM2][TN2];
+#pragma unroll
+    for (int a = 0; a < TM; ++a)
+#pragma unroll
+        for (int b = 0; b < TN; ++b)
+#pragma unroll
+            for (int e = 0; e < 16; ++e) acc[a][b][e] = 0.f;
+#pragma unroll
+    for (int a = 0; a < TM2; ++a)
+#pragma unroll
+        for (int b = 0; b < TN2; ++b)
+#pragma unroll
+            for (int e = 0; e < 16; ++e) acc2[a][b][e] = 0.f;
+
+    auto compute = [&](int buf) {
+        if (SPLIT) {
+            const unsigned* qA = reinterpret_cast<const unsigned*>(lds + buf * STAGE_FLOATS);
+            const unsigned* qB = qA + A_FLOATS;
+#pragma unroll
+            for (int ks = 0; ks < BK / 16; ++ks) {
+                u32x4 ah[TM], al[TM], bh[TN], bl[TN];
+                u32x4 a3[X6 ? TM : 1], b3[X6 ? TN : 1];
+#pragma unroll
+                for (int a = 0; a < TM; ++a) {
+                    const int xb = wm * WTM + a * 32 + li;
+                    const int w = ((ks * 2 + lh) ^ ((xb >> 4) & 7)) << 2;
+                    ah[a] = *reinterpret_cast<const u32x4*>(qA + xb * SLDK + w);
+                    al[a] = *reinterpret_cast<const u32x4*>(qA + xb * SLDK + (w ^ 16));
+                    if constexpr (X6) a3[a] = *reinterpret_cast<const u32x4*>(qA + xb * SLDK + 32 + (w & 15));
+                }
+#pragma unroll
+                for (int b = 0; b < TN; ++b) {
+                    const int xb = wn * WTN + b * 32 + li;
+                    const int w = ((ks * 2 + lh) ^ ((xb >> 4) & 7)) << 2;
+                    bh[b] = *reinterpret_cast<const u32x4*>(qB + xb * SLDK + w);
+                    bl[b] = *reinterpret_cast<const u32x4*>(qB + xb * SLDK + (w ^ 16));
+                    if constexpr (X6) b3[b] = *reinterpret_cast<const u32x4*>(qB + xb * SLDK + 32 + (w & 15));
+                }
+#pragma unroll
+                for (int a = 0; a < TM; ++a)
+#pragma unroll
+                    for (int b = 0; b < TN; ++b) {
+                        if constexpr (X6) {
+#define BF8(v) __builtin_bit_cast(bf16x8, v)
+                            acc[a][b] = __builtin_amdgcn_mfma_f32_32x32x16_bf16(BF8(a3[a]), BF8(bh[b]), acc[a][b], 0, 0, 0);
+                            acc[a][b] = __builtin_amdgcn_mfma_f32_32x32x16_bf16(BF8(ah[a]), BF8(b3[b]), acc[a][b], 0, 0, 0);
+                            acc[a][b] = __builtin_amdgcn_mfma_f32_32x32x16_bf16(BF8(al[a]), BF8(bl[b]), acc[a][b], 0, 0, 0);
+                            acc[a][b] = __builtin_amdgcn_mfma_f32_32x32x16_bf16(BF8(al[a]), BF8(bh[b]), acc[a][b], 0, 0, 0);
+                            acc[a][b] = __builtin_amdgcn_mfma_f32_32x32x16_bf16(BF8(ah[a]), BF8(bl[b]), acc[a][b], 0, 0, 0);
+                            acc[a][b] = __builtin_amdgcn_mfma_f32_32x32x16_bf16(BF8(ah[a]), BF8(bh[b]), acc[a][b], 0, 0, 0);
+#undef BF8
+                        } else if constexpr (ARITH == AR_BF16X3) {
+#define BF8(v) __builtin_bit_cast(bf16x8, v)
+                            acc[a][b] = __builtin_amdgcn_mfma_f32_32x32x16_bf16(BF8(al[a]), BF8(bh[b]), acc[a][b], 0, 0, 0);
+                            acc[a][b] = __builtin_amdgcn_mfma_f32_32x32x16_bf16(BF8(ah[a]), BF8(bl[b]), acc[a][b], 0, 0, 0);
+                            acc[a][b] = __builtin_amdgcn_mfma_f32_32x32x16_bf16(BF8(ah[a]), BF8(bh[b]), acc[a][b], 0, 0, 0);
+#undef BF8
+                        } else if constexpr (ARITH == AR_FP16X3) {
+#define H8(v) __builtin_bit_cast(f16x8, v)
+                            acc2[a][b] = __builtin_amdgcn_mfma_f32_32x32x16_f16(H8(al[a]), H8(bh[b]), acc2[a][b], 0, 0, 0);
+                            acc2[a][b] = __builtin_amdgcn_mfma_f32_32x32x16_f16(H8(ah[a]), H8(bl[b]), acc2[a][b], 0, 0, 0);
+                            acc[a][b] = __builtin_amdgcn_mfma_f32_32x32x16_f16(H8(ah[a]), H8(bh[b]), acc[a][b], 0, 0, 0);
+#undef H8
+                        }
+                    }
+            }
+            return;
+        }
+        const float* sA = lds + buf * STAGE_FLOATS;
+        const float* sB = sA + GA::LDS_FLOATS;
+#pragma unroll
+        for (int kb = 0; kb < BK / 8; ++kb) {
+            f32x4 fa[TM], fb[TN];
+#pragma unroll
+            for (int a = 0; a < TM; ++a) {
+                const int xb = wm * WTM + a * 32 + li;
+                if (A_RC) {
+                    fa[a] = *reinterpret_cast<const f32x4*>(sA + xb * GA::LDS_LD + kb * 8 + 4 * lh);
+                } else {
+#pragma unroll
+                    for (int e = 0; e < 4; ++e) fa[a][e] = sA[(kb * 8 + 4 * lh + e) * GA::LDS_LD + xb];
+                }
+            }
+#pragma unroll
+            for (int b = 0; b < TN; ++b) {
+                const int xb = wn * WTN + b * 32 + li;
+                if (B_RC) {
+                    fb[b] = *reinterpret_cast<const f32x4*>(sB + xb * GB::LDS_LD + kb * 8 + 4 * lh);
+                } else {
+#pragma unroll
+                    for (int e = 0; e < 4; ++e) fb[b][e] = sB[(kb * 8 + 4 * lh + e) * GB::LDS_LD + xb];
+                }
+            }
+#pragma unroll
+            for (int e = 0; e < 4; ++e)
+#pragma unroll
+                for (int a = 0; a < TM; ++a)
+#pragma unroll
+                    for (int b = 0; b < TN; ++b)
+                        acc[a][b] = __builtin_amdgcn_mfma_f32_32x32x2f32(fa[a][e], fb[b][e], acc[a][b], 0, 0, 0);
+        }
+    };
+
+    const int nk = (r_end - r_begin + BK - 1) / BK;
+    constexpr bool PF1 = SPLIT && BM * BN >= 128 * 128;
+#if IGEMM_MULTI
+    static_assert(ARITH != AR_FP16X3, "gradient products never take the fp16 split");
+    f32x16 run[TM][TN];
+#pragma unroll
+    for (int a = 0; a < TM; ++a)
+#pragma unroll
+        for (int b = 0; b < TN; ++b)
+#pragma unroll
+            for (int e = 0; e < 16; ++e) {
+                const int i = i0 + wm * WTM + a * 32 + (e & 3) + 8 * (e >> 2) + 4 * lh, j = j0 + wn * WTN + b * 32 + li;
+                run[a][b][e] = (ms_old != nullptr && i < g.I && j < g.J) ? ms_old[(int64_t)i * g.ldc + j] : 0.f;
+            }
+    for (int ms_m = 0; ms_m < ms_count; ++ms_m) {
+    if (ms_m > 0) {
+        rsA = make_rsrc(ms.a[ms_first + ms_m]);
+        rsB = make_rsrc(ms.b[ms_first + ms_m]);
+#pragma unroll
+        for (int a = 0; a < TM; ++a)
+#pragma unroll
+            for (int b = 0; b < TN; ++b)
+#pragma unroll
+                for (int e = 0; e < 16; ++e) acc[a][b][e] = 0.f;
+    }
+#endif
+    if constexpr (PF1) {
+        if (nk > 0) { load_stage(r_begin, stA0, stB0); write_stage(0, stA0, stB0); }
+        __syncthreads();
+        for (int kt = 0; kt < nk; ++kt) {
+            if (kt + 1 < nk) load_stage(r_begin + (kt + 1) * BK, stA0, stB0);
+            compute(kt & 1);
+            if (kt + 1 < nk) write_stage((kt + 1) & 1, stA0, stB0);
+            __syncthreads();
+        }
+    } else {
+    if (nk > 0) {
+        load_stage(r_begin, stA0, stB0);
+        if (nk > 1) load_stage(r_begin + BK, stA1, stB1);
+        write_stage(0, stA0, stB0);
+    }
+    __syncthreads();
+
+    for (int kt = 0; kt < nk; kt += 2) {
+        if (kt + 2 < nk) load_stage(r_begin + (kt + 2) * BK, stA0, stB0);
+        compute(0);
+        if (kt + 1 < nk) write_stage(1, stA1, stB1);
+        __syncthreads();
+        if (kt + 1 >= nk) break;
+        if (kt + 3 < nk) load_stage(r_begin + (kt + 3) * BK, stA1, stB1);
+        compute(1);
+        if (kt + 2 < nk) write_stage(0, stA0, stB0);
+        __syncthreads();
+    }
+    }
+#if IGEMM_MULTI
+    {
+        const bool copy = ms_m == 0 && ms_old == nullptr;
+#pragma unroll
+        for (int a = 0; a < TM; ++a)
+#pragma unroll
+            for (int b = 0; b < TN; ++b)
+#pragma unroll
+                for (int e = 0; e < 16; ++e) run[a][b][e] = copy ? acc[a][b][e] : run[a][b][e] + acc[a][b][e];
+    }
+    }
+#pragma unroll
+    for (int a = 0; a < TM; ++a)
+#pragma unroll
+        for (int b = 0; b < TN; ++b) acc[a][b] = run[a][b];
+#endif
+
+    if constexpr (ARITH == AR_FP16X3) {
+#pragma unroll
+        for (int a = 0; a < TM; ++a)
+#pragma unroll
+            for (int b = 0; b < TN; ++b)
+#pragma unroll
+                for (int e = 0; e < 16; ++e) acc[a][b][e] += acc2[a][b][e] * (1.f / LO_SCALE);
+    }
+    gemm_epilogue<BM, BN, WM, WN, NTHREADS, 2 * STAGE_FLOATS>(acc, g, lds, tile_i, i0, j0, g.c + (int64_t)(sk_ ? zz_ : b0) * g.sc0 + (int64_t)b1 * g.sc1);
+}
diff --git a/boosted_detr_amd/engine.py b/boosted_detr_amd/engine.py
--- a/boosted_detr_amd/engine.py
+++ b/boosted_detr_amd/engine.py
@@ -226,7 +226,10 @@
                 for t in inputs:
                     have = grads.get(id(t)) if t is not None else None
                     acc.append(have if info(have).owned else None)
-                gins = fn(*gouts, acc=acc)
+                if getattr(fn, "wants_have", False):
+                    gins = fn(*gouts, acc=acc, have=[grads.get(id(t)) if t is not None else None for t in inputs])
+                else:
+                    gins = fn(*gouts, acc=acc)
             else:
                 gins = fn(*gouts)
             if not isinstance(gins, (tuple, list)):
diff --git a/boosted_detr_amd/kernels.py b/boosted_detr_amd/kernels.py
--- a/boosted_detr_amd/kernels.py
+++ b/boosted_detr_amd/kernels.py
@@ -8,7 +8,7 @@
 import torch
 
 from . import _lib
-from ._lib import BnAffine, BnBwdFuse, ConvDesc, GemmDesc, LossDesc, RowchainBwdDesc, RowchainFwdDesc, check
+from ._lib import BnAffine, BnBwdFuse, BwdDataMember, ConvDesc, GemmDesc, LossDesc, RowchainBwdDesc, RowchainFwdDesc, check
 
 ACT_NONE, ACT_RELU, ACT_TANH = 0, 1, 2
 
@@ -477,6 +477,50 @@
     dxs = [empty(dy.shape[0], K_, like=dy) for dy in dys]
     gemm_grouped([(dy.shape[0], K_, O, dy, O, True, w, K_, False, dx, K_, None, ACT_NONE, False) for dy, w, dx in zip(dys, ws, dxs)])
     return dxs
+
+
+FANIN = [_os.environ.get("BDETR_FANIN", "1") != "0"]
+
+
+def linear_bwd_data_fanin(dys, ws, slots, olds, owned):
+    order = sorted(range(len(dys)), key=lambda k: slots[k])
+    nslots = max(slots) + 1
+    first = [next(k for k in order if slots[k] == s) for s in range(nslots)]
+    O, K_ = ws[0].shape
+    _chk(*dys, *ws, *olds)
+    same = all(tuple(w.shape) == (O, K_) for w in ws) and all(dy.dim() == 2 and dy.shape[1] == O for dy in dys)
+    aligned = same and O % 4 == 0 and K_ % 4 == 0 and all(t.data_ptr() % 16 == 0 for t in (*dys, *ws, *(o for o in olds if o is not None)))
+    rows = [dys[k].shape[0] for k in first]
+    fused = (FANIN[0] and aligned and len(dys) <= 16 and nslots <= 4
+             and all(dys[k].shape[0] == rows[slots[k]] for k in order)
+             and all(o is None or tuple(o.shape) == (r, K_) for o, r in zip(olds, rows))
+             and _lib.lib().bdetr_linear_bwd_data_multi_ok(max(rows), O, K_, nslots) == 1)
+    if fused:
+        outs = [o if (o is not None and own_) else empty(r, K_, like=dys[0]) for o, own_, r in zip(olds, owned, rows)]
+        arr = (BwdDataMember * len(order))()
+        for n, k in enumerate(order):
+            s = slots[k]
+            arr[n] = BwdDataMember(_p(dys[k]), _p(ws[k]), _p(outs[s]), _p(olds[s]) if k == first[s] else None, dys[k].shape[0])
+        check(_lib.lib().bdetr_linear_bwd_data_multi(arr, len(order), O, K_, _stream()), "linear_bwd_data_multi")
+        return outs
+    if aligned:
+        prods = []
+        for c in range(0, len(dys), 4):
+            prods += linear_bwd_data_group(dys[c:c + 4], ws[c:c + 4])
+    else:
+        prods = [linear_bwd_data(dy, w) for dy, w in zip(dys, ws)]
+    outs = [None] * nslots
+    for k in order:
+        s, p = slots[k], prods[k]
+        if outs[s] is not None:
+            axpy_(1.0, p, outs[s])
+        elif olds[s] is None:
+            outs[s] = p
+        elif owned[s]:
+            outs[s] = axpy_(1.0, p, olds[s])
+        else:
+            outs[s] = add(olds[s], p)
+    return outs
 
 
 def linear_fwd(x2d, w, bias, act=ACT_NONE):
diff --git a/boosted_detr_amd/ops.py b/boosted_detr_amd/ops.py
--- a/boosted_detr_amd/ops.py
+++ b/boosted_detr_amd/ops.py
@@ -577,7 +577,7 @@
     y2 = K.linear_fwd_group(x2, [w.value for w in ws], [b.value for b in bs])
     ys = [y.view(*x.shape[:-1], y.shape[1]) for y, x in zip(y2, xs)]
 
-    def backward(*gs):
+    def backward(*gs, acc=None, have=None):
         g2 = [_2d(g.contiguous()) for g in gs]
 
         def param_grads():
@@ -601,9 +601,28 @@
                 s.commit()
         if any(w.needs_grad or b.needs_grad for w, b in zip(ws, bs)):
             side_task(param_grads, *x2, *g2)
-        dxs = K.linear_bwd_data_group(g2, [w.value for w in ws])
-        return tuple(own(dx.view(x.shape)) for dx, x in zip(dxs, xs))
-
+        slot_of, slots = {}, []
+        for x in xs:
+            slots.append(slot_of.setdefault(id(x), len(slot_of)))
+        first = [slots.index(s_) for s_ in range(len(slot_of))]
+        held = [have[i] if have is not None else None for i in first]
+        plain = all(h is None or (info(h).lazy_mask is None and info(h).compact_even is None and h.is_contiguous() and h.shape == xs[i].shape)
+                    for h, i in zip(held, first))
+        if not K.FANIN[0] or acc is None or have is None or not plain:
+            dxs = K.linear_bwd_data_group(g2, [w.value for w in ws])
+            return tuple(own(dx.view(x.shape)) for dx, x in zip(dxs, xs))
+        owned = [acc[i] is not None for i in first]
+        outs = K.linear_bwd_data_fanin(g2, [w.value for w in ws], slots, [_2d(h) if h is not None else None for h in held], owned)
+        gins = [None] * len(xs)
+        for i, h, o, out in zip(first, held, owned, outs):
+            if h is not None:
+                dense_contribution(h)
+            gins[i] = h if (h is not None and o) else own(out.view(xs[i].shape))
+            if h is not None:
+                acc[i] = gins[i]
+        return tuple(gins)
+
+    backward.wants_acc = backward.wants_have = True
     _rec(ys, list(xs), backward)
     return ys
 
diff --git a/include/bdetr.h b/include/bdetr.h
--- a/include/bdetr.h
+++ b/include/bdetr.h
@@ -118,6 +118,11 @@
 int bdetr_gemm(const bdetr_gemm_desc* g, void* stream);
 int bdetr_gemm_ws(const bdetr_gemm_desc* g, float* ws, int64_t ws_elems, void* stream);
 int bdetr_gemm_grouped(const bdetr_gemm_desc* g, int n, void* stream);
+typedef struct {
+    const float* dy; const float* w; float* dx; const float* old; int rows;
+} bdetr_bwd_data_member;
+int bdetr_linear_bwd_data_multi_ok(int max_rows, int out_features, int in_features, int outputs);
+int bdetr_linear_bwd_data_multi(const bdetr_bwd_data_member* m, int n, int out_features, int in_features, void* stream);
 
 int bdetr_colsum_chunks(int64_t rows);
 int bdetr_colsum(const float* x, int64_t rows, int cols, float* out, float* ws, void* stream);
```

Result: no change. 661.6, median of 6 (+0.7%).
